# lisvulaczo/lodestar

Hardware: AMD Instinct MI355X
Metric: BLS signature sets verified/sec (whole node) at 1/2/4/8 MI355X; p50 batch latency (higher is better)
Workload: dtype u32

## Files before the change

### include/lodestar_bls.h

```cpp
#ifndef LODESTAR_BLS_H
#define LODESTAR_BLS_H

#include <stddef.h>
#include <stdint.h>

#ifdef __cplusplus
extern "C" {
#endif

#define LSG_OK 0
#define LSG_ERR_INVALID_ARG 1
#define LSG_ERR_NO_DEVICE 2
#define LSG_ERR_DEVICE 3
#define LSG_ERR_NOMEM 4
#define LSG_ERR_CLOSED 5
#define LSG_ERR_BUSY 6
#define LSG_ERR_ENTROPY 7

#define LSG_BLST_SUCCESS 0
#define LSG_BLST_BAD_ENCODING 1
#define LSG_BLST_POINT_NOT_ON_CURVE 2
#define LSG_BLST_POINT_NOT_IN_GROUP 3
#define LSG_BLST_AGGR_TYPE_MISMATCH 4
#define LSG_BLST_VERIFY_FAIL 5
// ... 35 lines not shown

typedef struct {
  int32_t status;
  int32_t err_code;
} lsg_job_result;

typedef struct {
  uint32_t batch_retries;
  uint32_t batch_sigs_success;
  uint64_t start_ns;
  uint64_t end_ns;
  uint32_t n_final_exps;
  uint32_t submit_us;
  int32_t key_error;
  uint32_t key_error_job;
} lsg_stats;

int lsg_init(int device_ordinal, lsg_ctx** out);
int lsg_init_devices(const int* device_ids, int n_devices, lsg_ctx** out);
int lsg_destroy(lsg_ctx* ctx);
int lsg_device_count(lsg_ctx* ctx, int32_t* n);
const char* lsg_last_error(lsg_ctx* ctx);
int lsg_device_name(lsg_ctx* ctx, char* buf, size_t len);
int lsg_reserve(lsg_ctx* ctx, size_t max_sets, size_t max_pks, size_t max_msg_bytes, int32_t n_slots);
int lsg_allocation_count(lsg_ctx* ctx, uint64_t* n);

int lsg_submit_jobs(lsg_ctx* ctx, const lsg_job* jobs, size_t n_jobs, uint64_t seed, lsg_ticket* ticket);
int lsg_wait_jobs(lsg_ctx* ctx, lsg_ticket ticket, lsg_job_result* results , lsg_stats* stats);
int lsg_jobs_partial(lsg_ctx* ctx, lsg_ticket ticket, uint8_t* out576, int32_t* has_batch);
int lsg_jobs_partial_device(lsg_ctx* ctx, lsg_ticket ticket, void* dev_out576, int32_t* has_batch);
int lsg_wait_jobs_node(lsg_ctx* ctx, lsg_ticket ticket, int32_t node_valid, lsg_job_result* results,
                       lsg_stats* stats);
int lsg_set_coalesce(lsg_ctx* ctx, uint32_t max_sets, int32_t max_inflight);
int lsg_assign_jobs(const uint32_t* job_sets, size_t n_jobs, int32_t n_devices, int32_t* owner);
int lsg_pipeline_slots(lsg_ctx* ctx, int32_t* n);
int lsg_poll(lsg_ctx* ctx, lsg_ticket ticket, int32_t* done);
int lsg_verify_jobs(lsg_ctx* ctx, const lsg_job* jobs, size_t n_jobs, uint64_t seed, lsg_job_result* results,
                    lsg_stats* stats);

int lsg_verify_sets(lsg_ctx* ctx, const lsg_set* sets, size_t n_sets, uint64_t seed, lsg_job_result* result);

int lsg_aggregate_pubkeys(lsg_ctx* ctx, const uint8_t* pks, uint32_t pk_len, size_t n, uint8_t* out96,
                          int32_t* err_code);
int lsg_aggregate_pubkeys_multi(lsg_ctx* ctx, const lsg_set* sets, size_t n_sets, uint8_t* out96, int32_t* err);

int lsg_hash_to_g2(lsg_ctx* ctx, const uint8_t* msgs, uint32_t msg_len, size_t n, const uint8_t* dst,
                   uint32_t dst_len, uint8_t* out192);

int lsg_sig_decode(lsg_ctx* ctx, const uint8_t* sigs, uint32_t sig_len, size_t n, uint8_t* out192, int32_t* err);

int lsg_batch_partial(lsg_ctx* ctx, const lsg_set* sets, size_t n_sets, uint64_t seed, uint8_t* out576,
                      int32_t* set_err, int32_t* any_error);
int lsg_final_verify(lsg_ctx* ctx, const uint8_t* partials576, size_t n_partials, int32_t* valid);
int lsg_final_submit(lsg_ctx* ctx, const uint8_t* partials576, size_t n_partials, lsg_ticket* ticket);
int lsg_final_submit_device(lsg_ctx* ctx, const void* dev_partials576, size_t n_partials, lsg_ticket* ticket);
int lsg_final_wait(lsg_ctx* ctx, lsg_ticket ticket, int32_t* valid);
int lsg_final_submit_groups(lsg_ctx* ctx, const uint8_t* partials576, size_t n_groups, size_t per_group,
                            lsg_ticket* ticket);
int lsg_final_wait_groups(lsg_ctx* ctx, lsg_ticket ticket, int32_t* valid );

int lsg_pubkey_table_set(lsg_ctx* ctx, size_t first_index, const uint8_t* pks, uint32_t pk_len, size_t n,
                         int32_t* err);
int lsg_pubkey_table_size(lsg_ctx* ctx, size_t* n);

int lsg_pubkey_validate(lsg_ctx* ctx, const uint8_t* pks, uint32_t pk_len, size_t n, uint8_t* out96, int32_t* err);

int lsg_aggregate_signatures(lsg_ctx* ctx, const uint8_t* sigs, uint32_t sig_len, const uint32_t* offsets,
                             size_t n_groups, uint8_t* out96, int32_t* err);

int lsg_signing_roots(lsg_ctx* ctx, const uint8_t* roots32, size_t n, const uint8_t* domain32, uint32_t domain_stride,
                      uint8_t* out32);
int lsg_attestation_signing_roots(lsg_ctx* ctx, const uint8_t* data128, size_t n, const uint8_t* domain32,
                                  uint32_t domain_stride, uint8_t* out32);
int lsg_deposit_signing_roots(lsg_ctx* ctx, const uint8_t* msgs88, size_t n, const uint8_t* domain32,
                              uint32_t domain_stride, uint8_t* out32);

int lsg_verify_deposits(lsg_ctx* ctx, const uint8_t* data184, size_t n, const uint8_t* domain32, uint64_t seed,
                        uint8_t* valid, int32_t* err);

int lsg_sign(lsg_ctx* ctx, const uint8_t* sks32, const uint8_t* msgs, uint32_t msg_len, size_t n, uint8_t* out96);
int lsg_sk_to_pk(lsg_ctx* ctx, const uint8_t* sks32, size_t n, uint8_t* out96);

int lsg_check_fp2_mul(lsg_ctx* ctx, const uint32_t* in, size_t n, uint32_t* out);
int lsg_probe_fp_mul_rate(lsg_ctx* ctx, double* fp_mul_per_s, double* mad_per_s);

int lsg_probe_mad_peak(lsg_ctx* ctx, double* mad_per_s);

int lsg_last_kernel_times(lsg_ctx* ctx, const char** names, double* ms, int max);

#ifdef __cplusplus
}
#endif
#endif
```

### lodestar_amd/_native.py

```python
import ctypes
import os
import struct
import threading

HERE = os.path.dirname(os.path.abspath(__file__))
LIB_PATH = os.environ.get("LSG_LIB", os.path.join(HERE, "liblodestar_bls.so"))
AB_LIB_PATH = os.path.join(HERE, "liblodestar_bls_ab.so")

LSG_OK = 0
LSG_ERR_NO_DEVICE = 2
LSG_ERR_BUSY = 6
LSG_ERR_ENTROPY = 7

LSG_INVALID = 0
LSG_VALID = 1
LSG_ERROR = 2

LSG_JOB_BATCHABLE = 1
LSG_JOB_PRIORITY = 2
LSG_JOB_VALIDATE_KEYS = 4

BLST_NAMES = {
    0: "BLST_SUCCESS", 1: "BLST_BAD_ENCODING", 2: "BLST_POINT_NOT_ON_CURVE", 3: "BLST_POINT_NOT_IN_GROUP",
    4: "BLST_AGGR_TYPE_MISMATCH", 5: "BLST_VERIFY_FAIL", 6: "BLST_PK_IS_INFINITY", 7: "BLST_BAD_SCALAR",
    10: "BLST_INVALID_SIZE",
}
LSG_ERR_EMPTY_SET = 100
LSG_ERR_EMPTY_AGGREGATE = 101
LSG_ERR_BAD_INDEX = 102
LSG_PK_INDEX = 4


def error_message(code):
    if code == LSG_ERR_EMPTY_SET:
        return "Empty signature set"
    if code == LSG_ERR_EMPTY_AGGREGATE:
        return "EMPTY_AGGREGATE_ARRAY"
    if code == LSG_ERR_BAD_INDEX:
        return "Unknown pubkey index"
    return "BLST_ERROR: " + BLST_NAMES.get(code, f"BLST_UNKNOWN_{code}")


class NativeUnavailable(RuntimeError):
    pass


class PkIndices(list):

    def tobytes(self):
        import array
        a = array.array("I", self)
        assert a.itemsize == 4
        return a.tobytes()


class LsgSet(ctypes.Structure):
    _fields_ = [
        ("pks", ctypes.c_void_p), ("pk_len", ctypes.c_uint32), ("n_pks", ctypes.c_uint32),
        ("msg", ctypes.c_void_p), ("msg_len", ctypes.c_uint32),
        ("sig", ctypes.c_void_p), ("sig_len", ctypes.c_uint32),
    ]


class LsgJob(ctypes.Structure):
    _fields_ = [("sets", ctypes.POINTER(LsgSet)), ("n_sets", ctypes.c_uint32), ("flags", ctypes.c_uint32)]


class LsgJobResult(ctypes.Structure):
    _fields_ = [("status", ctypes.c_int32), ("err_code", ctypes.c_int32)]


class LsgStats(ctypes.Structure):
    _fields_ = [
        ("batch_retries", ctypes.c_uint32), ("batch_sigs_success", ctypes.c_uint32),
        ("start_ns", ctypes.c_uint64), ("end_ns", ctypes.c_uint64),
        ("n_final_exps", ctypes.c_uint32), ("submit_us", ctypes.c_uint32),
        ("key_error", ctypes.c_int32), ("key_error_job", ctypes.c_uint32),
    ]


_lib = None
_lib_lock = threading.Lock()

EXPORTS = [
    "lsg_init", "lsg_init_devices", "lsg_destroy", "lsg_device_count", "lsg_last_error", "lsg_device_name",
    "lsg_reserve", "lsg_allocation_count", "lsg_verify_jobs", "lsg_verify_sets",
    "lsg_aggregate_pubkeys", "lsg_hash_to_g2", "lsg_sig_decode", "lsg_batch_partial", "lsg_final_verify",
    "lsg_probe_fp_mul_rate", "lsg_last_kernel_times", "lsg_sign", "lsg_sk_to_pk",
    "lsg_submit_jobs", "lsg_wait_jobs", "lsg_wait_jobs_node", "lsg_jobs_partial", "lsg_assign_jobs", "lsg_poll",
    "lsg_final_submit", "lsg_final_wait", "lsg_pipeline_slots", "lsg_probe_mad_peak",
    "lsg_pubkey_table_set", "lsg_pubkey_table_size", "lsg_pubkey_validate",
    "lsg_final_submit_groups", "lsg_final_wait_groups", "lsg_aggregate_signatures",
    "lsg_signing_roots", "lsg_attestation_signing_roots", "lsg_jobs_partial_device", "lsg_final_submit_device",
    "lsg_set_coalesce", "lsg_aggregate_pubkeys_multi", "lsg_check_fp2_mul",
    "lsg_deposit_signing_roots", "lsg_verify_deposits",
]


def load_library(path=LIB_PATH):
    global _lib
    with _lib_lock:
        if _lib is not None and path == LIB_PATH:
            return _lib
        if not os.path.exists(path):
            raise NativeUnavailable(f"{path} not built (run python -c 'import __graft_entry__; __graft_entry__.build()')")
        lib = ctypes.CDLL(path)
        vp, u32, u64, i32, sz = ctypes.c_void_p, ctypes.c_uint32, ctypes.c_uint64, ctypes.c_int32, ctypes.c_size_t
        pi32 = ctypes.POINTER(ctypes.c_int32)
        lib.lsg_init.argtypes = [ctypes.c_int, ctypes.POINTER(vp)]
        lib.lsg_init_devices.argtypes = [ctypes.POINTER(ctypes.c_int), ctypes.c_int, ctypes.POINTER(vp)]
        lib.lsg_device_count.argtypes = [vp, pi32]
        lib.lsg_reserve.argtypes = [vp, sz, sz, sz, i32]
        lib.lsg_allocation_count.argtypes = [vp, ctypes.POINTER(u64)]
        lib.lsg_wait_jobs_node.argtypes = [vp, u64, i32, ctypes.POINTER(LsgJobResult), ctypes.POINTER(LsgStats)]
        lib.lsg_jobs_partial.argtypes = [vp, u64, ctypes.c_char_p, pi32]
        lib.lsg_jobs_partial_device.argtypes = [vp, u64, vp, pi32]
        lib.lsg_final_submit_device.argtypes = [vp, vp, sz, ctypes.POINTER(u64)]
        lib.lsg_assign_jobs.argtypes = [ctypes.POINTER(u32), sz, i32, pi32]
        lib.lsg_destroy.argtypes = [vp]
        lib.lsg_last_error.argtypes = [vp]
        lib.lsg_last_error.restype = ctypes.c_char_p
        lib.lsg_device_name.argtypes = [vp, ctypes.c_char_p, sz]
        lib.lsg_verify_jobs.argtypes = [vp, ctypes.POINTER(LsgJob), sz, u64, ctypes.POINTER(LsgJobResult),
                                        ctypes.POINTER(LsgStats)]
        lib.lsg_verify_sets.argtypes = [vp, ctypes.POINTER(LsgSet), sz, u64, ctypes.POINTER(LsgJobResult)]
        lib.lsg_aggregate_pubkeys.argtypes = [vp, ctypes.c_char_p, u32, sz, ctypes.c_char_p, pi32]
        lib.lsg_aggregate_pubkeys_multi.argtypes = [vp, ctypes.POINTER(LsgSet), sz, ctypes.c_char_p, pi32]
        lib.lsg_hash_to_g2.argtypes = [vp, ctypes.c_char_p, u32, sz, ctypes.c_char_p, u32, ctypes.c_char_p]
        lib.lsg_sig_decode.argtypes = [vp, ctypes.c_char_p, u32, sz, ctypes.c_char_p, pi32]
        lib.lsg_batch_partial.argtypes = [vp, ctypes.POINTER(LsgSet), sz, u64, ctypes.c_char_p, pi32, pi32]
        lib.lsg_final_verify.argtypes = [vp, ctypes.c_char_p, sz, pi32]
        lib.lsg_probe_fp_mul_rate.argtypes = [vp, ctypes.POINTER(ctypes.c_double), ctypes.POINTER(ctypes.c_double)]
        lib.lsg_last_kernel_times.argtypes = [vp, ctypes.POINTER(ctypes.c_char_p), ctypes.POINTER(ctypes.c_double),
                                              ctypes.c_int]
        lib.lsg_sign.argtypes = [vp, ctypes.c_char_p, ctypes.c_char_p, u32, sz, ctypes.c_char_p]
        lib.lsg_sk_to_pk.argtypes = [vp, ctypes.c_char_p, sz, ctypes.c_char_p]
        pu64 = ctypes.POINTER(u64)
        lib.lsg_submit_jobs.argtypes = [vp, ctypes.POINTER(LsgJob), sz, u64, pu64]
        lib.lsg_wait_jobs.argtypes = [vp, u64, ctypes.POINTER(LsgJobResult), ctypes.POINTER(LsgStats)]
        lib.lsg_poll.argtypes = [vp, u64, pi32]
        lib.lsg_pubkey_table_set.argtypes = [vp, sz, ctypes.c_char_p, u32, sz, pi32]
        lib.lsg_pubkey_table_size.argtypes = [vp, ctypes.POINTER(sz)]
        lib.lsg_final_submit_groups.argtypes = [vp, ctypes.c_char_p, sz, sz, pu64]
        lib.lsg_final_wait_groups.argtypes = [vp, u64, pi32]
        lib.lsg_pubkey_validate.argtypes = [vp, ctypes.c_char_p, u32, sz, ctypes.c_char_p, pi32]
        lib.lsg_signing_roots.argtypes = [vp, ctypes.c_char_p, sz, ctypes.c_char_p, u32, ctypes.c_char_p]
        lib.lsg_attestation_signing_roots.argtypes = [vp, ctypes.c_char_p, sz, ctypes.c_char_p, u32, ctypes.c_char_p]
        lib.lsg_deposit_signing_roots.argtypes = [vp, ctypes.c_char_p, sz, ctypes.c_char_p, u32, ctypes.c_char_p]
        lib.lsg_verify_deposits.argtypes = [vp, ctypes.c_char_p, sz, ctypes.c_char_p, u64, ctypes.c_char_p, pi32]
        lib.lsg_aggregate_signatures.argtypes = [vp, ctypes.c_char_p, u32, ctypes.POINTER(u32), sz,
                                                 ctypes.c_char_p, pi32]
        lib.lsg_final_submit.argtypes = [vp, ctypes.c_char_p, sz, pu64]
        lib.lsg_final_wait.argtypes = [vp, u64, pi32]
        lib.lsg_pipeline_slots.argtypes = [vp, pi32]
        lib.lsg_set_coalesce.argtypes = [vp, u32, i32]
        lib.lsg_check_fp2_mul.argtypes = [vp, ctypes.c_char_p, sz, ctypes.c_char_p]
        lib.lsg_probe_mad_peak.argtypes = [vp, ctypes.POINTER(ctypes.c_double)]
        for name in EXPORTS:
            if name != "lsg_last_error":
                getattr(lib, name).restype = ctypes.c_int
        if path == LIB_PATH:
            _lib = lib
        return lib


class SetBuffer:

    def __init__(self, sets):
        self._keep = []
        sets = list(sets)
        self.arr = (LsgSet * max(len(sets), 1))()
        for i, (pks, msg, sig) in enumerate(sets):
            if isinstance(pks, PkIndices):
                pk_len, pkb = LSG_PK_INDEX, pks.tobytes()
            else:
                pk_len = len(pks[0]) if pks else 96
                if any(len(p) != pk_len for p in pks):
                    raise ValueError("all pubkeys of one set must share one encoding length")
                pkb = b"".join(pks)
            for b in (pkb, msg, sig):
                self._keep.append(b)
            s = self.arr[i]
            s.pks = ctypes.cast(ctypes.c_char_p(pkb), ctypes.c_void_p) if pkb else None
            s.pk_len = pk_len
            s.n_pks = len(pks)
            s.msg = ctypes.cast(ctypes.c_char_p(msg), ctypes.c_void_p) if msg else None
            s.msg_len = len(msg)
            s.sig = ctypes.cast(ctypes.c_char_p(sig), ctypes.c_void_p) if sig else None
            s.sig_len = len(sig)
        self.n = len(sets)


def assign_jobs(job_sizes, n_devices):
    lib = load_library()
    n = len(job_sizes)
    sizes = (ctypes.c_uint32 * max(n, 1))(*job_sizes)
    owner = (ctypes.c_int32 * max(n, 1))()
    rc = lib.lsg_assign_jobs(sizes, n, int(n_devices), owner)
    if rc != LSG_OK:
        raise ValueError(f"lsg_assign_jobs failed ({rc})")
    return list(owner[:n])


class PreparedJobs:

    def __init__(self, jobs):
        import numpy as np
        flat = [st for sets, _ in jobs for st in sets]
        n = len(flat)
        pk_parts, pk_len, n_pks = [], np.zeros(max(n, 1), np.uint32), np.zeros(max(n, 1), np.uint32)
        for i, (pks, _m, _s) in enumerate(flat):
            if isinstance(pks, PkIndices):
                pk_len[i], b = LSG_PK_INDEX, pks.tobytes()
            else:
                pk_len[i] = len(pks[0]) if pks else 96
                if any(len(p) != pk_len[i] for p in pks):
                    raise ValueError("all pubkeys of one set must share one encoding length")
                b = b"".join(pks)
            n_pks[i] = len(pks)
            pk_parts.append(b)

        def pack(parts):
            lens = np.array([len(p) for p in parts] or [0], np.uint64)
            offs = np.zeros_like(lens)
            if len(parts) > 1:
                offs[1:] = np.cumsum(lens)[:-1]
            buf = np.frombuffer(b"".join(parts) + b"\0", dtype=np.uint8).copy()
            return buf, offs, lens

        self._pk, pk_off, _ = pack(pk_parts)
        self._msg, msg_off, msg_len = pack([m for _, m, _ in flat])
        self._sig, sig_off, sig_len = pack([s for _, _, s in flat])
        self.sets = (LsgSet * max(n, 1))()
        dt = np.dtype({"names": ["pks", "pk_len", "n_pks", "msg", "msg_len", "sig", "sig_len"],
                       "formats": [np.uint64, np.uint32, np.uint32, np.uint64, np.uint32, np.uint64, np.uint32],
                       "offsets": [LsgSet.pks.offset, LsgSet.pk_len.offset, LsgSet.n_pks.offset, LsgSet.msg.offset,
                                   LsgSet.msg_len.offset, LsgSet.sig.offset, LsgSet.sig_len.offset],
                       "itemsize": ctypes.sizeof(LsgSet)})
        v = np.frombuffer(self.sets, dtype=dt)
# ... 268 lines not shown
            return []
        sl = len(sigs[0])
        assert all(len(s) == sl for s in sigs)
        out = ctypes.create_string_buffer(192 * len(sigs))
        err = (ctypes.c_int32 * len(sigs))()
        self._check(self.lib.lsg_sig_decode(self.h, b"".join(sigs), sl, len(sigs), out, err), "lsg_sig_decode")
        raw = out.raw
        return [(raw[192 * i:192 * i + 192], err[i]) for i in range(len(sigs))]

    def batch_partial(self, sets, seed=0):
        b = SetBuffer(sets)
        out = ctypes.create_string_buffer(576)
        errs = (ctypes.c_int32 * max(b.n, 1))()
        anyerr = ctypes.c_int32()
        self._check(self.lib.lsg_batch_partial(self.h, b.arr, b.n, seed, out, errs, ctypes.byref(anyerr)),
                    "lsg_batch_partial")
        return out.raw, [errs[i] for i in range(b.n)], bool(anyerr.value)

    def final_verify(self, partials):
        v = ctypes.c_int32()
        self._check(self.lib.lsg_final_verify(self.h, b"".join(partials), len(partials), ctypes.byref(v)),
                    "lsg_final_verify")
        return bool(v.value)

    def final_submit(self, partials):
        t = ctypes.c_uint64()
        rc = self.lib.lsg_final_submit(self.h, b"".join(partials), len(partials), ctypes.byref(t))
        if rc == LSG_ERR_BUSY:
            return None
        self._check(rc, "lsg_final_submit")
        return t.value

    def final_wait(self, ticket):
        v = ctypes.c_int32()
        self._check(self.lib.lsg_final_wait(self.h, ticket, ctypes.byref(v)), "lsg_final_wait")
        return bool(v.value)

    def final_submit_groups(self, groups):
        ng = len(groups)
        pg = len(groups[0]) if groups else 0
        if any(len(g) != pg for g in groups):
            raise ValueError("every group needs the same number of partials")
        t = ctypes.c_uint64()
        rc = self.lib.lsg_final_submit_groups(self.h, b"".join(b"".join(g) for g in groups), ng, pg, ctypes.byref(t))
        if rc == LSG_ERR_BUSY:
            return None
        self._check(rc, "lsg_final_submit_groups")
        t_ng = ng
        return (t.value, t_ng)

    def final_wait_groups(self, ticket):
        t, ng = ticket
        v = (ctypes.c_int32 * max(ng, 1))()
        self._check(self.lib.lsg_final_wait_groups(self.h, t, v), "lsg_final_wait_groups")
        return [bool(x) for x in v[:ng]]

    def sign(self, sks, msgs):
        if not sks:
            return []
        ml = len(msgs[0])
        out = ctypes.create_string_buffer(96 * len(sks))
        skb = b"".join(int(k).to_bytes(32, "big") for k in sks)
        self._check(self.lib.lsg_sign(self.h, skb, b"".join(msgs), ml, len(sks), out), "lsg_sign")
        raw = out.raw
        return [raw[96 * i:96 * i + 96] for i in range(len(sks))]

    def sk_to_pk(self, sks):
        if not sks:
            return []
        out = ctypes.create_string_buffer(96 * len(sks))
        skb = b"".join(int(k).to_bytes(32, "big") for k in sks)
        self._check(self.lib.lsg_sk_to_pk(self.h, skb, len(sks), out), "lsg_sk_to_pk")
        raw = out.raw
        return [raw[96 * i:96 * i + 96] for i in range(len(sks))]

    def check_fp2_mul(self, words):
        n = len(words) // 56
        assert len(words) == 56 * n
        out = ctypes.create_string_buffer(4 * 28 * n)
        src = struct.pack(f"<{len(words)}I", *words)
        self._check(self.lib.lsg_check_fp2_mul(self.h, src, n, out), "lsg_check_fp2_mul")
        return list(struct.unpack(f"<{28 * n}I", out.raw))

    def probe_fp_mul_rate(self):
        a, b = ctypes.c_double(), ctypes.c_double()
        self._check(self.lib.lsg_probe_fp_mul_rate(self.h, ctypes.byref(a), ctypes.byref(b)), "lsg_probe_fp_mul_rate")
        return a.value, b.value

    def last_kernel_times(self, max_entries=1024):
        names = (ctypes.c_char_p * max_entries)()
        ms = (ctypes.c_double * max_entries)()
        n = self.lib.lsg_last_kernel_times(self.h, names, ms, max_entries)
        return [(names[i].decode(), ms[i]) for i in range(n)]
```

### lodestar_amd/csrc/lsg_curve.hpp

```cpp
#pragma once
#include "lsg_tower.hpp"

LSG_INL fp_t fadd(const fp_t& a, const fp_t& b) { return fp_add(a, b); }
LSG_INL fp2_t fadd(const fp2_t& a, const fp2_t& b) { return fp2_add(a, b); }
LSG_INL fp_t fsub(const fp_t& a, const fp_t& b) { return fp_sub(a, b); }
LSG_INL fp2_t fsub(const fp2_t& a, const fp2_t& b) { return fp2_sub(a, b); }
LSG_INL fp_t fmul(const fp_t& a, const fp_t& b) { return fp_mul(a, b); }
LSG_INL fp2_t fmul(const fp2_t& a, const fp2_t& b) { return fp2_mul(a, b); }
LSG_INL fp_t fsqr(const fp_t& a) { return fp_sqr(a); }
LSG_INL fp2_t fsqr(const fp2_t& a) { return fp2_sqr(a); }
LSG_INL fp_t fneg(const fp_t& a) { return fp_neg(a); }
LSG_INL fp2_t fneg(const fp2_t& a) { return fp2_neg(a); }
LSG_INL fp_t fmul_b3(const fp_t& a) { return fp_mul12(a); }
LSG_INL fp2_t fmul_b3(const fp2_t& a) { return fp2_mul_b3(a); }
LSG_INL bool fis_zero(const fp_t& a) { return fp_is_zero(a); }
LSG_INL bool fis_zero(const fp2_t& a) { return fp2_is_zero(a); }
LSG_INL bool feq(const fp_t& a, const fp_t& b) { return fp_eq(a, b); }
LSG_INL bool feq(const fp2_t& a, const fp2_t& b) { return fp2_eq(a, b); }
LSG_INL fp_t fselect(bool c, const fp_t& a, const fp_t& b) { return fp_select(c, a, b); }
LSG_INL fp2_t fselect(bool c, const fp2_t& a, const fp2_t& b) { return fp2_select(c, a, b); }
LSG_INL fp_t finv(const fp_t& a) { return fp_inv(a); }
LSG_INL fp2_t finv(const fp2_t& a) { return fp2_inv(a); }
template <class F> LSG_INL F fzero();
template <> LSG_INL fp_t fzero<fp_t>() { return fp_zero(); }
template <> LSG_INL fp2_t fzero<fp2_t>() { return fp2_zero(); }
template <class F> LSG_INL F fone();
template <> LSG_INL fp_t fone<fp_t>() { return FP_ONE; }
template <> LSG_INL fp2_t fone<fp2_t>() { return fp2_one(); }

template <class F>
struct aff_t {
  F x, y;
};
template <class F>
struct proj_t {
  F X, Y, Z;
};
typedef aff_t<fp_t> g1a_t;
typedef aff_t<fp2_t> g2a_t;
typedef proj_t<fp_t> g1p_t;
typedef proj_t<fp2_t> g2p_t;

template <class F>
LSG_INL proj_t<F> proj_inf() {
  proj_t<F> r;
  r.X = fzero<F>();
  r.Y = fone<F>();
  r.Z = fzero<F>();
  return r;
}

template <class F>
LSG_INL proj_t<F> proj_from_aff(const aff_t<F>& a) {
  proj_t<F> r;
  r.X = a.x;
  r.Y = a.y;
  r.Z = fone<F>();
  return r;
}

template <class F>
LSG_INL bool proj_is_inf(const proj_t<F>& a) {
  return fis_zero(a.Z);
}

template <class F>
LSG_INL proj_t<F> proj_neg(const proj_t<F>& a) {
  proj_t<F> r = a;
  r.Y = fneg(a.Y);
  return r;
}

template <class F>
LSG_INL proj_t<F> proj_add(const proj_t<F>& p, const proj_t<F>& q) {
  F t0 = fmul(p.X, q.X);
  F t1 = fmul(p.Y, q.Y);
  F t2 = fmul(p.Z, q.Z);
  F t3 = fmul(fadd(p.X, p.Y), fadd(q.X, q.Y));
  F t4 = fadd(t0, t1);
  t3 = fsub(t3, t4);
  t4 = fmul(fadd(p.Y, p.Z), fadd(q.Y, q.Z));
  F X3 = fadd(t1, t2);
  t4 = fsub(t4, X3);
  X3 = fmul(fadd(p.X, p.Z), fadd(q.X, q.Z));
  F Y3 = fadd(t0, t2);
  Y3 = fsub(X3, Y3);
  X3 = fadd(t0, t0);
  t0 = fadd(X3, t0);
  t2 = fmul_b3(t2);
  F Z3 = fadd(t1, t2);
  t1 = fsub(t1, t2);
  Y3 = fmul_b3(Y3);
  X3 = fmul(t4, Y3);
  t2 = fmul(t3, t1);
  X3 = fsub(t2, X3);
  Y3 = fmul(Y3, t0);
  t1 = fmul(t1, Z3);
  Y3 = fadd(t1, Y3);
  t0 = fmul(t0, t3);
  Z3 = fmul(Z3, t4);
  Z3 = fadd(Z3, t0);
  proj_t<F> r;
  r.X = X3;
  r.Y = Y3;
  r.Z = Z3;
  return r;
}

template <class F>
LSG_INL proj_t<F> proj_add_mixed(const proj_t<F>& p, const aff_t<F>& q) {
  F t0 = fmul(p.X, q.x);
  F t1 = fmul(p.Y, q.y);
  F t3 = fmul(fadd(q.x, q.y), fadd(p.X, p.Y));
  F t4 = fadd(t0, t1);
  t3 = fsub(t3, t4);
  t4 = fadd(fmul(q.y, p.Z), p.Y);
  F Y3 = fadd(fmul(q.x, p.Z), p.X);
  F X3 = fadd(t0, t0);
  t0 = fadd(X3, t0);
  F t2 = fmul_b3(p.Z);
  F Z3 = fadd(t1, t2);
  t1 = fsub(t1, t2);
  Y3 = fmul_b3(Y3);
  X3 = fmul(t4, Y3);
  t2 = fmul(t3, t1);
  X3 = fsub(t2, X3);
  Y3 = fmul(Y3, t0);
  t1 = fmul(t1, Z3);
  Y3 = fadd(t1, Y3);
  t0 = fmul(t0, t3);
  Z3 = fmul(Z3, t4);
  Z3 = fadd(Z3, t0);
  proj_t<F> r;
  r.X = X3;
  r.Y = Y3;
  r.Z = Z3;
  return r;
}

template <class F>
LSG_INL proj_t<F> proj_dbl(const proj_t<F>& p) {
  F t0 = fsqr(p.Y);
  F Z3 = fadd(t0, t0);
  Z3 = fadd(Z3, Z3);
  Z3 = fadd(Z3, Z3);
  F t1 = fmul(p.Y, p.Z);
  F t2 = fmul_b3(fsqr(p.Z));
  F X3 = fmul(t2, Z3);
  F Y3 = fadd(t0, t2);
  Z3 = fmul(t1, Z3);
  t1 = fadd(t2, t2);
  t2 = fadd(t1, t2);
  t0 = fsub(t0, t2);
  Y3 = fmul(t0, Y3);
  Y3 = fadd(X3, Y3);
  t1 = fmul(p.X, p.Y);
  X3 = fmul(t0, t1);
  X3 = fadd(X3, X3);
  proj_t<F> r;
  r.X = X3;
  r.Y = Y3;
  r.Z = Z3;
  return r;
}

LSG_BIGFN g1p_t g1_add(g1p_t p, g1p_t q) { return proj_add(p, q); }
LSG_BIGFN g1p_t g1_add_mixed(g1p_t p, g1a_t q) { return proj_add_mixed(p, q); }
LSG_BIGFN g1p_t g1_dbl(g1p_t p) { return proj_dbl(p); }
#ifdef LSG_ROW_SPLIT
LSG_INL void kar_prep(fp_t* x, fp_t* y, int k, const fp2_t& a, const fp2_t& b) {
  x[k] = a.c0;
  y[k] = b.c0;
  x[k + 1] = a.c1;
  y[k + 1] = b.c1;
  x[k + 2] = fp_add(a.c0, a.c1);
  y[k + 2] = fp_add(b.c0, b.c1);
}
LSG_INL fp2_t kar_fin(const fp_t* z, int k) {
  return fp2_t(fp_sub(z[k], z[k + 1]), fp_sub(fp_sub(z[k + 2], z[k]), z[k + 1]));
}
LSG_INL g2p_t g2_add_rows(const g2p_t& p, const g2p_t& q) {
  fp_t x[18], y[18], z[18];
  kar_prep(x, y, 0, p.X, q.X);
  kar_prep(x, y, 3, p.Y, q.Y);
  kar_prep(x, y, 6, p.Z, q.Z);
  kar_prep(x, y, 9, fp2_add(p.X, p.Y), fp2_add(q.X, q.Y));
  kar_prep(x, y, 12, fp2_add(p.Y, p.Z), fp2_add(q.Y, q.Z));
  kar_prep(x, y, 15, fp2_add(p.X, p.Z), fp2_add(q.X, q.Z));
  fp_mul_list<18>(z, x, y);
  fp2_t t0 = kar_fin(z, 0), t1 = kar_fin(z, 3), t2 = kar_fin(z, 6);
  const fp2_t t3 = fp2_sub(kar_fin(z, 9), fp2_add(t0, t1));
  const fp2_t t4 = fp2_sub(kar_fin(z, 12), fp2_add(t1, t2));
  fp2_t Y3 = fp2_sub(kar_fin(z, 15), fp2_add(t0, t2));
  t0 = fp2_add(fp2_add(t0, t0), t0);
  t2 = fp2_mul_b3(t2);
  const fp2_t Z3 = fp2_add(t1, t2);
  t1 = fp2_sub(t1, t2);
  Y3 = fp2_mul_b3(Y3);
  kar_prep(x, y, 0, t4, Y3);
  kar_prep(x, y, 3, t3, t1);
  kar_prep(x, y, 6, Y3, t0);
  kar_prep(x, y, 9, t1, Z3);
  kar_prep(x, y, 12, t0, t3);
  kar_prep(x, y, 15, Z3, t4);
  fp_mul_list<18>(z, x, y);
  g2p_t r;
  r.X = fp2_sub(kar_fin(z, 3), kar_fin(z, 0));
  r.Y = fp2_add(kar_fin(z, 9), kar_fin(z, 6));
  r.Z = fp2_add(kar_fin(z, 15), kar_fin(z, 12));
  return r;
}
LSG_INL g2p_t g2_dbl_rows(const g2p_t& p) {
  fp_t x[12], y[12], z[12];
  kar_prep(x, y, 0, p.Y, p.Y);
  kar_prep(x, y, 3, p.Y, p.Z);
  kar_prep(x, y, 6, p.Z, p.Z);
  kar_prep(x, y, 9, p.X, p.Y);
  fp_mul_list<12>(z, x, y);
  const fp2_t t0 = kar_fin(z, 0), t1 = kar_fin(z, 3), t2 = fp2_mul_b3(kar_fin(z, 6)), xy = kar_fin(z, 9);
  const fp2_t z8 = fp2_dbl(fp2_dbl(fp2_dbl(t0)));
  const fp2_t y3 = fp2_add(t0, t2);
  const fp2_t s0 = fp2_sub(t0, fp2_add(fp2_add(t2, t2), t2));
  kar_prep(x, y, 0, t2, z8);
  kar_prep(x, y, 3, t1, z8);
  kar_prep(x, y, 6, s0, y3);
  kar_prep(x, y, 9, s0, xy);
  fp_mul_list<12>(z, x, y);
  g2p_t r;
  r.X = fp2_dbl(kar_fin(z, 9));
  r.Y = fp2_add(kar_fin(z, 0), kar_fin(z, 6));
  r.Z = kar_fin(z, 3);
  return r;
}
LSG_BIGFN g2p_t g2_add(g2p_t p, g2p_t q) { return g2_add_rows(p, q); }
LSG_BIGFN g2p_t g2_dbl(g2p_t p) { return g2_dbl_rows(p); }
#else
LSG_BIGFN g2p_t g2_add(g2p_t p, g2p_t q) { return proj_add(p, q); }
LSG_BIGFN g2p_t g2_dbl(g2p_t p) { return proj_dbl(p); }
#endif
LSG_BIGFN g2p_t g2_add_mixed(g2p_t p, g2a_t q) { return proj_add_mixed(p, q); }

LSG_INL g1p_t gadd(const g1p_t& p, const g1p_t& q) { return g1_add(p, q); }
LSG_INL g2p_t gadd(const g2p_t& p, const g2p_t& q) { return g2_add(p, q); }
LSG_INL g1p_t gdbl(const g1p_t& p) { return g1_dbl(p); }
LSG_INL g2p_t gdbl(const g2p_t& p) { return g2_dbl(p); }

template <class F>
struct jac_t {
  F X, Y, Z;
};

template <class F>
LSG_INL jac_t<F> jac_from_proj(const proj_t<F>& p) {
  F zz = fsqr(p.Z);
  jac_t<F> r;
  bool inf = fis_zero(p.Z);
  r.X = fselect(inf, fone<F>(), fmul(p.X, p.Z));
  r.Y = fselect(inf, fone<F>(), fmul(p.Y, zz));
  r.Z = p.Z;
  return r;
}

template <class F>
LSG_INL proj_t<F> jac_to_proj(const jac_t<F>& p) {
  F zz = fsqr(p.Z);
  proj_t<F> r;
  bool inf = fis_zero(p.Z);
  r.X = fmul(p.X, p.Z);
  r.Y = fselect(inf, fone<F>(), p.Y);
  r.Z = fmul(zz, p.Z);
  return r;
}

template <class F>
LSG_INL jac_t<F> jac_dbl_t(const jac_t<F>& p) {
  F A = fsqr(p.X);
  F B = fsqr(p.Y);
  F C = fsqr(B);
  F D = fsub(fsqr(fadd(p.X, B)), fadd(A, C));
  D = fadd(D, D);
  F E = fadd(fadd(A, A), A);
  F Fq = fsqr(E);
  jac_t<F> r;
  r.X = fsub(Fq, fadd(D, D));
  F C8 = fadd(C, C);
  C8 = fadd(C8, C8);
  C8 = fadd(C8, C8);
  r.Y = fsub(fmul(E, fsub(D, r.X)), C8);
  F yz = fmul(p.Y, p.Z);
  r.Z = fadd(yz, yz);
  return r;
}
LSG_BIGFN jac_t<fp_t> jac_dbl(jac_t<fp_t> p) { return jac_dbl_t(p); }
LSG_BIGFN jac_t<fp2_t> jac_dbl(jac_t<fp2_t> p) { return jac_dbl_t(p); }

template <class F>
LSG_INL jac_t<F> jac_add_proj(const jac_t<F>& acc, const proj_t<F>& q) {
  return jac_from_proj(gadd(jac_to_proj(acc), q));
}

template <class F>
LSG_INL proj_t<F> proj_mul_u64(const proj_t<F>& p, uint64_t k) {
  proj_t<F> T[16];
  T[0] = proj_inf<F>();
  T[1] = p;
  T[2] = gdbl(p);
#pragma unroll 1
  for (int d = 3; d < 16; d++) T[d] = gadd(T[d - 1], p);
  auto pick = [&](uint32_t d) { return T[d]; };
  jac_t<F> acc = jac_from_proj(pick((uint32_t)(k >> 60) & 15u));
#pragma unroll 1
  for (int w = 14; w >= 0; w--) {
    acc = jac_dbl(acc);
    acc = jac_dbl(acc);
    acc = jac_dbl(acc);
    acc = jac_dbl(acc);
    acc = jac_add_proj(acc, pick((uint32_t)(k >> (4 * w)) & 15u));
  }
  return jac_to_proj(acc);
}

template <class F>
LSG_INL proj_t<F> proj_pick_signed(const proj_t<F>& T1, const proj_t<F>& T2, const proj_t<F>& T3,
                                   const proj_t<F>& T4, int d) {
  const int a = d < 0 ? -d : d;
  proj_t<F> r = proj_inf<F>();
  auto take = [&](bool s, const proj_t<F>& t) {
    r.X = fselect(s, t.X, r.X);
    r.Y = fselect(s, t.Y, r.Y);
    r.Z = fselect(s, t.Z, r.Z);
  };
  take(a == 1, T1);
  take(a == 2, T2);
  take(a == 3, T3);
  take(a == 4, T4);
  r.Y = fselect(d < 0, fneg(r.Y), r.Y);
  return r;
}
template <class F>
LSG_INL proj_t<F> proj_mul_u64_s3(const proj_t<F>& p, uint64_t k) {
  const proj_t<F> T2 = gdbl(p);
  const proj_t<F> T3 = gadd(T2, p);
  const proj_t<F> T4 = gdbl(T2);
  uint32_t cm = 0;
#pragma unroll
  for (int i = 0; i < 21; i++) {
    const uint32_t v = (uint32_t)((k >> (3 * i)) & 7u) + ((cm >> i) & 1u);
    cm |= (v >= 4u ? 1u : 0u) << (i + 1);
  }
  auto digit = [&](int i) {
    return (int)((k >> (3 * i)) & 7u) + (int)((cm >> i) & 1u) - (i < 21 ? 8 * (int)((cm >> (i + 1)) & 1u) : 0);
  };
  jac_t<F> acc = jac_from_proj(proj_pick_signed(p, T2, T3, T4, digit(21)));
#pragma unroll 1
  for (int i = 20; i >= 0; i--) {
    acc = jac_dbl(acc);
    acc = jac_dbl(acc);
    acc = jac_dbl(acc);
    acc = jac_add_proj(acc, proj_pick_signed(p, T2, T3, T4, digit(i)));
  }
  return jac_to_proj(acc);
}

template <class F, class G>
LSG_INL proj_t<F> proj_mul_xabs_get(const G& get) {
  const uint64_t xa = ((uint64_t)LSG_X_ABS_HI << 32) | LSG_X_ABS_LO;
  jac_t<F> acc = jac_from_proj(get());
#pragma unroll 1
  for (int b = 62; b >= 0; b--) {
    acc = jac_dbl(acc);
    if ((xa >> b) & 1u) acc = jac_add_proj(acc, get());
  }
  return jac_to_proj(acc);
}
template <class F>
LSG_INL proj_t<F> proj_mul_xabs(const proj_t<F>& p) {
  return proj_mul_xabs_get<F>([&]() { return p; });
}

template <class F>
LSG_INL bool proj_eq(const proj_t<F>& a, const proj_t<F>& b) {
  bool ia = proj_is_inf(a), ib = proj_is_inf(b);
  if (ia || ib) return ia && ib;
  return feq(fmul(a.X, b.Z), fmul(b.X, a.Z)) && feq(fmul(a.Y, b.Z), fmul(b.Y, a.Z));
}

template <class F>
LSG_INL aff_t<F> proj_to_aff(const proj_t<F>& p) {
  F zi = finv(p.Z);
  aff_t<F> r;
  r.x = fmul(p.X, zi);
  r.y = fmul(p.Y, zi);
  return r;
}

LSG_INL g2p_t g2_psi(const g2p_t& p) {
  g2p_t r;
  r.X = fp2_mul(fp2_conj(p.X), PSI_CX);
  r.Y = fp2_mul(fp2_conj(p.Y), PSI_CY);
  r.Z = fp2_conj(p.Z);
  return r;
}
LSG_INL g2p_t g2_psi2(const g2p_t& p) {
  g2p_t r;
  r.X = fp2_mul_fp(p.X, PSI2_CX);
  r.Y = fp2_mul_fp(p.Y, PSI2_CY);
  r.Z = p.Z;
  return r;
}

template <class G>
LSG_INL bool g2_in_group_get(const G& get) {
  if (proj_is_inf(get())) return true;
  g2p_t xp = proj_neg(proj_mul_xabs_get<fp2_t>(get));
  return proj_eq(g2_psi(get()), xp);
}
LSG_BIGFN bool g2_in_group(g2p_t p) {
  return g2_in_group_get([&]() { return p; });
}

LSG_BIGFN bool g1_in_group(g1p_t p) {
  const uint32_t rw[8] = {0x73eda753u, 0x299d7d48u, 0x3339d808u, 0x09a1d805u,
                          0x53bda402u, 0xfffe5bfeu, 0xffffffffu, 0x00000001u};
  g1p_t acc = proj_inf<fp_t>();
#pragma unroll 1
  for (int w = 0; w < 8; w++) {
#pragma unroll 1
    for (int b = 31; b >= 0; b--) {
      acc = g1_dbl(acc);
      if ((rw[w] >> b) & 1u) acc = g1_add(acc, p);
    }
  }
  return proj_is_inf(acc);
}

LSG_INL bool g1_on_curve_aff(const g1a_t& a) {
  fp_t rhs = fp_add(fp_mul(fp_sqr(a.x), a.x), FP_B_G1);
  return fp_eq(fp_sqr(a.y), rhs);
}
LSG_INL bool g2_on_curve_aff(const g2a_t& a) {
  fp2_t rhs = fp2_add(fp2_mul(fp2_sqr(a.x), a.x), FP2_B_G2);
  return fp2_eq(fp2_sqr(a.y), rhs);
}

#ifndef LSG_BLST_SUCCESS
#define LSG_BLST_SUCCESS 0
#define LSG_BLST_BAD_ENCODING 1
#define LSG_BLST_POINT_NOT_ON_CURVE 2
#define LSG_BLST_POINT_NOT_IN_GROUP 3
#define LSG_BLST_AGGR_TYPE_MISMATCH 4
#define LSG_BLST_VERIFY_FAIL 5
#define LSG_BLST_PK_IS_INFINITY 6
#define LSG_BLST_BAD_SCALAR 7
#define LSG_BLST_INVALID_SIZE 10
#endif

LSG_INL int g2_uncompress(g2a_t& out, bool& inf, const uint8_t* in) {
  uint8_t in0 = in[0];
  inf = false;
  if (!(in0 & 0x80)) return LSG_BLST_BAD_ENCODING;
  if (in0 & 0x40) {
    uint32_t acc = in0 & 0x3f;
    for (int i = 1; i < 96; i++) acc |= in[i];
    if (acc == 0) {
      inf = true;
      out.x = fp2_zero();
      out.y = fp2_zero();
      return LSG_BLST_SUCCESS;
    }
    return LSG_BLST_BAD_ENCODING;
  }
  fp_t x1 = fp_from_be48(in);
  x1 = fp_mask_flags(x1);
  fp_t x0 = fp_from_be48(in + 48);
  if (!fp_canon_lt_p(x1) || !fp_canon_lt_p(x0)) return LSG_BLST_BAD_ENCODING;
  fp2_t x = fp2_make(fp_to_mont(x0), fp_to_mont(x1));
  fp2_t rhs = fp2_add(fp2_mul(fp2_sqr(x), x), FP2_B_G2);
  fp2_t y;
  if (!fp2_sqrt(y, rhs)) return LSG_BLST_POINT_NOT_ON_CURVE;
  bool want = (in0 & 0x20) != 0;
  if (fp2_lexi_largest(y) != want) y = fp2_neg(y);
  out.x = x;
  out.y = y;
  if (fp2_is_zero(x)) return LSG_BLST_POINT_NOT_IN_GROUP;
  return LSG_BLST_SUCCESS;
}

LSG_INL int g2_deserialize_uncompressed(g2a_t& out, bool& inf, const uint8_t* in) {
  uint8_t in0 = in[0];
  inf = false;
  if (in0 & 0x80) return LSG_BLST_BAD_ENCODING;
  if (in0 & 0x40) {
    uint32_t acc = in0 & 0x3f;
    for (int i = 1; i < 192; i++) acc |= in[i];
    if (acc == 0) {
      inf = true;
      out.x = fp2_zero();
      out.y = fp2_zero();
      return LSG_BLST_SUCCESS;
    }
// ... 87 lines not shown
```

### lodestar_amd/csrc/lsg_fp_pair.hpp

```cpp
#pragma once
#include "lsg_constants_r29.hpp"

#ifndef LSG_PAIR_G
#define LSG_PAIR_G 2
#endif
#define LSG_GROUP LSG_PAIR_G
#define LSG_PAIR_MODE 1
#define LSG_LEAN_TOWER 1
constexpr int LSG_PL = 14 / LSG_GROUP;
constexpr uint32_t LSG_M29 = (1u << 29) - 1;

#if LSG_PAIR_G == 2
#undef LSG_INL
#define LSG_INL __device__ __forceinline__
#undef LSG_NOINL
#define LSG_NOINL __device__ __noinline__
#define LSG_PFN __device__ __forceinline__
#define LSG_PLEAF __device__ __noinline__
LSG_PFN uint32_t pair_h() { return __lane_id() & 1u; }
template <int CTRL>
LSG_PFN uint32_t pdpp(uint32_t x) {
  return (uint32_t)__builtin_amdgcn_mov_dpp((int)x, CTRL, 0xf, 0xf, false);
}
template <int S>
// ... 311 lines not shown
  r.l[5] = hi[1];
  r.l[6] = hi[2];
  return r;
}
#define LSG_TAIL_PARAMS(x) fp_arg4_t x##_lo, fp_arg3_t x##_hi
#define LSG_TAIL_ARGS(v) fp_pack_lo(v), fp_pack_hi(v)
#define LSG_TAIL_UNPACK(x) fp_unpack2(x##_lo, x##_hi)
typedef uint32_t fp_arg_t __attribute__((ext_vector_type(8)));
LSG_PFN fp_arg_t fp_pack(const fp_t& a) {
  fp_arg_t v;
#pragma unroll
  for (int k = 0; k < LSG_PL; k++) v[k] = a.l[k];
  return v;
}
LSG_PFN fp_t fp_unpack(const fp_arg_t& v) {
  fp_t r;
#pragma unroll
  for (int k = 0; k < LSG_PL; k++) r.l[k] = v[k];
  return r;
}
#else
#define LSG_TAIL_PARAMS(x) fp_t x
#define LSG_TAIL_ARGS(v) (v)
#define LSG_TAIL_UNPACK(x) (x)
typedef fp_t fp_arg_t;
LSG_PFN fp_arg_t fp_pack(const fp_t& a) { return a; }
LSG_PFN fp_t fp_unpack(const fp_arg_t& v) { return v; }
#endif
struct fp_duo {
  fp_t x, y;
};
LSG_PLEAF fp_duo pair_mont_mul2_v(fp_arg_t a0, fp_arg_t b0, fp_arg_t a1, LSG_TAIL_PARAMS(b1)) {
  LSG_COUNT_MUL();
  LSG_COUNT_MUL();
  const fp_t x[2] = {fp_unpack(a0), fp_unpack(a1)}, y[2] = {fp_unpack(b0), LSG_TAIL_UNPACK(b1)};
  fp_t r[2];
#if LSG_LEAF_MODE == 2
  pair_mont_mul_n<2>(r, x, y);
#else
  pair_mont_mul_n<1>(&r[0], &x[0], &y[0]);
  LSG_SCHED_FENCE();
  pair_mont_mul_n<1>(&r[1], &x[1], &y[1]);
#endif
  return fp_duo{r[0], r[1]};
}
LSG_PFN fp_duo pair_mont_mul2(const fp_t& a0, const fp_t& b0, const fp_t& a1, const fp_t& b1) {
  return pair_mont_mul2_v(fp_pack(a0), fp_pack(b0), fp_pack(a1), LSG_TAIL_ARGS(b1));
}
LSG_PLEAF fp_duo pair_fp2_mul_v(fp_arg_t a0, fp_arg_t a1, fp_arg_t b0, LSG_TAIL_PARAMS(b1));
LSG_PLEAF fp_duo pair_fp2_sqr_v(fp_arg_t a0, fp_arg_t a1);
LSG_PFN fp_duo pair_fp2_mul(const fp_t& a0, const fp_t& a1, const fp_t& b0, const fp_t& b1) {
  return pair_fp2_mul_v(fp_pack(a0), fp_pack(a1), fp_pack(b0), LSG_TAIL_ARGS(b1));
}
LSG_PFN fp_duo pair_fp2_sqr(const fp_t& a0, const fp_t& a1) { return pair_fp2_sqr_v(fp_pack(a0), fp_pack(a1)); }
#if LSG_LEAF_MODE != 0
#define LSG_FP2_LEAF 1
#endif

LSG_PFN fp_t fp_zero() {
  fp_t r;
#pragma unroll
  for (int k = 0; k < LSG_PL; k++) r.l[k] = 0u;
  return r;
}
LSG_PFN fp_t fp_select(bool c, const fp_t& a, const fp_t& b) {
  fp_t r;
#pragma unroll
  for (int k = 0; k < LSG_PL; k++) r.l[k] = c ? a.l[k] : b.l[k];
  return r;
}
LSG_PFN fp_t fp_add(const fp_t& a, const fp_t& b) {
  fp_t r;
#pragma unroll
  for (int k = 0; k < LSG_PL; k++) r.l[k] = a.l[k] + b.l[k];
  return pair_carry(r);
}
LSG_PFN fp_t fp_sub(const fp_t& a, const fp_t& b) {
  fp_t r;
#pragma unroll
  for (int k = 0; k < LSG_PL; k++) r.l[k] = a.l[k] - b.l[k];
  return pair_carry(r);
}
LSG_PFN fp_t fp_neg(const fp_t& a) { return fp_sub(fp_zero(), a); }
LSG_PFN fp_t fp_mul(const fp_t& a, const fp_t& b) { return pair_mont_mul(a, b); }
#if LSG_LEAF_MODE == 0
LSG_PFN void fp_mul2(fp_t& r0, fp_t& r1, const fp_t& a0, const fp_t& b0, const fp_t& a1, const fp_t& b1) {
  fp_t t = pair_mont_mul(a0, b0);
  r1 = pair_mont_mul(a1, b1);
  r0 = t;
}
LSG_PFN void fp_mul3(fp_t& r0, fp_t& r1, fp_t& r2, const fp_t& a0, const fp_t& b0, const fp_t& a1, const fp_t& b1,
                     const fp_t& a2, const fp_t& b2) {
  fp_t t0 = pair_mont_mul(a0, b0);
  fp_t t1 = pair_mont_mul(a1, b1);
  r2 = pair_mont_mul(a2, b2);
  r0 = t0;
  r1 = t1;
}
#else
LSG_PFN void fp_mul2(fp_t& r0, fp_t& r1, const fp_t& a0, const fp_t& b0, const fp_t& a1, const fp_t& b1) {
  const fp_duo d = pair_mont_mul2(a0, b0, a1, b1);
  r0 = d.x;
  r1 = d.y;
}
LSG_PFN void fp_mul3(fp_t& r0, fp_t& r1, fp_t& r2, const fp_t& a0, const fp_t& b0, const fp_t& a1, const fp_t& b1,
                     const fp_t& a2, const fp_t& b2) {
  const fp_duo d = pair_mont_mul2(a0, b0, a1, b1);
  r2 = pair_mont_mul(a2, b2);
  r0 = d.x;
  r1 = d.y;
}
#endif
LSG_PFN void fp_mul9(fp_t* r, const fp_t* a, const fp_t* b) {
#pragma unroll
  for (int g = 0; g < 9; g += 3) fp_mul3(r[g], r[g + 1], r[g + 2], a[g], b[g], a[g + 1], b[g + 1], a[g + 2], b[g + 2]);
}

LSG_PLEAF fp_duo pair_fp2_mul_v(fp_arg_t va0, fp_arg_t va1, fp_arg_t vb0, LSG_TAIL_PARAMS(vb1)) {
  LSG_COUNT_MUL();
  LSG_COUNT_MUL();
  LSG_COUNT_MUL();
  const fp_t a0 = fp_unpack(va0), a1 = fp_unpack(va1), b0 = fp_unpack(vb0), b1 = LSG_TAIL_UNPACK(vb1);
#if LSG_FP2_SOP
  fp_duo d;
  pair_fp2_mul_sop(d.x, d.y, a0, a1, b0, b1);
  return d;
#endif
  fp_t t[3];
#if LSG_LEAF_MODE == 2
  const fp_t a[3] = {a0, a1, fp_add(a0, a1)}, b[3] = {b0, b1, fp_add(b0, b1)};
  pair_mont_mul_n<3>(t, a, b);
#else
  pair_mont_mul_n<1>(&t[0], &a0, &b0);
  LSG_SCHED_FENCE();
  pair_mont_mul_n<1>(&t[1], &a1, &b1);
  LSG_SCHED_FENCE();
  const fp_t s0 = fp_add(a0, a1), s1 = fp_add(b0, b1);
  pair_mont_mul_n<1>(&t[2], &s0, &s1);
#endif
  return fp_duo{fp_sub(t[0], t[1]), fp_sub(fp_sub(t[2], t[0]), t[1])};
}
LSG_PLEAF fp_duo pair_fp2_sqr_v(fp_arg_t va0, fp_arg_t va1) {
  LSG_COUNT_MUL();
  LSG_COUNT_MUL();
  const fp_t a0 = fp_unpack(va0), a1 = fp_unpack(va1);
  fp_t t[2];
#if LSG_LEAF_MODE == 2
  const fp_t a[2] = {fp_add(a0, a1), a0}, b[2] = {fp_sub(a0, a1), a1};
  pair_mont_mul_n<2>(t, a, b);
#else
  const fp_t s = fp_add(a0, a1), d = fp_sub(a0, a1);
  pair_mont_mul_n<1>(&t[0], &s, &d);
  LSG_SCHED_FENCE();
  pair_mont_mul_n<1>(&t[1], &a0, &a1);
#endif
  return fp_duo{t[0], fp_add(t[1], t[1])};
}

LSG_PLEAF fp_t pair_pow_fixed(fp_t a, const uint32_t* __restrict__ e) {
  auto mul = [](const fp_t& x, const fp_t& y) {
    LSG_COUNT_MUL();
    fp_t r;
    pair_mont_mul_n<1>(&r, &x, &y);
    return r;
  };
  fp_t T[8];
// ... 273 lines not shown
```

### lodestar_amd/csrc/lsg_host.hip

```cpp
#include <hip/hip_runtime.h>
#include <rccl/rccl.h>
#include <stdio.h>
#include <stdlib.h>
#include <errno.h>
#include <string.h>
#include <sys/random.h>
#include <time.h>

#include <algorithm>
#include <atomic>
#include <condition_variable>
#include <chrono>
#include <mutex>
#include <shared_mutex>
#include <thread>
#include <unordered_map>
#include <string>
#include <vector>

#include "../../include/lodestar_bls.h"
#include "lsg_launch.h"
#include "lsg_layout.h"
#include "lsg_serial.h"
#include "lsg_ab.h"
// ... 2952 lines not shown
    }
    return (int)LSG_OK;
  };
  size_t pkg = 0;
  for (size_t o = 0; o < n && !rc; pkg++) {
    const size_t cnt = std::min(DEPOSIT_PKG, n - o);
    lsg_ticket t = 0;
    if (out.size() >= DEPOSIT_INFLIGHT) {
      rc = wait_oldest();
      pkg--;
      continue;
    }
    {
      CtxLock lk(c->mu);
      const hipError_t he = hipSetDevice(d->device);
      if (he != hipSuccess)
        rc = fail_c(c, "hipSetDevice", he);
      else
        rc = submit_pkg(c, lk, jobs.data() + o, cnt, seed ? seed + 0x9e3779b97f4a7c15ull * pkg : 0, &t, true,
                        resident ? P_<uint8_t>(d->d_dep_roots) + 32 * o : nullptr);
    }
    if (rc == LSG_ERR_BUSY && !out.empty()) {
      rc = wait_oldest();
      pkg--;
      continue;
    }
    if (rc) break;
    out.push_back({t, o, cnt});
    o += cnt;
  }
  while (!out.empty()) {
    const int w = wait_oldest();
    if (!rc) rc = w;
  }
  return rc;
}

int lsg_sign(lsg_ctx* c, const uint8_t* sks32, const uint8_t* msgs, uint32_t msg_len, size_t n, uint8_t* out96) {
  if (!c || !out96 || (n && (!sks32 || !msgs))) return LSG_ERR_INVALID_ARG;
  LSG_ENTER(c);
  Slot* s = &c->dev[0]->util;
  timer_reset(s);
  if (n == 0) return LSG_OK;
  LSG_RC(util_hash(s, msgs, msg_len, n, DST_POP, DST_POP_LEN));
  LSG_RC(ensure(s, s->d_aux, 96 * n));
  LSG_RC(ensure(s, s->d_Fb, 32 * n));
  LSG_HIP(s, hipMemcpyAsync(s->d_Fb.p, sks32, 32 * n, hipMemcpyHostToDevice, s->st[0]));
  KL(s, "k_sign", lsgk::sign(S_(s), (int)n, P_<uint8_t>(s->d_Fb), P_<uint32_t>(s->d_H), P_<uint8_t>(s->d_aux)));
  LSG_HIP(s, hipMemcpyAsync(out96, s->d_aux.p, 96 * n, hipMemcpyDeviceToHost, s->st[0]));
  LSG_HIP(s, hipStreamSynchronize(s->st[0]));
  return LSG_OK;
}

int lsg_sk_to_pk(lsg_ctx* c, const uint8_t* sks32, size_t n, uint8_t* out96) {
  if (!c || !out96 || (n && !sks32)) return LSG_ERR_INVALID_ARG;
  LSG_ENTER(c);
  Slot* s = &c->dev[0]->util;
  timer_reset(s);
  if (n == 0) return LSG_OK;
  LSG_RC(ensure(s, s->d_aux, 96 * n));
  LSG_RC(ensure(s, s->d_Fb, 32 * n));
  LSG_HIP(s, hipMemcpyAsync(s->d_Fb.p, sks32, 32 * n, hipMemcpyHostToDevice, s->st[0]));
  KL(s, "k_sk_to_pk", lsgk::sk_to_pk(S_(s), (int)n, P_<uint8_t>(s->d_Fb), P_<uint8_t>(s->d_aux)));
  LSG_HIP(s, hipMemcpyAsync(out96, s->d_aux.p, 96 * n, hipMemcpyDeviceToHost, s->st[0]));
  LSG_HIP(s, hipStreamSynchronize(s->st[0]));
  return LSG_OK;
}

int lsg_check_fp2_mul(lsg_ctx* c, const uint32_t* in, size_t n, uint32_t* out) {
  if (!c || (n && (!in || !out)) || n > 0x7fffffffull / (4 * W_FP)) return LSG_ERR_INVALID_ARG;
  LSG_ENTER(c);
  if (n == 0) return LSG_OK;
  Slot* s = &c->dev[0]->util;
  timer_reset(s);
  LSG_RC(ensure(s, s->d_aux, 4 * 4 * W_FP * n));
  LSG_RC(ensure(s, s->d_Fb, 4 * 2 * W_FP * n));
  LSG_HIP(s, hipMemcpyAsync(s->d_aux.p, in, 4 * 4 * W_FP * n, hipMemcpyHostToDevice, s->st[0]));
  KL(s, "k_check_fp2_mul", lsgk::check_fp2_mul(S_(s), (int)n, P_<uint32_t>(s->d_aux), P_<uint32_t>(s->d_Fb)));
  LSG_HIP(s, hipMemcpyAsync(out, s->d_Fb.p, 4 * 2 * W_FP * n, hipMemcpyDeviceToHost, s->st[0]));
  LSG_HIP(s, hipStreamSynchronize(s->st[0]));
  return LSG_OK;
}

int lsg_probe_fp_mul_rate(lsg_ctx* c, double* fp_mul_per_s, double* mad_per_s) {
  if (!c || !fp_mul_per_s || !mad_per_s) return LSG_ERR_INVALID_ARG;
  LSG_ENTER(c);
  Slot* s = &c->dev[0]->util;
  hipDeviceProp_t prop;
  LSG_HIP(s, hipGetDeviceProperties(&prop, c->dev[0]->device));
  const int items = prop.multiProcessorCount * 32 * 32;
  LSG_RC(ensure(s, s->d_aux, 4 * W_FP * (size_t)items));
  std::vector<uint32_t> init(W_FP * (size_t)items, 0);
  for (size_t i = 0; i < init.size(); i += 4) init[i] = (uint32_t)(i * 2654435761u) & 0x1fffffffu;
  LSG_HIP(s, hipMemcpy(s->d_aux.p, init.data(), 4 * init.size(), hipMemcpyHostToDevice));
  const int iters = 64;
  hipStream_t S = s->st[0];
  LSG_HIP(s, lsgk::probe_fp_mul(S, items, 2, P_<uint32_t>(s->d_aux)));
  hipEvent_t a, b;
  LSG_HIP(s, hipEventCreate(&a));
  LSG_HIP(s, hipEventCreate(&b));
  LSG_HIP(s, hipEventRecord(a, S));
  LSG_HIP(s, lsgk::probe_fp_mul(S, items, iters, P_<uint32_t>(s->d_aux)));
  LSG_HIP(s, hipEventRecord(b, S));
  LSG_HIP(s, hipEventSynchronize(b));
  float ms = 0;
  LSG_HIP(s, hipEventElapsedTime(&ms, a, b));
  (void)hipEventDestroy(a);
  (void)hipEventDestroy(b);
  *fp_mul_per_s = (double)items * iters * 4.0 / (ms * 1e-3);
  *mad_per_s = *fp_mul_per_s * 300.0;
  return LSG_OK;
}

int lsg_probe_mad_peak(lsg_ctx* c, double* mad_per_s) {
  if (!c || !mad_per_s) return LSG_ERR_INVALID_ARG;
  LSG_ENTER(c);
  Slot* s = &c->dev[0]->util;
  hipDeviceProp_t prop;
  LSG_HIP(s, hipGetDeviceProperties(&prop, c->dev[0]->device));
  const int blocks = prop.multiProcessorCount * 32;
  const size_t threads = (size_t)blocks * 256;
  LSG_RC(ensure(s, s->d_aux, 8 * threads));
  hipStream_t S = s->st[0];
  const int iters = 4096;
  LSG_HIP(s, lsgk::probe_mad(S, blocks, 16, 3u, P_<uint64_t>(s->d_aux)));
  hipEvent_t a, b;
  LSG_HIP(s, hipEventCreate(&a));
  LSG_HIP(s, hipEventCreate(&b));
  LSG_HIP(s, hipEventRecord(a, S));
  LSG_HIP(s, lsgk::probe_mad(S, blocks, iters, 5u, P_<uint64_t>(s->d_aux)));
  LSG_HIP(s, hipEventRecord(b, S));
  LSG_HIP(s, hipEventSynchronize(b));
  float ms = 0;
  LSG_HIP(s, hipEventElapsedTime(&ms, a, b));
  (void)hipEventDestroy(a);
  (void)hipEventDestroy(b);
  *mad_per_s = (double)threads * iters * 16.0 / (ms * 1e-3);
  return LSG_OK;
}

int lsg_last_kernel_times(lsg_ctx* c, const char** names, double* ms, int max) {
  if (!c) return 0;
  std::lock_guard<std::mutex> lk(c->mu);
  const auto& v = c->dev[0]->last_times;
  int n = 0;
  for (size_t i = 0; i < v.size() && n < max; i++, n++) {
    if (names) names[n] = v[i].first;
    if (ms) ms[n] = v[i].second;
  }
  return n;
}

int lsg_assign_jobs(const uint32_t* job_sets, size_t n_jobs, int32_t n_devices, int32_t* owner) {
  if ((n_jobs && (!job_sets || !owner)) || n_devices < 1) return LSG_ERR_INVALID_ARG;
  assign_jobs(job_sets, n_jobs, n_devices, owner);
  return LSG_OK;
}

}
```

### lodestar_amd/csrc/lsg_k_miller.hip

```cpp
#include "lsg_kcommon.hpp"

constexpr int W_LINE_LANE = (int)(sizeof(line_t) / 4);
LSG_DEVI void line_store(uint32_t* __restrict__ lines, size_t n, size_t i, int st, const line_t& L) {
  uint32_t w[W_LINE_LANE];
  __builtin_memcpy(w, &L, sizeof(line_t));
  uint32_t* p = lines + (((size_t)st * W_LINE_LANE) * n + i) * LSG_GROUP + (threadIdx.x % LSG_GROUP);
#pragma unroll
  for (int k = 0; k < W_LINE_LANE; k++) p[(size_t)k * n * LSG_GROUP] = w[k];
}
LSG_DEVI line_t line_load(const uint32_t* __restrict__ lines, size_t n, size_t i, int st) {
  uint32_t w[W_LINE_LANE];
  const uint32_t* p = lines + (((size_t)st * W_LINE_LANE) * n + i) * LSG_GROUP + (threadIdx.x % LSG_GROUP);
#pragma unroll
  for (int k = 0; k < W_LINE_LANE; k++) w[k] = p[(size_t)k * n * LSG_GROUP];
  line_t L;
  __builtin_memcpy(&L, w, sizeof(line_t));
  return L;
}

__global__ void LSG_KERNEL_ATTR k_miller_lines(int n, const uint32_t* __restrict__ H, uint32_t* __restrict__ lines) {
  LANE_ITEM(n);
  (void)lead;
  const g2a_t Q = lane_load<g2a_t>(H, item);
  miller_lines(Q, [&](int st, const line_t& L) { line_store(lines, (size_t)n, item, st, L); });
// ... 1 lines not shown

#ifndef LSG_ACCUM_WAVES
#define LSG_ACCUM_WAVES 1
#endif
template <int K>
__global__ void LSG_KERNEL_ATTR_W(LSG_ACCUM_WAVES)
    k_miller_accum(int n_items, const int32_t* __restrict__ item_first, const int32_t* __restrict__ item_cnt,
                   const uint32_t* __restrict__ P, const uint8_t* __restrict__ pinf, const uint8_t* __restrict__ hinf,
                   const int32_t* __restrict__ err, int n_sets, const uint32_t* __restrict__ lines,
                   uint32_t* __restrict__ f) {
  LANE_ITEM(n_items);
  (void)lead;
  const int first = item_first[item], cnt = item_cnt[item];
  g1a_t Pk[K];
  bool use[K];
  int idx[K];
#pragma unroll
  for (int k = 0; k < K; k++) {
    const int i = first + (k < cnt ? k : cnt - 1);
    idx[k] = i;
    use[k] = k < cnt && err[i] == 0 && !pinf[i] && !hinf[i];
    Pk[k] = lane_load<g1a_t>(P, i);
  }
  lane_store(f, item, miller_accum_multi<K>(Pk, use, [&](int k, int st) {
               return line_load(lines, (size_t)n_sets, (size_t)idx[k], st);
             }));
}

__global__ void LSG_KERNEL_ATTR k_miller_lines_list(int n, const int32_t* __restrict__ list, const uint32_t* __restrict__ H,
                                                    uint32_t* __restrict__ lines) {
  LANE_ITEM(n);
  (void)lead;
  const g2a_t Q = lane_load<g2a_t>(H, (size_t)list[item]);
  miller_lines(Q, [&](int st, const line_t& L) { line_store(lines, (size_t)n, item, st, L); });
}
__global__ void LSG_KERNEL_ATTR_W(LSG_ACCUM_WAVES)
    k_miller_accum_list(int n, const int32_t* __restrict__ list, const uint32_t* __restrict__ P,
                        const uint8_t* __restrict__ pinf, const uint8_t* __restrict__ hinf, const int32_t* __restrict__ err,
                        const uint32_t* __restrict__ lines, uint32_t* __restrict__ f) {
  LANE_ITEM(n);
  (void)lead;
  const int i = list[item];
  g1a_t Pk[1] = {lane_load<g1a_t>(P, (size_t)i)};
  bool use[1] = {err[i] == 0 && !pinf[i] && !hinf[i]};
  lane_store(f, item, miller_accum_multi<1>(Pk, use, [&](int, int st) { return line_load(lines, (size_t)n, item, st); }));
}

constexpr int MF_ITEMS = 32;
constexpr int MF_F = 0, MF_L = 12, MF_V = 36, MF_T = 66, MF_COMPS = 90;
constexpr size_t MF_LDS_BYTES = (size_t)MF_COMPS * 7 * 64 * 4;

LSG_DEVI uint32_t* mf_slot(uint32_t* lds, int c) { return lds + (size_t)c * 7 * 64 + (threadIdx.x & 63); }
LSG_DEVI void mf_put(uint32_t* lds, int c, const fp_t& v) {
  uint32_t* p = mf_slot(lds, c);
#pragma unroll
  for (int k = 0; k < LSG_PL; k++) p[k * 64] = v.l[k];
}
LSG_DEVI fp_t mf_get(uint32_t* lds, int c) {
  const uint32_t* p = mf_slot(lds, c);
  fp_t v;
#pragma unroll
  for (int k = 0; k < LSG_PL; k++) v.l[k] = p[k * 64];
  return v;
}
LSG_DEVI void mf_put2(uint32_t* lds, int c, const fp2_t& v) {
  mf_put(lds, c, v.c0);
  mf_put(lds, c + 1, v.c1);
}
LSG_DEVI fp2_t mf_get2(uint32_t* lds, int c) { return fp2_t(mf_get(lds, c), mf_get(lds, c + 1)); }
#define MF_FC(j) (MF_F + 2 * (j))
#define MF_LC(k, j) (MF_L + 6 * (k) + 2 * (j))
#define MF_VC(p) ((p) < 15 ? MF_V + 2 * (p) : ((p) == 15 ? MF_LC(1, 2) : MF_LC(3, 2)))

LSG_DEVI void mf_sqr(uint32_t* lds, int w) {
  {
    fp6_t x, y;
    const fp6_t a = fp6_make(mf_get2(lds, MF_FC(0)), mf_get2(lds, MF_FC(1)), mf_get2(lds, MF_FC(2)));
    const fp6_t b = fp6_make(mf_get2(lds, MF_FC(3)), mf_get2(lds, MF_FC(4)), mf_get2(lds, MF_FC(5)));
    if (w < 2) {
      x = a;
      y = b;
    } else {
      x = fp6_add(a, b);
      y = fp6_add(a, fp6_mul_v(b));
    }
    fp2_t p0, p1, p2;
    if ((w & 1) == 0) {
      p0 = fp2_mul(x.c0, y.c0);
      p1 = fp2_mul(x.c1, y.c1);
      p2 = fp2_mul(x.c2, y.c2);
    } else {
      p0 = fp2_mul(fp2_add(x.c1, x.c2), fp2_add(y.c1, y.c2));
      p1 = fp2_mul(fp2_add(x.c0, x.c1), fp2_add(y.c0, y.c1));
      p2 = fp2_mul(fp2_add(x.c0, x.c2), fp2_add(y.c0, y.c2));
    }
    mf_put2(lds, MF_VC(3 * w), p0);
    mf_put2(lds, MF_VC(3 * w + 1), p1);
    mf_put2(lds, MF_VC(3 * w + 2), p2);
  }
  __syncthreads();
  auto fin = [&](int base, int j) {
    const fp2_t v0 = mf_get2(lds, MF_VC(base)), v1 = mf_get2(lds, MF_VC(base + 1)), v2 = mf_get2(lds, MF_VC(base + 2));
    if (j == 0) return fp2_add(v0, fp2_mul_xi(fp2_sub(fp2_sub(mf_get2(lds, MF_VC(base + 3)), v1), v2)));
    if (j == 1) return fp2_add(fp2_sub(fp2_sub(mf_get2(lds, MF_VC(base + 4)), v0), v1), fp2_mul_xi(v2));
    return fp2_add(fp2_sub(fp2_sub(mf_get2(lds, MF_VC(base + 5)), v0), v2), v1);
  };
  fp2_t o0, o1, o2;
  if (w == 0) {
    o0 = fin(0, 0);
    o1 = fin(0, 1);
    o2 = fin(0, 2);
  } else if (w == 1) {
    o0 = fp2_sub(fp2_sub(fin(6, 0), fin(0, 0)), fp2_mul_xi(fin(0, 2)));
  } else if (w == 2) {
    o0 = fp2_sub(fp2_sub(fin(6, 1), fin(0, 1)), fin(0, 0));
  } else {
    o0 = fp2_sub(fp2_sub(fin(6, 2), fin(0, 2)), fin(0, 1));
  }
  if (w == 0) {
    mf_put2(lds, MF_FC(3), fp2_add(o0, o0));
    mf_put2(lds, MF_FC(4), fp2_add(o1, o1));
    mf_put2(lds, MF_FC(5), fp2_add(o2, o2));
  } else {
    mf_put2(lds, MF_FC(w - 1), o0);
  }
}

LSG_DEVI void mf_pair_lines(uint32_t* lds, int w) {
  const int pi = w >> 1, h = w & 1;
  {
    const fp2_t a0 = mf_get2(lds, MF_LC(2 * pi, 0)), a1 = mf_get2(lds, MF_LC(2 * pi, 1)),
                a2 = mf_get2(lds, MF_LC(2 * pi, 2));
    const fp2_t b0 = mf_get2(lds, MF_LC(2 * pi + 1, 0)), b1 = mf_get2(lds, MF_LC(2 * pi + 1, 1)),
                b2 = mf_get2(lds, MF_LC(2 * pi + 1, 2));
    if (h == 0) {
      mf_put2(lds, MF_VC(6 * pi), fp2_mul(a0, b0));
      mf_put2(lds, MF_VC(6 * pi + 1), fp2_mul(a2, b2));
      mf_put2(lds, MF_VC(6 * pi + 2), fp2_mul(a1, b1));
    } else {
      mf_put2(lds, MF_VC(6 * pi + 3), fp2_mul(fp2_add(a0, a1), fp2_add(b0, b1)));
      mf_put2(lds, MF_VC(6 * pi + 4), fp2_mul(fp2_add(a0, a2), fp2_add(b0, b2)));
      mf_put2(lds, MF_VC(6 * pi + 5), fp2_mul(fp2_add(a1, a2), fp2_add(b1, b2)));
    }
  }
  __syncthreads();
  const fp2_t P0 = mf_get2(lds, MF_VC(6 * pi)), P1 = mf_get2(lds, MF_VC(6 * pi + 1)), P2 = mf_get2(lds, MF_VC(6 * pi + 2));
  if (h == 0) {
    mf_put2(lds, MF_LC(2 * pi, 0), fp2_add(P0, fp2_mul_xi(P1)));
    mf_put2(lds, MF_LC(2 * pi, 1), fp2_sub(fp2_sub(mf_get2(lds, MF_VC(6 * pi + 3)), P0), P2));
    mf_put2(lds, MF_LC(2 * pi, 2), P2);
  } else {
    mf_put2(lds, MF_LC(2 * pi + 1, 0), fp2_sub(fp2_sub(mf_get2(lds, MF_VC(6 * pi + 4)), P0), P1));
    mf_put2(lds, MF_LC(2 * pi + 1, 1), fp2_sub(fp2_sub(mf_get2(lds, MF_VC(6 * pi + 5)), P2), P1));
  }
  __syncthreads();
}

LSG_DEVI void mf_mul_pair(uint32_t* lds, int w, int k) {
  {
    const fp2_t m0 = mf_get2(lds, MF_LC(2 * k, 0)), m1 = mf_get2(lds, MF_LC(2 * k, 1)), m2 = mf_get2(lds, MF_LC(2 * k, 2));
    if (w == 0) {
      const fp2_t a0 = mf_get2(lds, MF_FC(0)), a1 = mf_get2(lds, MF_FC(1)), a2 = mf_get2(lds, MF_FC(2));
      mf_put2(lds, MF_VC(0), fp2_mul(a0, m0));
      mf_put2(lds, MF_VC(1), fp2_mul(a1, m1));
      mf_put2(lds, MF_VC(2), fp2_mul(a2, m2));
      mf_put2(lds, MF_VC(3), fp2_mul(fp2_add(a0, a1), fp2_add(m0, m1)));
      mf_put2(lds, MF_VC(4), fp2_mul(fp2_add(a1, a2), fp2_add(m1, m2)));
    } else if (w == 1) {
      const fp2_t m4 = mf_get2(lds, MF_LC(2 * k + 1, 0)), m5 = mf_get2(lds, MF_LC(2 * k + 1, 1));
      const fp2_t b0 = mf_get2(lds, MF_FC(3)), b1 = mf_get2(lds, MF_FC(4));
      mf_put2(lds, MF_VC(5), fp2_mul(fp2_add(mf_get2(lds, MF_FC(0)), mf_get2(lds, MF_FC(2))), fp2_add(m0, m2)));
      mf_put2(lds, MF_VC(6), fp2_mul(b0, m4));
      mf_put2(lds, MF_VC(7), fp2_mul(b1, m5));
      mf_put2(lds, MF_VC(8), fp2_mul(fp2_add(b0, b1), fp2_add(m4, m5)));
    } else if (w == 2) {
      const fp2_t m4 = mf_get2(lds, MF_LC(2 * k + 1, 0)), m5 = mf_get2(lds, MF_LC(2 * k + 1, 1));
      const fp2_t b2 = mf_get2(lds, MF_FC(5));
      mf_put2(lds, MF_VC(9), fp2_mul(b2, m4));
      mf_put2(lds, MF_VC(10), fp2_mul(b2, m5));
      const fp2_t s0 = fp2_add(mf_get2(lds, MF_FC(0)), mf_get2(lds, MF_FC(3)));
      const fp2_t s1 = fp2_add(mf_get2(lds, MF_FC(1)), mf_get2(lds, MF_FC(4)));
      mf_put2(lds, MF_VC(11), fp2_mul(s0, m0));
      mf_put2(lds, MF_VC(12), fp2_mul(s1, fp2_add(m1, m4)));
    } else {
      const fp2_t m4 = mf_get2(lds, MF_LC(2 * k + 1, 0)), m5 = mf_get2(lds, MF_LC(2 * k + 1, 1));
      const fp2_t s0 = fp2_add(mf_get2(lds, MF_FC(0)), mf_get2(lds, MF_FC(3)));
      const fp2_t s1 = fp2_add(mf_get2(lds, MF_FC(1)), mf_get2(lds, MF_FC(4)));
      const fp2_t s2 = fp2_add(mf_get2(lds, MF_FC(2)), mf_get2(lds, MF_FC(5)));
      const fp2_t q1 = fp2_add(m1, m4), q2 = fp2_add(m2, m5);
      mf_put2(lds, MF_VC(13), fp2_mul(s2, q2));
      mf_put2(lds, MF_VC(14), fp2_mul(fp2_add(s0, s1), fp2_add(m0, q1)));
      mf_put2(lds, MF_VC(15), fp2_mul(fp2_add(s1, s2), fp2_add(q1, q2)));
      mf_put2(lds, MF_VC(16), fp2_mul(fp2_add(s0, s2), fp2_add(m0, q2)));
    }
  }
  __syncthreads();
  auto V = [&](int p) { return mf_get2(lds, MF_VC(p)); };
  auto t0c = [&](int j) {
    if (j == 0) return fp2_add(V(0), fp2_mul_xi(fp2_sub(fp2_sub(V(4), V(1)), V(2))));
    if (j == 1) return fp2_add(fp2_sub(fp2_sub(V(3), V(0)), V(1)), fp2_mul_xi(V(2)));
    return fp2_add(fp2_sub(fp2_sub(V(5), V(0)), V(2)), V(1));
  };
  auto t2c = [&](int j) {
    if (j == 0) return fp2_add(V(11), fp2_mul_xi(fp2_sub(fp2_sub(V(15), V(12)), V(13))));
    if (j == 1) return fp2_add(fp2_sub(fp2_sub(V(14), V(11)), V(12)), fp2_mul_xi(V(13)));
    return fp2_add(fp2_sub(fp2_sub(V(16), V(11)), V(13)), V(12));
  };
  auto nc = [&](int j) {
    if (j == 0) return fp2_add(V(6), fp2_mul_xi(V(10)));
    if (j == 1) return fp2_sub(fp2_sub(V(8), V(6)), V(7));
    return fp2_add(V(7), V(9));
  };
  fp2_t o0, o1;
  int j0, j1 = -1;
  if (w == 0) {
    o0 = fp2_add(t0c(0), fp2_mul_xi(nc(1)));
    o1 = fp2_add(t0c(1), fp2_mul_xi(nc(2)));
    j0 = 0;
    j1 = 1;
  } else if (w == 1) {
    o0 = fp2_add(t0c(2), nc(0));
    o1 = fp2_sub(fp2_sub(t2c(0), t0c(0)), fp2_mul_xi(nc(2)));
    j0 = 2;
    j1 = 3;
  } else if (w == 2) {
    o0 = fp2_sub(fp2_sub(t2c(1), t0c(1)), nc(0));
    j0 = 4;
  } else {
    o0 = fp2_sub(fp2_sub(t2c(2), t0c(2)), nc(1));
    j0 = 5;
  }
  mf_put2(lds, MF_FC(j0), o0);
  if (j1 >= 0) mf_put2(lds, MF_FC(j1), o1);
  __syncthreads();
}

#ifndef LSG_MF_STAGED
#define LSG_MF_STAGED 1
#endif
LSG_DEVI void mf_put_line(uint32_t* lds, int wl, bool use, const fp2_t& l00, const fp2_t& l01P, const fp2_t& l11P) {
  mf_put2(lds, MF_LC(wl, 0), fp2_select(use, l00, fp2_one()));
  mf_put2(lds, MF_LC(wl, 1), fp2_select(use, l01P, fp2_zero()));
  mf_put2(lds, MF_LC(wl, 2), fp2_select(use, l11P, fp2_zero()));
}
LSG_DEVI void mf_dbl_line(uint32_t* lds, int wl, bool use, const uint32_t* __restrict__ P, size_t sl) {
  const int tb = MF_T + 6 * wl;
  fp2_t t0, t1, t2, v1;
  {
    const fp2_t X = mf_get2(lds, tb), Y = mf_get2(lds, tb + 2), Z = mf_get2(lds, tb + 4);
    t0 = fp2_sqr(Y);
    t1 = fp2_mul(Y, Z);
    t2 = fp2_mul_b3(fp2_sqr(Z));
    const fp2_t XX = fp2_sqr(X);
    v1 = fp2_mul(X, Y);
    const g1a_t Pk = lane_load<g1a_t>(P, sl);
    mf_put_line(lds, wl, use, fp2_sub(t2, t0), fp2_mul_fp(fp2_add(fp2_add(XX, XX), XX), Pk.x),
                fp2_mul_fp(fp2_neg(fp2_add(t1, t1)), Pk.y));
  }
  fp2_t Z3 = fp2_add(t0, t0);
  Z3 = fp2_add(Z3, Z3);
  Z3 = fp2_add(Z3, Z3);
  fp2_t X3 = fp2_mul(t2, Z3);
  fp2_t Y3 = fp2_add(t0, t2);
  mf_put2(lds, tb + 4, fp2_mul(t1, Z3));
  const fp2_t u2 = fp2_add(fp2_add(t2, t2), t2);
  const fp2_t s0 = fp2_sub(t0, u2);
  Y3 = fp2_mul(s0, Y3);
  mf_put2(lds, tb + 2, fp2_add(X3, Y3));
  X3 = fp2_mul(s0, v1);
  mf_put2(lds, tb, fp2_add(X3, X3));
}
LSG_DEVI void mf_add_line(uint32_t* lds, int wl, bool use, const uint32_t* __restrict__ P, const uint32_t* __restrict__ H,
                          size_t sl) {
  const int tb = MF_T + 6 * wl;
  fp2_t theta, delta;
  {
    const g2a_t Q = lane_load<g2a_t>(H, sl);
    const fp2_t Z = mf_get2(lds, tb + 4);
    theta = fp2_sub(mf_get2(lds, tb + 2), fp2_mul(Q.y, Z));
    delta = fp2_sub(mf_get2(lds, tb), fp2_mul(Q.x, Z));
    const fp2_t l00 = fp2_sub(fp2_mul(delta, Q.y), fp2_mul(theta, Q.x));
    const g1a_t Pk = lane_load<g1a_t>(P, sl);
    mf_put_line(lds, wl, use, l00, fp2_mul_fp(theta, Pk.x), fp2_mul_fp(fp2_neg(delta), Pk.y));
  }
  const fp2_t C = fp2_sqr(theta);
  const fp2_t D = fp2_sqr(delta);
  const fp2_t E = fp2_mul(D, delta);
  const fp2_t F = fp2_mul(mf_get2(lds, tb + 4), C);
  const fp2_t G = fp2_mul(mf_get2(lds, tb), D);
  const fp2_t Hs = fp2_sub(fp2_add(E, F), fp2_add(G, G));
  mf_put2(lds, tb, fp2_mul(delta, Hs));
  const fp2_t Y3 = fp2_sub(fp2_mul(theta, fp2_sub(G, Hs)), fp2_mul(E, mf_get2(lds, tb + 2)));
  mf_put2(lds, tb + 2, Y3);
  mf_put2(lds, tb + 4, fp2_mul(E, mf_get2(lds, tb + 4)));
}

#ifndef LSG_MF_PRIO
#define LSG_MF_PRIO 2
#endif
#ifndef LSG_MF_WAVES
#define LSG_MF_WAVES 2
#endif
__global__ void __launch_bounds__(256) __attribute__((amdgpu_waves_per_eu(LSG_MF_WAVES)))
k_miller_fused(int n_items, const int32_t* __restrict__ item_first, const int32_t* __restrict__ item_cnt,
               const uint32_t* __restrict__ P, const uint8_t* __restrict__ pinf, const uint8_t* __restrict__ hinf,
               const int32_t* __restrict__ err, const uint32_t* __restrict__ H, uint32_t* __restrict__ f_out) {
  extern __shared__ uint32_t lds[];
#if LSG_MF_PRIO
  __builtin_amdgcn_s_setprio(LSG_MF_PRIO);
#endif
  const int w = __builtin_amdgcn_readfirstlane((int)(threadIdx.x >> 6));
  const size_t it = (size_t)blockIdx.x * MF_ITEMS + ((threadIdx.x & 63) >> 1);
  const bool live = it < (size_t)n_items;
  const size_t itc = live ? it : 0;
  const int first = item_first[itc], cnt = item_cnt[itc];
  const int si = first + (w < cnt ? w : cnt - 1);
  const uint64_t use_mask = __ballot(live && w < cnt && err[si] == 0 && !pinf[si] && !hinf[si]);
  {
    const g2p_t T = proj_from_aff(lane_load<g2a_t>(H, (size_t)si));
    mf_put2(lds, MF_T + 6 * w, T.X);
    mf_put2(lds, MF_T + 6 * w + 2, T.Y);
    mf_put2(lds, MF_T + 6 * w + 4, T.Z);
  }
  auto line_phase = [&](bool add) {
    int wl = w, sl = si;
    asm volatile("" : "+s"(wl), "+v"(sl));
#if LSG_MF_STAGED
    const bool use = (use_mask >> __lane_id()) & 1u;
    if (add)
      mf_add_line(lds, wl, use, P, H, (size_t)sl);
    else
      mf_dbl_line(lds, wl, use, P, (size_t)sl);
#else
    g2p_t T;
    T.X = mf_get2(lds, MF_T + 6 * wl);
    T.Y = mf_get2(lds, MF_T + 6 * wl + 2);
    T.Z = mf_get2(lds, MF_T + 6 * wl + 4);
    line_t L = add ? ml_add_step_raw(T, lane_load<g2a_t>(H, (size_t)sl)) : ml_dbl_step_raw(T);
    mf_put2(lds, MF_T + 6 * wl, T.X);
    mf_put2(lds, MF_T + 6 * wl + 2, T.Y);
    mf_put2(lds, MF_T + 6 * wl + 4, T.Z);
    const g1a_t Pk = lane_load<g1a_t>(P, (size_t)sl);
    L = line_eval(L, Pk.x, Pk.y);
    const bool use = (use_mask >> __lane_id()) & 1u;
    mf_put2(lds, MF_LC(wl, 0), fp2_select(use, L.l00, fp2_one()));
    mf_put2(lds, MF_LC(wl, 1), fp2_select(use, L.l01, fp2_zero()));
    mf_put2(lds, MF_LC(wl, 2), fp2_select(use, L.l11, fp2_zero()));
#endif
    __syncthreads();
    mf_pair_lines(lds, wl);
#pragma unroll 1
    for (int k = 0; k < 2; k++) mf_mul_pair(lds, wl, k);
  };
  if (w < 2) {
    mf_put2(lds, MF_FC(3 * w), w == 0 ? fp2_one() : fp2_zero());
    mf_put2(lds, MF_FC(3 * w + 1), fp2_zero());
    mf_put2(lds, MF_FC(3 * w + 2), fp2_zero());
  }
  const uint64_t xa = ((uint64_t)LSG_X_ABS_HI << 32) | LSG_X_ABS_LO;
  line_phase(false);
  line_phase(true);
#pragma unroll 1
  for (int b = 61; b >= 0; b--) {
    mf_sqr(lds, w);
    line_phase(false);
    if ((xa >> b) & 1u) line_phase(true);
  }
  if (live) {
    uint32_t* o = f_out + it * (size_t)lsgl::W_F12 + pair_h();
#pragma unroll
    for (int j = 0; j < 3; j++) {
      const int c = 3 * w + j;
      fp_t v = mf_get(lds, MF_F + c);
// ... 38 lines not shown
```

### lodestar_amd/csrc/lsg_k_pk.hip

```cpp
#include "lsg_kcommon.hpp"
namespace {
#include "lsg_inv.hpp"
}

LSG_DEVI int pk_fetch_aff(size_t item, const uint8_t* __restrict__ pk, uint32_t stride, const uint32_t* __restrict__ pk_len,
                          const uint32_t* __restrict__ tab, const uint8_t* __restrict__ tab_ok, uint32_t tab_n,
                          g1a_t& a, bool& is_inf) {
  const uint32_t len = pk_len[item];
  is_inf = true;
  if (len == LSG_PK_INDEX) {
    const uint8_t* b = pk + (size_t)stride * item;
    const uint32_t idx = (uint32_t)b[0] | ((uint32_t)b[1] << 8) | ((uint32_t)b[2] << 16) | ((uint32_t)b[3] << 24);
    const uint8_t ok = idx < tab_n ? tab_ok[idx] : 0;
    a = lane_load<g1a_t>(tab + (size_t)(ok == 1 ? idx : 0) * lsgl::W_TAB, 0);
    is_inf = ok != 1;
    return ok ? 0 : LSG_ERR_BAD_INDEX;
  }
  a.x = fp_zero();
  a.y = fp_zero();
  bool inf = false;
  const int e = (len == 48 || len == 96) ? g1_deserialize(a, inf, pk + (size_t)stride * item, (int)len) : LSG_BLST_INVALID_SIZE;
  is_inf = e != 0 || inf;
  return e;
}
// ... 279 lines not shown

__global__ void LSG_KERNEL_ATTR k_pk_keyvalidate(int n, const int32_t* __restrict__ keys, const uint8_t* __restrict__ pk,
                                                 const uint32_t* __restrict__ pk_len, int32_t* __restrict__ code) {
  LANE_ITEM(n);
  const size_t key = (size_t)keys[item];
  g1p_t p;
  const int e = g1_key_validate(pk + 96 * key, pk_len[key], p);
  if (lead) code[item] = e;
}

__global__ void __launch_bounds__(64) k_pk_keyvalidate_apply(int n, const int32_t* __restrict__ sets,
                                                             const int32_t* __restrict__ code,
                                                             int32_t* __restrict__ set_err) {
  const size_t j = gtid();
  if (j >= (size_t)n) return;
  const int32_t e = code[j];
  if (e == 0) return;
  const int32_t set = sets[j];
  for (size_t k = j; k > 0 && sets[k - 1] == set; k--)
    if (code[k - 1] != 0) return;
  set_err[set] = e;
}

__global__ void LSG_KERNEL_ATTR k_pk_scale(int n, const uint32_t* __restrict__ agg, const uint64_t* __restrict__ rnd,
                                           uint32_t* __restrict__ Pp, uint32_t* __restrict__ zP,
                                           uint8_t* __restrict__ pinf) {
  LANE_ITEM(n);
  g1p_t acc = lane_load<g1p_t>(agg, item);
  uint64_t r = rnd[item];
  bool is_inf = proj_is_inf(acc);
  if (r != 0 && !is_inf) acc = proj_mul_u64_s3(acc, r);
  lane_store(Pp, item, acc);
  lane_store(zP, item, is_inf ? fp_zero() : acc.Z);
  if (lead) pinf[item] = is_inf ? 1 : 0;
}

__global__ void LSG_KERNEL_ATTR k_pk_affine(int n, const uint32_t* __restrict__ Pp, const uint32_t* __restrict__ zinv,
                                            uint32_t* __restrict__ P) {
  LANE_ITEM(n);
  (void)lead;
  g1p_t p = lane_load<g1p_t>(Pp, item);
  fp_t zi = lane_load<fp_t>(zinv, item);
  g1a_t a;
  fp_mul2(a.x, a.y, p.X, zi, p.Y, zi);
  lane_store(P, item, a);
}

__global__ void LSG_KERNEL_ATTR k_pk_mask(int n, const uint32_t* __restrict__ Pp, const int32_t* __restrict__ err,
                                          const uint8_t* __restrict__ pinf, uint32_t* __restrict__ out) {
  LANE_ITEM(n);
  (void)lead;
  g1p_t p = proj_inf<fp_t>();
  if (err[item] == 0 && !pinf[item]) p = lane_load<g1p_t>(Pp, item);
  lane_store(out, item, p);
}
__global__ void LSG_KERNEL_ATTR k_g1p_affine_inv(int n, const uint32_t* __restrict__ Pp, uint32_t* __restrict__ P,
                                                 uint8_t* __restrict__ pinf) {
  LANE_ITEM(n);
  const g1p_t p = lane_load<g1p_t>(Pp, item);
  const bool is_inf = proj_is_inf(p);
  const fp_t d = pair_inv_gcd(pair_canon(is_inf ? fp_one() : p.Z));
  const fp_t zi = pair_mont_mul(d, fp_t(FP_RCUBE));
  g1a_t a;
  fp_mul2(a.x, a.y, p.X, zi, p.Y, zi);
  lane_store(P, item, a);
  if (lead) pinf[item] = is_inf ? 1 : 0;
}

__global__ void LSG_KERNEL_ATTR k_g1p_to_bytes(int n, const uint32_t* __restrict__ pts, uint8_t* __restrict__ out) {
  LANE_ITEM(n);
  (void)lead;
  g1p_t p = lane_load<g1p_t>(pts, item);
  bool is_inf = proj_is_inf(p);
  g1a_t a;
  if (is_inf) {
    a.x = fp_zero();
    a.y = fp_zero();
  } else {
    a = proj_to_aff(p);
  }
  g1_serialize(out + 96 * item, a, is_inf);
}

__global__ void LSG_KERNEL_ATTR k_sk_to_pk(int n, const uint8_t* __restrict__ sks, uint8_t* __restrict__ out96) {
  LANE_ITEM(n);
  (void)lead;
  g1a_t g;
  g.x = fp_t(G1_GEN_X);
  g.y = fp_t(G1_GEN_Y);
  const g1p_t base = proj_from_aff(g);
  g1p_t acc = proj_inf<fp_t>();
  const uint8_t* k = sks + 32 * item;
  for (int byte = 0; byte < 32; byte++) {
    uint32_t v = k[byte];
    for (int b = 7; b >= 0; b--) {
      acc = g1_dbl(acc);
      g1p_t s = g1_add(acc, base);
      bool bit = (v >> b) & 1u;
      acc.X = fp_select(bit, s.X, acc.X);
      acc.Y = fp_select(bit, s.Y, acc.Y);
      acc.Z = fp_select(bit, s.Z, acc.Z);
    }
  }
  bool is_inf = proj_is_inf(acc);
  g1a_t a;
  if (is_inf) {
    a.x = fp_zero();
    a.y = fp_zero();
  } else {
    a = proj_to_aff(acc);
  }
  g1_serialize(out96 + 96 * item, a, is_inf);
}

namespace lsgk {
hipError_t pk_decode(hipStream_t st, int n, const uint8_t* pk, uint32_t stride, const uint32_t* pk_len, uint32_t* pts,
                     int32_t* err, const uint32_t* tab, const uint8_t* tab_ok, uint32_t tab_n) {
  LSG_LAUNCH_ITEMS(k_pk_decode, n, st, n, pk, stride, pk_len, pts, err, tab, tab_ok, tab_n);
}
hipError_t pk_gather_aff(hipStream_t st, int n, const uint8_t* pk, uint32_t stride, const uint32_t* pk_len, uint32_t* pts,
                         uint8_t* inf, int32_t* err, const uint32_t* tab, const uint8_t* tab_ok, uint32_t tab_n) {
  LSG_LAUNCH_ITEMS(k_pk_gather_aff, n, st, n, pk, stride, pk_len, pts, inf, err, tab, tab_ok, tab_n);
}
hipError_t pk_agg_seg(hipStream_t st, int n_chunks, int ips_log2, const int32_t* chunks, const uint8_t* pk, uint32_t stride,
                      const uint32_t* pk_len, int32_t* err, const uint32_t* tab, const uint8_t* tab_ok, uint32_t tab_n,
                      uint32_t* dst, uint32_t* tmp) {
  LSG_LAUNCH_ITEMS(k_pk_agg_seg, (size_t)n_chunks << ips_log2, st, n_chunks, ips_log2, chunks, pk, stride, pk_len, err,
                   tab, tab_ok, tab_n, dst, tmp);
}
hipError_t agg_leaf(hipStream_t st, const AggTreeArgs& a) {
  if (a.L <= 0) return hipSuccess;
  hipLaunchKernelGGL(k_agg_leaf, dim3((unsigned)(a.n_c0 / LSG_ITEMS_PER_BLOCK)), dim3(LSG_TPB), 0, st, a);
  return hipGetLastError();
}
hipError_t agg_step(hipStream_t st, const AggTreeArgs& a, int t) {
  hipLaunchKernelGGL(k_agg_step, dim3((unsigned)((a.n_c0 >> t) / LSG_ITEMS_PER_BLOCK)), dim3(LSG_TPB), 0, st, a, t);
  return hipGetLastError();
}
hipError_t agg_final(hipStream_t st, const AggTreeArgs& a, int n_sets, const int32_t* src, uint32_t* agg) {
  LSG_LAUNCH_ITEMS(k_agg_final, n_sets, st, a, n_sets, src, agg);
}
hipError_t pk_validate(hipStream_t st, int n, const uint8_t* pk, uint32_t len, uint32_t* pts, int32_t* err) {
  LSG_LAUNCH_ITEMS(k_pk_validate, n, st, n, pk, len, pts, err);
}
hipError_t pk_keyvalidate(hipStream_t st, int n, const int32_t* keys, const uint8_t* pk, const uint32_t* pk_len,
                          int32_t* code) {
  LSG_LAUNCH_ITEMS(k_pk_keyvalidate, n, st, n, keys, pk, pk_len, code);
}
hipError_t pk_keyvalidate_apply(hipStream_t st, int n, const int32_t* sets, const int32_t* code, int32_t* set_err) {
  if (n <= 0) return hipSuccess;
  hipLaunchKernelGGL(k_pk_keyvalidate_apply, dim3((n + 63) / 64), dim3(64), 0, st, n, sets, code, set_err);
  return hipGetLastError();
}
hipError_t pk_scale(hipStream_t st, int n, const uint32_t* agg, const uint64_t* rnd, uint32_t* Pp, uint32_t* zP,
                    uint8_t* pinf) {
  LSG_LAUNCH_ITEMS(k_pk_scale, n, st, n, agg, rnd, Pp, zP, pinf);
}
hipError_t pk_affine(hipStream_t st, int n, const uint32_t* Pp, const uint32_t* zinv, uint32_t* P) {
  LSG_LAUNCH_ITEMS(k_pk_affine, n, st, n, Pp, zinv, P);
}
hipError_t pk_mask(hipStream_t st, int n, const uint32_t* Pp, const int32_t* err, const uint8_t* pinf, uint32_t* out) {
  LSG_LAUNCH_ITEMS(k_pk_mask, n, st, n, Pp, err, pinf, out);
}
hipError_t g1p_affine_inv(hipStream_t st, int n, const uint32_t* Pp, uint32_t* P, uint8_t* pinf) {
  LSG_LAUNCH_ITEMS(k_g1p_affine_inv, n, st, n, Pp, P, pinf);
}
hipError_t g1p_to_bytes(hipStream_t st, int n, const uint32_t* pts, uint8_t* out96) {
  LSG_LAUNCH_ITEMS(k_g1p_to_bytes, n, st, n, pts, out96);
}
hipError_t sk_to_pk(hipStream_t st, int n, const uint8_t* sks, uint8_t* out96) {
  LSG_LAUNCH_ITEMS(k_sk_to_pk, n, st, n, sks, out96);
}
}
```

### lodestar_amd/csrc/lsg_k_reduce.hip

```cpp
#include "lsg_kcommon.hpp"
namespace {
#include "lsg_inv.hpp"
}

template <int OP>
struct seg_op;
template <>
struct seg_op<0> {
  typedef g1p_t T;
  static LSG_DEVI T ident() { return proj_inf<fp_t>(); }
  static LSG_DEVI T op(const T& a, const T& b) { return g1_add(a, b); }
};
template <>
struct seg_op<1> {
  typedef g2p_t T;
  static LSG_DEVI T ident() { return proj_inf<fp2_t>(); }
  static LSG_DEVI T op(const T& a, const T& b) { return g2_add(a, b); }
};
template <>
struct seg_op<2> {
  typedef fp12_t T;
  static LSG_DEVI T ident() { return fp12_one(); }
  static LSG_DEVI T op(const T& a, const T& b) { return fp12_mul(a, b); }
};
// ... 62 lines not shown
  const int n_chunks = (n + LSG_BINV_T - 1) / LSG_BINV_T;
  LANE_ITEM(n_chunks);
  (void)lead;
  const fp_t one = fp_one();
  const int first = (int)item * LSG_BINV_T, last = min(n, first + LSG_BINV_T);
  fp_t acc = lane_load<fp_t>(tinv, item);
#pragma unroll 1
  for (int k = last - 1; k >= first; k--) {
    fp_t x = lane_load<fp_t>(in, k);
    const bool z = zero_to_one && fp_is_zero(x);
    fp_t r = k > first ? fp_mul(acc, lane_load<fp_t>(pre, k - 1)) : acc;
    lane_store(out, k, z ? fp_zero() : r);
    if (k > first && !z) acc = fp_mul(acc, x);
  }
}

__global__ void LSG_KERNEL_ATTR k_binv_block(int n, int T, int zero_to_one, const uint32_t* __restrict__ in,
                                             uint32_t* __restrict__ pre, uint32_t* __restrict__ out) {
  __shared__ uint32_t H[2 * LSG_ITEMS_PER_BLOCK * lsgl::W_FP], I[2 * LSG_ITEMS_PER_BLOCK * lsgl::W_FP];
  lsg_lane_setup();
#if LSG_RED_PRIO
  __builtin_amdgcn_s_setprio(LSG_RED_PRIO);
#endif
  const int l = (int)(threadIdx.x / LSG_GROUP);
  const int64_t first = ((int64_t)blockIdx.x * LSG_ITEMS_PER_BLOCK + l) * T;
  const int64_t last = first + T < (int64_t)n ? first + T : (int64_t)n;
  const fp_t one = fp_one();
  fp_t acc = one;
#pragma unroll 1
  for (int64_t k = first; k < last; k++) {
    fp_t x = lane_load<fp_t>(in, (size_t)k);
    if (zero_to_one) x = fp_select(fp_is_zero(x), one, x);
    acc = k == first ? x : fp_mul(acc, x);
    if (T > 1) lane_store(pre, (size_t)k, acc);
  }
  fp_t inv = block_inv<LSG_ITEMS_PER_BLOCK>(H, I, l, acc);
#pragma unroll 1
  for (int64_t k = last - 1; k >= first; k--) {
    const fp_t x = lane_load<fp_t>(in, (size_t)k);
    const bool z = zero_to_one && fp_is_zero(x);
    const fp_t r = k > first ? fp_mul(inv, lane_load<fp_t>(pre, (size_t)k - 1)) : inv;
    lane_store(out, (size_t)k, z ? fp_zero() : r);
    if (k > first && !z) inv = fp_mul(inv, x);
  }
}

__global__ void LSG_KERNEL_ATTR k_blobs_to_fp12(int n, const uint8_t* __restrict__ blobs, uint32_t* __restrict__ out) {
  LANE_ITEM(n);
  (void)lead;
  lane_store(out, item, fp12_from_canon_bytes(blobs + 576 * item));
}
__global__ void LSG_KERNEL_ATTR k_fp12_to_canon(int n, const uint32_t* __restrict__ in, uint8_t* __restrict__ out) {
  LANE_ITEM(n);
  (void)lead;
  fp12_to_canon_bytes(out + 576 * item, lane_load<fp12_t>(in, item));
}

__global__ void LSG_KERNEL_ATTR_W(1) k_fp12_pow_u64(const uint8_t* __restrict__ in576, uint64_t r,
                                                    uint8_t* __restrict__ out576) {
  LANE_ITEM(1);
  (void)lead;
  const fp12_t f = fp12_from_canon_bytes(in576);
  fp12_t acc = f;
  int top = 63;
  while (top > 0 && !((r >> top) & 1u)) top--;
#pragma unroll 1
  for (int b = top - 1; b >= 0; b--) {
    acc = fp12_sqr(acc);
    if ((r >> b) & 1u) acc = fp12_mul(acc, f);
  }
  fp12_to_canon_bytes(out576, acc);
}

__global__ void LSG_KERNEL_ATTR k_check_fp2_mul(int n, const uint32_t* __restrict__ in, uint32_t* __restrict__ out) {
  LANE_ITEM(n);
  (void)lead;
  const fp2_t a(lane_load<fp_t>(in, 4 * item), lane_load<fp_t>(in, 4 * item + 1));
  const fp2_t b(lane_load<fp_t>(in, 4 * item + 2), lane_load<fp_t>(in, 4 * item + 3));
  const fp2_t c = fp2_mul(a, b);
  lane_store(out, 2 * item, c.c0);
  lane_store(out, 2 * item + 1, c.c1);
}

__global__ void LSG_KERNEL_ATTR k_probe_fp_mul(int n, int iters, uint32_t* __restrict__ io) {
  LANE_ITEM(n);
  (void)lead;
  fp_t a = lane_load<fp_t>(io, item), b = fp_t(FP_R2), c = fp_t(FP_R3), d = fp_t(FP_HALF);
  for (int k = 0; k < iters; k++) {
    a = fp_mul(a, b);
    b = fp_mul(b, c);
    c = fp_mul(c, d);
    d = fp_mul(d, a);
  }
  lane_store(io, item, fp_add(fp_add(a, b), fp_add(c, d)));
}

__global__ void __launch_bounds__(256) k_probe_mad(int iters, uint32_t seed, uint64_t* __restrict__ io) {
  const uint32_t t = blockIdx.x * blockDim.x + threadIdx.x;
  uint64_t acc[16];
  uint32_t x[16];
#pragma unroll
  for (int k = 0; k < 16; k++) {
    acc[k] = t + k;
    x[k] = (t * 2654435761u) ^ (seed + 977u * k);
  }
  const uint32_t y = seed | 1u;
  for (int i = 0; i < iters; i++) {
#pragma unroll
    for (int k = 0; k < 16; k++) acc[k] = (uint64_t)x[k] * y + acc[k];
  }
  uint64_t r = 0;
#pragma unroll
  for (int k = 0; k < 16; k++) r ^= acc[k];
  io[t] = r;
}

namespace lsgk {
hipError_t seg_reduce(hipStream_t st, int op, int n_chunks, int ips_log2, const int32_t* chunks, const int32_t* idx,
                      const uint32_t* src, uint32_t* dst, uint32_t* tmp) {
  const size_t items = (size_t)n_chunks << ips_log2;
  if (op == 0) LSG_LAUNCH_ITEMS(k_seg_reduce<0>, items, st, n_chunks, ips_log2, chunks, idx, src, dst, tmp);
  if (op == 1) LSG_LAUNCH_ITEMS(k_seg_reduce<1>, items, st, n_chunks, ips_log2, chunks, idx, src, dst, tmp);
  LSG_LAUNCH_ITEMS(k_seg_reduce<2>, items, st, n_chunks, ips_log2, chunks, idx, src, dst, tmp);
}
hipError_t binv_fold(hipStream_t st, int n, int zero_to_one, const uint32_t* in, uint32_t* pre, uint32_t* tot) {
  LSG_LAUNCH_ITEMS(k_binv_fold, (n + LSG_BINV_T - 1) / LSG_BINV_T, st, n, zero_to_one, in, pre, tot);
}
hipError_t binv_block(hipStream_t st, int n, int T, int zero_to_one, const uint32_t* in, uint32_t* pre, uint32_t* out) {
  if (n <= 0) return hipSuccess;
  const size_t chunks = ((size_t)n + T - 1) / T;
  hipLaunchKernelGGL(k_binv_block, dim3(lane_blocks(chunks)), dim3(LSG_TPB), 0, st, n, T, zero_to_one, in, pre, out);
  return hipGetLastError();
}
hipError_t binv_root(hipStream_t st, const uint32_t* top, uint32_t* inv) {
  LSG_LAUNCH_ITEMS(k_binv_root, 1, st, top, inv);
}
hipError_t binv_unfold(hipStream_t st, int n, int zero_to_one, const uint32_t* in, const uint32_t* pre,
                       const uint32_t* tinv, uint32_t* out) {
  LSG_LAUNCH_ITEMS(k_binv_unfold, (n + LSG_BINV_T - 1) / LSG_BINV_T, st, n, zero_to_one, in, pre, tinv, out);
}
hipError_t blobs_to_fp12(hipStream_t st, int n, const uint8_t* blobs, uint32_t* out) {
  LSG_LAUNCH_ITEMS(k_blobs_to_fp12, n, st, n, blobs, out);
}
hipError_t fp12_to_canon(hipStream_t st, int n, const uint32_t* in, uint8_t* out576) {
  LSG_LAUNCH_ITEMS(k_fp12_to_canon, n, st, n, in, out576);
}
hipError_t fp12_pow_u64(hipStream_t st, const uint8_t* in576, uint64_t r, uint8_t* out576) {
  LSG_LAUNCH_ITEMS(k_fp12_pow_u64, 1, st, in576, r, out576);
}
hipError_t check_fp2_mul(hipStream_t st, int n, const uint32_t* in, uint32_t* out) {
  LSG_LAUNCH_ITEMS(k_check_fp2_mul, n, st, n, in, out);
}
hipError_t probe_fp_mul(hipStream_t st, int items, int iters, uint32_t* io) {
  LSG_LAUNCH_ITEMS(k_probe_fp_mul, items, st, items, iters, io);
}
hipError_t probe_mad(hipStream_t st, int blocks, int iters, uint32_t seed, uint64_t* io) {
  if (blocks <= 0) return hipSuccess;
  hipLaunchKernelGGL(k_probe_mad, dim3(blocks), dim3(256), 0, st, iters, seed, io);
  return hipGetLastError();
}
}
```

### lodestar_amd/csrc/lsg_k_sig.hip

```cpp
#include "lsg_kcommon.hpp"

__global__ void LSG_KERNEL_ATTR k_sig_decode(int n, const uint8_t* __restrict__ sig, const uint32_t* __restrict__ sig_len,
                                             uint32_t* __restrict__ sig_aff, uint8_t* __restrict__ inf,
                                             int32_t* __restrict__ err) {
  LANE_ITEM(n);
  uint32_t len = sig_len[item];
  g2a_t p;
  p.x = fp2_zero();
  p.y = fp2_zero();
  bool is_inf = false;
  int e;
  if (len == 96)
    e = g2_uncompress(p, is_inf, sig + 192 * item);
  else if (len == 192)
    e = g2_deserialize_uncompressed(p, is_inf, sig + 192 * item);
  else
    e = LSG_BLST_INVALID_SIZE;
  lane_store(sig_aff, item, p);
  if (lead) {
    inf[item] = is_inf ? 1 : 0;
    err[item] = e;
  }
}

__global__ void LSG_KERNEL_ATTR k_sig_subgroup(int n, const uint32_t* __restrict__ sig_aff,
                                               const uint8_t* __restrict__ inf, int32_t* __restrict__ err) {
  __shared__ uint32_t park[sizeof(g2a_t) / 4 * LSG_TPB];
  LANE_ITEM(n);
  if (err[item] != 0 || inf[item]) return;
  lds_park(park, lane_load<g2a_t>(sig_aff, item));
  bool ok = g2_in_group_get([&]() { return proj_from_aff(lds_unpark<g2a_t>(park)); });
  if (lead && !ok) err[item] = LSG_BLST_POINT_NOT_IN_GROUP;
}

LSG_DEVI bool sig_usable(size_t i, const uint8_t* inf, const int32_t* err, const uint8_t* pinf) {
  return err[i] == 0 && !inf[i] && !(pinf && pinf[i]);
}
__global__ void LSG_KERNEL_ATTR k_sig_proj(int n, const uint32_t* __restrict__ sig_aff, const uint8_t* __restrict__ inf,
                                           const int32_t* __restrict__ err, const uint8_t* __restrict__ pinf,
                                           uint32_t* __restrict__ out) {
  LANE_ITEM(n);
  (void)lead;
  g2p_t r = proj_inf<fp2_t>();
  if (sig_usable(item, inf, err, pinf)) r = proj_from_aff(lane_load<g2a_t>(sig_aff, item));
  lane_store(out, item, r);
}
__global__ void LSG_KERNEL_ATTR_W(1) k_sig_scale3(int n, const uint32_t* __restrict__ sig_aff, const uint8_t* __restrict__ inf,
                                                  const int32_t* __restrict__ err, const uint8_t* __restrict__ pinf,
                                                  const uint64_t* __restrict__ rnd, const uint8_t* __restrict__ mode,
                                                  uint32_t* __restrict__ out) {
  LANE_ITEM(n);
  (void)lead;
  if (mode && !mode[item]) return;
  g2p_t r = proj_inf<fp2_t>();
  if (sig_usable(item, inf, err, pinf)) {
    r = proj_from_aff(lane_load<g2a_t>(sig_aff, item));
    if (rnd[item] != 0) r = proj_mul_u64_s3(r, rnd[item]);
  }
  lane_store(out, item, r);
}

__global__ void LSG_KERNEL_ATTR k_g2a_to_bytes(int n, const uint32_t* __restrict__ pts, const uint8_t* __restrict__ inf,
                                               uint8_t* __restrict__ out) {
  LANE_ITEM(n);
  (void)lead;
  g2_serialize(out + 192 * item, lane_load<g2a_t>(pts, item), inf[item] != 0);
}

__global__ void LSG_KERNEL_ATTR k_g2p_compress(int n, const uint32_t* __restrict__ pts, uint8_t* __restrict__ out96) {
  LANE_ITEM(n);
  (void)lead;
  g2p_t p = lane_load<g2p_t>(pts, item);
  bool is_inf = proj_is_inf(p);
  g2a_t a;
  if (is_inf) {
    a.x = fp2_zero();
    a.y = fp2_zero();
  } else {
    a = proj_to_aff(p);
  }
  g2_compress(out96 + 96 * item, a, is_inf);
}

__global__ void LSG_KERNEL_ATTR k_g2p_to_canon(int n, const uint32_t* __restrict__ in, uint8_t* __restrict__ out) {
  LANE_ITEM(n);
  (void)lead;
  g2p_to_canon_bytes(out + 288 * item, lane_load<g2p_t>(in, item));
}

template <class F>
__device__ proj_t<F> proj_mul_be256(const proj_t<F>& p, const uint8_t* k) {
  proj_t<F> acc = proj_inf<F>();
  for (int byte = 0; byte < 32; byte++) {
    uint32_t v = k[byte];
    for (int b = 7; b >= 0; b--) {
      acc = gdbl(acc);
      proj_t<F> s = gadd(acc, p);
      bool bit = (v >> b) & 1u;
      acc.X = fselect(bit, s.X, acc.X);
      acc.Y = fselect(bit, s.Y, acc.Y);
      acc.Z = fselect(bit, s.Z, acc.Z);
    }
  }
  return acc;
}

__global__ void LSG_KERNEL_ATTR k_sign(int n, const uint8_t* __restrict__ sks, const uint32_t* __restrict__ H,
                                       uint8_t* __restrict__ out96) {
  LANE_ITEM(n);
  (void)lead;
  g2p_t s = proj_mul_be256(proj_from_aff(lane_load<g2a_t>(H, item)), sks + 32 * item);
  bool is_inf = proj_is_inf(s);
  g2a_t a;
  if (is_inf) {
// ... 44 lines not shown
```

### lodestar_amd/csrc/lsg_launch.h

```cpp
#pragma once
#include <hip/hip_runtime.h>
#include <stddef.h>
#include <stdint.h>

namespace lsgk {
hipError_t expand_msg(hipStream_t st, int n, const uint8_t* msg, const uint32_t* off, const uint32_t* len,
                      const uint8_t* dst, uint32_t dst_len, uint8_t* ub);
hipError_t h2c_prep(hipStream_t st, int n, const uint8_t* ub, uint32_t* U, uint32_t* norms);
hipError_t h2c_map(hipStream_t st, int n, const uint32_t* U, const uint32_t* ninv, uint32_t* Hp);
hipError_t h2c_clear(hipStream_t st, int n, uint32_t* Hp, uint32_t* zN, uint8_t* hinf);
hipError_t h2c_gather(hipStream_t st, int n, const uint32_t* mid, const uint32_t* Hm, const uint8_t* hinfm, uint32_t* H,
                      uint8_t* hinf);
hipError_t h2c_affine(hipStream_t st, int n, const uint32_t* Hp, const uint32_t* ninv, const uint8_t* hinf,
                      uint32_t* H);
hipError_t signing_root(hipStream_t st, int n, const uint8_t* roots, const uint8_t* domains, uint32_t dstride,
                        uint8_t* out32);
hipError_t attestation_signing_root(hipStream_t st, int n, const uint8_t* data, const uint8_t* domains,
                                    uint32_t dstride, uint8_t* out32);
hipError_t deposit_signing_root(hipStream_t st, int n, const uint8_t* data, uint32_t stride, const uint8_t* domains,
                                uint32_t dstride, uint8_t* out32);

hipError_t sig_decode(hipStream_t st, int n, const uint8_t* sig, const uint32_t* sig_len, uint32_t* sig_aff,
                      uint8_t* inf, int32_t* err);
hipError_t sig_subgroup(hipStream_t st, int n, const uint32_t* sig_aff, const uint8_t* inf, int32_t* err);
hipError_t sig_prep(hipStream_t st, int n, const uint32_t* sig_aff, const uint8_t* inf, const int32_t* err,
                    const uint8_t* pinf, const uint64_t* rnd, const uint8_t* mode, uint32_t* out);
hipError_t sig_scale_only(hipStream_t st, int n, const uint32_t* sig_aff, const uint8_t* inf, const int32_t* err,
                          const uint8_t* pinf, const uint64_t* rnd, const uint8_t* mode, uint32_t* out);
hipError_t g2a_to_bytes(hipStream_t st, int n, const uint32_t* pts, const uint8_t* inf, uint8_t* out192);
hipError_t g2p_compress(hipStream_t st, int n, const uint32_t* pts, uint8_t* out96);
hipError_t g2p_to_canon(hipStream_t st, int n, const uint32_t* pts, uint8_t* out288);
hipError_t sign(hipStream_t st, int n, const uint8_t* sks, const uint32_t* H, uint8_t* out96);

hipError_t pk_decode(hipStream_t st, int n, const uint8_t* pk, uint32_t stride, const uint32_t* pk_len, uint32_t* pts,
                     int32_t* err, const uint32_t* tab, const uint8_t* tab_ok, uint32_t tab_n);
hipError_t pk_validate(hipStream_t st, int n, const uint8_t* pk, uint32_t len, uint32_t* pts, int32_t* err);
hipError_t pk_keyvalidate(hipStream_t st, int n, const int32_t* keys, const uint8_t* pk, const uint32_t* pk_len,
                          int32_t* code);
hipError_t pk_keyvalidate_apply(hipStream_t st, int n, const int32_t* sets, const int32_t* code, int32_t* set_err);
hipError_t pk_gather_aff(hipStream_t st, int n, const uint8_t* pk, uint32_t stride, const uint32_t* pk_len, uint32_t* pts,
                         uint8_t* inf, int32_t* err, const uint32_t* tab, const uint8_t* tab_ok, uint32_t tab_n);
hipError_t pk_agg_seg(hipStream_t st, int n_chunks, int ips_log2, const int32_t* chunks, const uint8_t* pk, uint32_t stride,
                      const uint32_t* pk_len, int32_t* err, const uint32_t* tab, const uint8_t* tab_ok, uint32_t tab_n,
                      uint32_t* dst, uint32_t* tmp);
struct AggTreeArgs {
  int L = 0, T = 1;
  int64_t n_c0 = 0, N0 = 0;
  const int32_t* blk_set = nullptr;
  const int32_t* set_o0 = nullptr;
  const int32_t* set_len = nullptr;
  const int32_t* set_pk0 = nullptr;
  const uint8_t* pk = nullptr;
  uint32_t stride = 0;
  const uint32_t* pk_len = nullptr;
  int32_t* pk_err = nullptr;
  const uint32_t* tab = nullptr;
  const uint8_t* tab_ok = nullptr;
  uint32_t tab_n = 0;
  uint32_t* pts = nullptr;
  uint8_t* inf = nullptr;
  uint32_t* pre[2] = {nullptr, nullptr};
  uint32_t* cinv[2] = {nullptr, nullptr};
  uint8_t* flag[2] = {nullptr, nullptr};
};
hipError_t agg_leaf(hipStream_t st, const AggTreeArgs& a);
hipError_t agg_step(hipStream_t st, const AggTreeArgs& a, int t);
hipError_t agg_final(hipStream_t st, const AggTreeArgs& a, int n_sets, const int32_t* src, uint32_t* agg);
hipError_t pk_scale(hipStream_t st, int n, const uint32_t* agg, const uint64_t* rnd, uint32_t* Pp, uint32_t* zP,
                    uint8_t* pinf);
hipError_t pk_affine(hipStream_t st, int n, const uint32_t* Pp, const uint32_t* zinv, uint32_t* P);
hipError_t pk_mask(hipStream_t st, int n, const uint32_t* Pp, const int32_t* err, const uint8_t* pinf, uint32_t* out);
hipError_t g1p_affine_inv(hipStream_t st, int n, const uint32_t* Pp, uint32_t* P, uint8_t* pinf);
hipError_t g1p_to_bytes(hipStream_t st, int n, const uint32_t* pts, uint8_t* out96);
hipError_t sk_to_pk(hipStream_t st, int n, const uint8_t* sks, uint8_t* out96);

hipError_t miller_fused(hipStream_t st, int n_items, const int32_t* item_first, const int32_t* item_cnt,
                        const uint32_t* P, const uint8_t* pinf, const uint8_t* hinf, const int32_t* err,
                        const uint32_t* H, uint32_t* f);
hipError_t miller_lines(hipStream_t st, int n, const uint32_t* H, uint32_t* lines);
hipError_t miller_lines_list(hipStream_t st, int n, const int32_t* list, const uint32_t* H, uint32_t* lines);
hipError_t miller_accum_list(hipStream_t st, int n, const int32_t* list, const uint32_t* P, const uint8_t* pinf,
                             const uint8_t* hinf, const int32_t* err, const uint32_t* lines, uint32_t* f);
hipError_t miller_accum(hipStream_t st, int K, int n_items, const int32_t* item_first, const int32_t* item_cnt,
                        const uint32_t* P, const uint8_t* pinf, const uint8_t* hinf, const int32_t* err, int n_sets,
                        const uint32_t* lines, uint32_t* f);

hipError_t seg_reduce(hipStream_t st, int op, int n_chunks, int ips_log2, const int32_t* chunks, const int32_t* idx,
                      const uint32_t* src, uint32_t* dst, uint32_t* tmp);
hipError_t binv_fold(hipStream_t st, int n, int zero_to_one, const uint32_t* in, uint32_t* pre, uint32_t* tot);
hipError_t binv_root(hipStream_t st, const uint32_t* top, uint32_t* inv);
hipError_t binv_block(hipStream_t st, int n, int T, int zero_to_one, const uint32_t* in, uint32_t* pre, uint32_t* out);
hipError_t binv_unfold(hipStream_t st, int n, int zero_to_one, const uint32_t* in, const uint32_t* pre,
                       const uint32_t* tinv, uint32_t* out);
hipError_t blobs_to_fp12(hipStream_t st, int n, const uint8_t* blobs, uint32_t* out);
hipError_t fp12_to_canon(hipStream_t st, int n, const uint32_t* in, uint8_t* out576);
hipError_t fp12_pow_u64(hipStream_t st, const uint8_t* in576, uint64_t r, uint8_t* out576);
hipError_t probe_fp_mul(hipStream_t st, int items, int iters, uint32_t* io);
hipError_t check_fp2_mul(hipStream_t st, int n, const uint32_t* in, uint32_t* out);
hipError_t probe_mad(hipStream_t st, int blocks, int iters, uint32_t seed, uint64_t* io);
}
```

### lodestar_amd/csrc/lsg_pairing.hpp

```cpp
#pragma once
#include "lsg_curve.hpp"

struct line_t {
  fp2_t l00, l01, l11;
};

LSG_BIGFN line_t ml_dbl_step_raw(g2p_t& T) {
  fp2_t t0 = fp2_sqr(T.Y);
  fp2_t t1 = fp2_mul(T.Y, T.Z);
  fp2_t t2 = fp2_mul_b3(fp2_sqr(T.Z));
  fp2_t XX = fp2_sqr(T.X);
  line_t L;
  L.l00 = fp2_sub(t2, t0);
  L.l01 = fp2_add(fp2_add(XX, XX), XX);
  L.l11 = fp2_neg(fp2_add(t1, t1));
  fp2_t Z3 = fp2_add(t0, t0);
  Z3 = fp2_add(Z3, Z3);
  Z3 = fp2_add(Z3, Z3);
  fp2_t X3 = fp2_mul(t2, Z3);
  fp2_t Y3 = fp2_add(t0, t2);
  Z3 = fp2_mul(t1, Z3);
  fp2_t u1 = fp2_add(t2, t2);
  fp2_t u2 = fp2_add(u1, t2);
  fp2_t s0 = fp2_sub(t0, u2);
  Y3 = fp2_mul(s0, Y3);
  Y3 = fp2_add(X3, Y3);
  fp2_t v1 = fp2_mul(T.X, T.Y);
  X3 = fp2_mul(s0, v1);
  X3 = fp2_add(X3, X3);
  T.X = X3;
  T.Y = Y3;
  T.Z = Z3;
  return L;
}

LSG_BIGFN line_t ml_add_step_raw(g2p_t& T, g2a_t Q) {
  fp2_t theta = fp2_sub(T.Y, fp2_mul(Q.y, T.Z));
  fp2_t delta = fp2_sub(T.X, fp2_mul(Q.x, T.Z));
  line_t L;
  L.l00 = fp2_sub(fp2_mul(delta, Q.y), fp2_mul(theta, Q.x));
  L.l01 = theta;
  L.l11 = fp2_neg(delta);
  fp2_t C = fp2_sqr(theta);
  fp2_t D = fp2_sqr(delta);
  fp2_t E = fp2_mul(D, delta);
  fp2_t F = fp2_mul(T.Z, C);
  fp2_t G = fp2_mul(T.X, D);
  fp2_t H = fp2_sub(fp2_add(E, F), fp2_add(G, G));
  fp2_t X3 = fp2_mul(delta, H);
  fp2_t Y3 = fp2_sub(fp2_mul(theta, fp2_sub(G, H)), fp2_mul(E, T.Y));
  fp2_t Z3 = fp2_mul(E, T.Z);
  T.X = X3;
  T.Y = Y3;
  T.Z = Z3;
  return L;
}

LSG_INL line_t line_eval(line_t L, const fp_t& xP, const fp_t& yP) {
  L.l01 = fp2_mul_fp(L.l01, xP);
  L.l11 = fp2_mul_fp(L.l11, yP);
  return L;
}

#ifdef LSG_ROW_SPLIT
LSG_INL line_t ml_dbl_step_rows(g2p_t& T, const fp_t& xP, const fp_t& yP) {
  fp_t x[16], y[16], z[16];
  kar_prep(x, y, 0, T.Y, T.Y);
  kar_prep(x, y, 3, T.Y, T.Z);
  kar_prep(x, y, 6, T.Z, T.Z);
  kar_prep(x, y, 9, T.X, T.X);
  kar_prep(x, y, 12, T.X, T.Y);
  fp_mul_list<15>(z, x, y);
  const fp2_t t0 = kar_fin(z, 0), t1 = kar_fin(z, 3), t2 = fp2_mul_b3(kar_fin(z, 6)), XX = kar_fin(z, 9),
              v1 = kar_fin(z, 12);
  line_t L;
  L.l00 = fp2_sub(t2, t0);
  const fp2_t l01 = fp2_add(fp2_add(XX, XX), XX), l11 = fp2_neg(fp2_add(t1, t1));
  const fp2_t z8 = fp2_dbl(fp2_dbl(fp2_dbl(t0)));
  const fp2_t y3 = fp2_add(t0, t2);
  const fp2_t s0 = fp2_sub(t0, fp2_add(fp2_add(t2, t2), t2));
  kar_prep(x, y, 0, t2, z8);
  kar_prep(x, y, 3, t1, z8);
  kar_prep(x, y, 6, s0, y3);
  kar_prep(x, y, 9, s0, v1);
  x[12] = l01.c0;
  y[12] = xP;
  x[13] = l01.c1;
  y[13] = xP;
  x[14] = l11.c0;
  y[14] = yP;
  x[15] = l11.c1;
  y[15] = yP;
  fp_mul_list<16>(z, x, y);
  const fp2_t X3 = kar_fin(z, 0);
  T.X = fp2_dbl(kar_fin(z, 9));
  T.Y = fp2_add(X3, kar_fin(z, 6));
  T.Z = kar_fin(z, 3);
  L.l01 = fp2_t(z[12], z[13]);
  L.l11 = fp2_t(z[14], z[15]);
  return L;
}
LSG_INL line_t ml_add_step_rows(g2p_t& T, const g2a_t& Q, const fp_t& xP, const fp_t& yP) {
  fp_t x[13], y[13], z[13];
  kar_prep(x, y, 0, Q.y, T.Z);
  kar_prep(x, y, 3, Q.x, T.Z);
  fp_mul_list<6>(z, x, y);
  const fp2_t theta = fp2_sub(T.Y, kar_fin(z, 0)), delta = fp2_sub(T.X, kar_fin(z, 3));
  kar_prep(x, y, 0, delta, Q.y);
  kar_prep(x, y, 3, theta, Q.x);
  kar_prep(x, y, 6, theta, theta);
  kar_prep(x, y, 9, delta, delta);
  fp_mul_list<12>(z, x, y);
  line_t L;
  L.l00 = fp2_sub(kar_fin(z, 0), kar_fin(z, 3));
  const fp2_t C = kar_fin(z, 6), D = kar_fin(z, 9), l11 = fp2_neg(delta);
  kar_prep(x, y, 0, D, delta);
  kar_prep(x, y, 3, T.Z, C);
  kar_prep(x, y, 6, T.X, D);
  x[9] = theta.c0;
  y[9] = xP;
  x[10] = theta.c1;
  y[10] = xP;
  x[11] = l11.c0;
  y[11] = yP;
  x[12] = l11.c1;
  y[12] = yP;
  fp_mul_list<13>(z, x, y);
  const fp2_t E = kar_fin(z, 0), F = kar_fin(z, 3), G = kar_fin(z, 6);
  L.l01 = fp2_t(z[9], z[10]);
  L.l11 = fp2_t(z[11], z[12]);
  const fp2_t H = fp2_sub(fp2_add(E, F), fp2_add(G, G));
  kar_prep(x, y, 0, delta, H);
  kar_prep(x, y, 3, theta, fp2_sub(G, H));
  kar_prep(x, y, 6, E, T.Y);
  kar_prep(x, y, 9, E, T.Z);
  fp_mul_list<12>(z, x, y);
  T.X = kar_fin(z, 0);
  T.Y = fp2_sub(kar_fin(z, 3), kar_fin(z, 6));
  T.Z = kar_fin(z, 9);
  return L;
}
LSG_INL line_t ml_dbl_step(g2p_t& T, fp_t xP, fp_t yP) { return ml_dbl_step_rows(T, xP, yP); }
LSG_INL line_t ml_add_step(g2p_t& T, g2a_t Q, fp_t xP, fp_t yP) { return ml_add_step_rows(T, Q, xP, yP); }
#else
// ... 147 lines not shown
```

### lodestar_amd/csrc/lsg_tower.hpp

```cpp
#pragma once

#ifndef LSG_BIGFN
#define LSG_BIGFN LSG_NOINL
#endif

LSG_INL fp_t fp_one() { return fp_t(FP_ONE); }
LSG_INL fp_t fp_dbl(const fp_t& a) { return fp_add(a, a); }
LSG_INL fp_t fp_sqr(const fp_t& a) { return fp_mul(a, a); }
LSG_INL fp_t fp_to_mont(const fp_t& a) { return fp_mul(a, fp_t(FP_R2)); }
LSG_INL fp_t fp_from_mont(const fp_t& a) { return fp_canonical(fp_mul(a, fp_t(FP_ONE_CANON))); }
LSG_INL fp_t fp_from_be48(const uint8_t* b) { return fp_from_be_bytes(b, 12); }

LSG_BIGFN fp_t fp_pow_fixed(fp_t a, const uint32_t* e) {
#ifdef LSG_POW_LEAF
  return pair_pow_fixed(a, e);
#else
  fp_t T[8];
  T[0] = a;
  const fp_t a2 = fp_sqr(a);
#pragma unroll
  for (int k = 1; k < 8; k++) T[k] = fp_mul(T[k - 1], a2);
  int i = 383;
  while (i >= 0 && !((e[i >> 5] >> (i & 31)) & 1u)) i--;
  fp_t r = fp_one();
  bool started = false;
  while (i >= 0) {
    if (!((e[i >> 5] >> (i & 31)) & 1u)) {
      r = fp_sqr(r);
      i--;
      continue;
    }
    int j = i - 3 < 0 ? 0 : i - 3;
    while (!((e[j >> 5] >> (j & 31)) & 1u)) j++;
    uint32_t v = 0;
    for (int t = i; t >= j; t--) v = (v << 1) | ((e[t >> 5] >> (t & 31)) & 1u);
    if (started)
      for (int t = i; t >= j; t--) r = fp_sqr(r);
    fp_t tv = T[0];
#pragma unroll
    for (int k = 1; k < 8; k++) tv = fp_select(v == (uint32_t)(2 * k + 1), T[k], tv);
    r = started ? fp_mul(r, tv) : tv;
    started = true;
    i = j - 1;
  }
  return r;
#endif
}

#ifndef LSG_POW_IDS
enum { LSG_POW_INV = 0, LSG_POW_SQRT = 1, LSG_POW_SQRT34 = 2 };
#endif
LSG_BIGFN fp_t fp_pow_id(fp_t a, int id) {
#ifdef LSG_POW_PLAN
  return pair_pow_plan(a, id);
#else
  return fp_pow_fixed(a, id == LSG_POW_INV ? LSG_EXP_P_MINUS_2
                         : id == LSG_POW_SQRT ? LSG_EXP_P_PLUS_1_DIV_4 : LSG_EXP_P_MINUS_3_DIV_4);
#endif
}

LSG_INL fp_t fp_inv(const fp_t& a) { return fp_pow_id(a, LSG_POW_INV); }

LSG_INL fp_t fp_mul12(const fp_t& a) {
  fp_t a2 = fp_dbl(a);
  fp_t a4 = fp_dbl(a2);
  fp_t a8 = fp_dbl(a4);
  return fp_add(a8, a4);
}

struct fp2_t {
  fp_t c0, c1;
  fp2_t() = default;
  LSG_INL fp2_t(const fp_t& a, const fp_t& b) : c0(a), c1(b) {}
  LSG_INL fp2_t(const fp2c_t& c) : c0(c.c0), c1(c.c1) {}
};
struct fp6_t {
  fp2_t c0, c1, c2;
};
struct fp12_t {
  fp6_t c0, c1;
};

LSG_INL fp2_t fp2_make(const fp_t& a, const fp_t& b) { return fp2_t(a, b); }
LSG_INL fp2_t fp2_zero() { return fp2_t(fp_zero(), fp_zero()); }
LSG_INL fp2_t fp2_one() { return fp2_t(fp_one(), fp_zero()); }
LSG_INL bool fp2_is_zero(const fp2_t& a) { return fp_is_zero(a.c0) && fp_is_zero(a.c1); }
LSG_INL bool fp2_eq(const fp2_t& a, const fp2_t& b) { return fp_eq(a.c0, b.c0) && fp_eq(a.c1, b.c1); }
LSG_INL fp2_t fp2_select(bool c, const fp2_t& a, const fp2_t& b) {
  return fp2_t(fp_select(c, a.c0, b.c0), fp_select(c, a.c1, b.c1));
}
LSG_INL fp2_t fp2_add(const fp2_t& a, const fp2_t& b) { return fp2_t(fp_add(a.c0, b.c0), fp_add(a.c1, b.c1)); }
LSG_INL fp2_t fp2_sub(const fp2_t& a, const fp2_t& b) { return fp2_t(fp_sub(a.c0, b.c0), fp_sub(a.c1, b.c1)); }
LSG_INL fp2_t fp2_dbl(const fp2_t& a) { return fp2_add(a, a); }
LSG_INL fp2_t fp2_neg(const fp2_t& a) { return fp2_t(fp_neg(a.c0), fp_neg(a.c1)); }
LSG_INL fp2_t fp2_conj(const fp2_t& a) { return fp2_t(a.c0, fp_neg(a.c1)); }

LSG_INL fp2_t fp2_mul(const fp2_t& a, const fp2_t& b) {
#ifdef LSG_FP2_LEAF
  const fp_duo d = pair_fp2_mul(a.c0, a.c1, b.c0, b.c1);
  return fp2_t(d.x, d.y);
#else
  fp_t t0, t1, t2;
  fp_mul3(t0, t1, t2, a.c0, b.c0, a.c1, b.c1, fp_add(a.c0, a.c1), fp_add(b.c0, b.c1));
  return fp2_t(fp_sub(t0, t1), fp_sub(fp_sub(t2, t0), t1));
#endif
}

LSG_INL fp2_t fp2_sqr(const fp2_t& a) {
#ifdef LSG_FP2_LEAF
  const fp_duo d = pair_fp2_sqr(a.c0, a.c1);
  return fp2_t(d.x, d.y);
#else
  fp_t t0, t1;
  fp_mul2(t0, t1, fp_add(a.c0, a.c1), fp_sub(a.c0, a.c1), a.c0, a.c1);
  return fp2_t(t0, fp_dbl(t1));
#endif
}

LSG_INL fp2_t fp2_mul_fp(const fp2_t& a, const fp_t& k) {
  fp_t r0, r1;
  fp_mul2(r0, r1, a.c0, k, a.c1, k);
  return fp2_t(r0, r1);
}

template <int N>
LSG_INL void fp_mul_list(fp_t* r, const fp_t* x, const fp_t* y) {
#ifdef LSG_ROW_SPLIT
#ifndef LSG_SPLIT_MIN
#define LSG_SPLIT_MIN 4
#endif
  if (N >= LSG_SPLIT_MIN) {
    fp_mul_list_rows<N>(r, x, y);
    return;
  }
#endif
#pragma unroll
  for (int g = 0; g + 9 <= N; g += 9) fp_mul9(r + g, x + g, y + g);
  constexpr int T = N % 9, B = N - T;
#pragma unroll
  for (int g = B; g + 3 <= N; g += 3) fp_mul3(r[g], r[g + 1], r[g + 2], x[g], y[g], x[g + 1], y[g + 1], x[g + 2], y[g + 2]);
  constexpr int B2 = B + (T / 3) * 3;
  if (N - B2 == 2) fp_mul2(r[B2], r[B2 + 1], x[B2], y[B2], x[B2 + 1], y[B2 + 1]);
  if (N - B2 == 1) r[B2] = fp_mul(x[B2], y[B2]);
}

template <int K>
LSG_INL void fp2_mul_n(fp2_t* r, const fp2_t* a, const fp2_t* b) {
  fp_t x[3 * K], y[3 * K], z[3 * K];
#pragma unroll
  for (int k = 0; k < K; k++) {
    x[3 * k] = a[k].c0;
    y[3 * k] = b[k].c0;
    x[3 * k + 1] = a[k].c1;
    y[3 * k + 1] = b[k].c1;
    x[3 * k + 2] = fp_add(a[k].c0, a[k].c1);
    y[3 * k + 2] = fp_add(b[k].c0, b[k].c1);
  }
  fp_mul_list<3 * K>(z, x, y);
#pragma unroll
  for (int k = 0; k < K; k++)
    r[k] = fp2_t(fp_sub(z[3 * k], z[3 * k + 1]), fp_sub(fp_sub(z[3 * k + 2], z[3 * k]), z[3 * k + 1]));
}

template <int K>
LSG_INL void fp2_sqr_n(fp2_t* r, const fp2_t* a) {
  fp_t x[2 * K], y[2 * K], z[2 * K];
#pragma unroll
  for (int k = 0; k < K; k++) {
    x[2 * k] = fp_add(a[k].c0, a[k].c1);
    y[2 * k] = fp_sub(a[k].c0, a[k].c1);
    x[2 * k + 1] = a[k].c0;
    y[2 * k + 1] = a[k].c1;
  }
  fp_mul_list<2 * K>(z, x, y);
#pragma unroll
  for (int k = 0; k < K; k++) r[k] = fp2_t(z[2 * k], fp_dbl(z[2 * k + 1]));
}

LSG_INL fp2_t fp2_mul_xi(const fp2_t& a) { return fp2_t(fp_sub(a.c0, a.c1), fp_add(a.c0, a.c1)); }

LSG_INL fp_t fp2_norm(const fp2_t& a) {
  fp_t s0, s1;
  fp_mul2(s0, s1, a.c0, a.c0, a.c1, a.c1);
  return fp_add(s0, s1);
}

LSG_INL fp2_t fp2_inv(const fp2_t& a) {
  fp_t ni = fp_inv(fp2_norm(a));
  return fp2_t(fp_mul(a.c0, ni), fp_neg(fp_mul(a.c1, ni)));
}

LSG_INL fp2_t fp2_mul_b3(const fp2_t& a) {
  fp2_t t = fp2_mul_xi(a);
  return fp2_t(fp_mul12(t.c0), fp_mul12(t.c1));
}

LSG_INL uint32_t fp2_sgn0(const fp2_t& a) {
  fp_t c0 = fp_from_mont(a.c0), c1 = fp_from_mont(a.c1);
  uint32_t sign0 = fp_canon_parity(c0);
  uint32_t zero0 = fp_is_zero(c0) ? 1u : 0u;
  uint32_t sign1 = fp_canon_parity(c1);
  return sign0 | (zero0 & sign1);
}

LSG_INL bool fp2_lexi_largest(const fp2_t& y) {
  fp_t c0 = fp_from_mont(y.c0), c1 = fp_from_mont(y.c1);
  return fp_is_zero(c1) ? fp_canon_gt_half(c0) : fp_canon_gt_half(c1);
}

LSG_INL fp_t fp2_norm_sqrt_candidate(const fp2_t& a, bool* is_sq) {
  fp_t n = fp2_norm(a);
  fp_t s = fp_pow_id(n, LSG_POW_SQRT);
  *is_sq = fp_eq(fp_sqr(s), n);
  return s;
}
LSG_BIGFN bool fp2_sqrt_with_norm_root(fp2_t& out, fp2_t a, fp_t s) {
  fp_t c = fp_mul(fp_add(a.c0, s), fp_t(FP_HALF));
  c = fp_select(fp_is_zero(c), a.c0, c);
  fp_t t = fp_pow_id(c, LSG_POW_SQRT34);
  fp_t ct = fp_mul(c, t);
  bool c_sq = fp_eq(fp_mul(ct, t), fp_one()) || fp_is_zero(c);
  fp_t h = fp_mul(fp_mul(a.c1, t), fp_t(FP_HALF));
  fp2_t r = c_sq ? fp2_t(ct, h) : fp2_t(h, fp_neg(ct));
  out = r;
  return fp2_eq(fp2_sqr(r), a);
}
LSG_BIGFN bool fp2_sqrt(fp2_t& out, fp2_t a) {
  bool ok;
  fp_t s = fp2_norm_sqrt_candidate(a, &ok);
  bool r = fp2_sqrt_with_norm_root(out, a, s);
  return ok && r;
}

LSG_INL fp6_t fp6_make(const fp2_t& a, const fp2_t& b, const fp2_t& c) {
  fp6_t r;
  r.c0 = a;
  r.c1 = b;
  r.c2 = c;
  return r;
}
LSG_INL fp6_t fp6_zero() { return fp6_make(fp2_zero(), fp2_zero(), fp2_zero()); }
LSG_INL fp6_t fp6_one() { return fp6_make(fp2_one(), fp2_zero(), fp2_zero()); }
LSG_INL fp6_t fp6_add(const fp6_t& a, const fp6_t& b) {
  return fp6_make(fp2_add(a.c0, b.c0), fp2_add(a.c1, b.c1), fp2_add(a.c2, b.c2));
}
LSG_INL fp6_t fp6_sub(const fp6_t& a, const fp6_t& b) {
  return fp6_make(fp2_sub(a.c0, b.c0), fp2_sub(a.c1, b.c1), fp2_sub(a.c2, b.c2));
}
LSG_INL fp6_t fp6_neg(const fp6_t& a) { return fp6_make(fp2_neg(a.c0), fp2_neg(a.c1), fp2_neg(a.c2)); }

LSG_INL void fp6_mul_prep(fp2_t* A, fp2_t* B, const fp6_t& a, const fp6_t& b) {
  A[0] = a.c0;
  B[0] = b.c0;
  A[1] = a.c1;
  B[1] = b.c1;
  A[2] = a.c2;
  B[2] = b.c2;
  A[3] = fp2_add(a.c1, a.c2);
  B[3] = fp2_add(b.c1, b.c2);
  A[4] = fp2_add(a.c0, a.c1);
  B[4] = fp2_add(b.c0, b.c1);
  A[5] = fp2_add(a.c0, a.c2);
  B[5] = fp2_add(b.c0, b.c2);
}
LSG_INL fp6_t fp6_mul_fin(const fp2_t* V) {
  fp2_t c0 = fp2_add(V[0], fp2_mul_xi(fp2_sub(fp2_sub(V[3], V[1]), V[2])));
  fp2_t c1 = fp2_add(fp2_sub(fp2_sub(V[4], V[0]), V[1]), fp2_mul_xi(V[2]));
  fp2_t c2 = fp2_add(fp2_sub(fp2_sub(V[5], V[0]), V[2]), V[1]);
  fp6_t r;
  r.c0 = c0;
  r.c1 = c1;
  r.c2 = c2;
  return r;
}
#ifdef LSG_LEAN_TOWER
LSG_BIGFN fp6_t fp6_mul(fp6_t a, fp6_t b) {
  fp2_t v0 = fp2_mul(a.c0, b.c0);
  fp2_t v1 = fp2_mul(a.c1, b.c1);
  fp2_t v2 = fp2_mul(a.c2, b.c2);
  fp2_t c0 = fp2_add(v0, fp2_mul_xi(fp2_sub(fp2_sub(fp2_mul(fp2_add(a.c1, a.c2), fp2_add(b.c1, b.c2)), v1), v2)));
  fp2_t c1 = fp2_add(fp2_sub(fp2_sub(fp2_mul(fp2_add(a.c0, a.c1), fp2_add(b.c0, b.c1)), v0), v1), fp2_mul_xi(v2));
  fp2_t c2 = fp2_add(fp2_sub(fp2_sub(fp2_mul(fp2_add(a.c0, a.c2), fp2_add(b.c0, b.c2)), v0), v2), v1);
  return fp6_make(c0, c1, c2);
}
#else
LSG_BIGFN fp6_t fp6_mul(fp6_t a, fp6_t b) {
  fp2_t A[6], B[6], V[6];
  fp6_mul_prep(A, B, a, b);
  fp2_mul_n<6>(V, A, B);
  return fp6_mul_fin(V);
}
#endif

LSG_INL fp6_t fp6_mul_v(const fp6_t& a) { return fp6_make(fp2_mul_xi(a.c2), a.c0, a.c1); }

LSG_BIGFN fp6_t fp6_mul_01(fp6_t a, fp2_t b0, fp2_t b1) {
  fp2_t t0 = fp2_mul(a.c0, b0);
  fp2_t t1 = fp2_mul(a.c1, b1);
  fp2_t c0 = fp2_add(fp2_mul_xi(fp2_mul(a.c2, b1)), t0);
  fp2_t c1 = fp2_sub(fp2_sub(fp2_mul(fp2_add(a.c0, a.c1), fp2_add(b0, b1)), t0), t1);
  fp2_t c2 = fp2_add(fp2_mul(a.c2, b0), t1);
  return fp6_make(c0, c1, c2);
}

LSG_INL fp6_t fp6_mul_1(const fp6_t& a, const fp2_t& b1) {
  return fp6_make(fp2_mul_xi(fp2_mul(a.c2, b1)), fp2_mul(a.c0, b1), fp2_mul(a.c1, b1));
}

LSG_BIGFN fp6_t fp6_inv(fp6_t a) {
  fp2_t t0 = fp2_sub(fp2_sqr(a.c0), fp2_mul_xi(fp2_mul(a.c1, a.c2)));
  fp2_t t1 = fp2_sub(fp2_mul_xi(fp2_sqr(a.c2)), fp2_mul(a.c0, a.c1));
  fp2_t t2 = fp2_sub(fp2_sqr(a.c1), fp2_mul(a.c0, a.c2));
  fp2_t den = fp2_add(fp2_mul(a.c0, t0), fp2_mul_xi(fp2_add(fp2_mul(a.c2, t1), fp2_mul(a.c1, t2))));
  fp2_t di = fp2_inv(den);
  return fp6_make(fp2_mul(t0, di), fp2_mul(t1, di), fp2_mul(t2, di));
}

LSG_INL fp12_t fp12_make(const fp6_t& a, const fp6_t& b) {
  fp12_t r;
  r.c0 = a;
  r.c1 = b;
  return r;
}
LSG_INL fp12_t fp12_one() { return fp12_make(fp6_one(), fp6_zero()); }
LSG_INL bool fp12_is_one(const fp12_t& a) {
  return fp2_eq(a.c0.c0, fp2_one()) && fp2_is_zero(a.c0.c1) && fp2_is_zero(a.c0.c2) && fp2_is_zero(a.c1.c0) &&
         fp2_is_zero(a.c1.c1) && fp2_is_zero(a.c1.c2);
}
LSG_INL fp12_t fp12_conj(const fp12_t& a) { return fp12_make(a.c0, fp6_neg(a.c1)); }

#ifdef LSG_LEAN_TOWER
LSG_BIGFN fp12_t fp12_mul(fp12_t a, fp12_t b) {
  fp6_t t0 = fp6_mul(a.c0, b.c0);
  fp6_t t1 = fp6_mul(a.c1, b.c1);
  fp6_t t2 = fp6_mul(fp6_add(a.c0, a.c1), fp6_add(b.c0, b.c1));
  return fp12_make(fp6_add(t0, fp6_mul_v(t1)), fp6_sub(fp6_sub(t2, t0), t1));
}
LSG_BIGFN fp12_t fp12_sqr(fp12_t a) {
  fp6_t t = fp6_mul(a.c0, a.c1);
  fp6_t u = fp6_mul(fp6_add(a.c0, a.c1), fp6_add(a.c0, fp6_mul_v(a.c1)));
  return fp12_make(fp6_sub(fp6_sub(u, t), fp6_mul_v(t)), fp6_add(t, t));
}
#else
LSG_BIGFN fp12_t fp12_mul(fp12_t a, fp12_t b) {
  fp2_t A[18], B[18], V[18];
  fp6_mul_prep(A, B, a.c0, b.c0);
  fp6_mul_prep(A + 6, B + 6, a.c1, b.c1);
  fp6_mul_prep(A + 12, B + 12, fp6_add(a.c0, a.c1), fp6_add(b.c0, b.c1));
  fp2_mul_n<18>(V, A, B);
  fp6_t t0 = fp6_mul_fin(V), t1 = fp6_mul_fin(V + 6), t2 = fp6_mul_fin(V + 12);
  return fp12_make(fp6_add(t0, fp6_mul_v(t1)), fp6_sub(fp6_sub(t2, t0), t1));
}

LSG_BIGFN fp12_t fp12_sqr(fp12_t a) {
  fp2_t A[12], B[12], V[12];
  fp6_mul_prep(A, B, a.c0, a.c1);
  fp6_mul_prep(A + 6, B + 6, fp6_add(a.c0, a.c1), fp6_add(a.c0, fp6_mul_v(a.c1)));
  fp2_mul_n<12>(V, A, B);
  fp6_t t = fp6_mul_fin(V), u = fp6_mul_fin(V + 6);
  return fp12_make(fp6_sub(fp6_sub(u, t), fp6_mul_v(t)), fp6_add(t, t));
}
#endif

LSG_INL void fp4_square(fp2_t& c0, fp2_t& c1, const fp2_t& a, const fp2_t& b) {
  fp2_t t0 = fp2_sqr(a);
  fp2_t t1 = fp2_sqr(b);
  c0 = fp2_add(fp2_mul_xi(t1), t0);
  c1 = fp2_sub(fp2_sub(fp2_sqr(fp2_add(a, b)), t0), t1);
}

LSG_BIGFN fp12_t fp12_cyclotomic_sqr(fp12_t f) {
  fp2_t z0 = f.c0.c0, z4 = f.c0.c1, z3 = f.c0.c2, z2 = f.c1.c0, z1 = f.c1.c1, z5 = f.c1.c2;
#ifdef LSG_LEAN_TOWER
  fp2_t t0, t1, u0, u1, t2, t3;
  fp4_square(t0, t1, z0, z1);
  fp4_square(u0, u1, z2, z3);
  fp4_square(t2, t3, z4, z5);
#else
  fp2_t S[9], Q[9];
  S[0] = z0;
  S[1] = z1;
  S[2] = fp2_add(z0, z1);
  S[3] = z2;
  S[4] = z3;
  S[5] = fp2_add(z2, z3);
  S[6] = z4;
  S[7] = z5;
  S[8] = fp2_add(z4, z5);
  fp2_sqr_n<9>(Q, S);
  fp2_t t0 = fp2_add(fp2_mul_xi(Q[1]), Q[0]);
  fp2_t t1 = fp2_sub(fp2_sub(Q[2], Q[0]), Q[1]);
  fp2_t u0 = fp2_add(fp2_mul_xi(Q[4]), Q[3]);
  fp2_t u1 = fp2_sub(fp2_sub(Q[5], Q[3]), Q[4]);
  fp2_t t2 = fp2_add(fp2_mul_xi(Q[7]), Q[6]);
  fp2_t t3 = fp2_sub(fp2_sub(Q[8], Q[6]), Q[7]);
#endif
  z0 = fp2_sub(t0, z0);
  z0 = fp2_add(fp2_add(z0, z0), t0);
  z1 = fp2_add(t1, z1);
  z1 = fp2_add(fp2_add(z1, z1), t1);
  t0 = u0;
  t1 = u1;
  z4 = fp2_sub(t0, z4);
  z4 = fp2_add(fp2_add(z4, z4), t0);
  z5 = fp2_add(t1, z5);
  z5 = fp2_add(fp2_add(z5, z5), t1);
  t0 = fp2_mul_xi(t3);
  z2 = fp2_add(t0, z2);
  z2 = fp2_add(fp2_add(z2, z2), t0);
  z3 = fp2_sub(t2, z3);
  z3 = fp2_add(fp2_add(z3, z3), t2);
#ifdef LSG_PAIR_MODE
  fp2_t* zs[6] = {&z0, &z1, &z2, &z3, &z4, &z5};
  for (int k = 0; k < 6; k++) *zs[k] = fp2_t(fp_tame(zs[k]->c0), fp_tame(zs[k]->c1));
#endif
  return fp12_make(fp6_make(z0, z4, z3), fp6_make(z2, z1, z5));
}

LSG_BIGFN fp12_t fp12_mul_line(fp12_t f, fp2_t l00, fp2_t l01, fp2_t l11) {
#ifdef LSG_LEAN_TOWER
  fp6_t t0 = fp6_mul_01(f.c0, l00, l01);
  fp6_t u = fp6_mul_01(fp6_add(f.c0, f.c1), l00, fp2_add(l01, l11));
  fp6_t t1 = fp6_mul_1(f.c1, l11);
  return fp12_make(fp6_add(t0, fp6_mul_v(t1)), fp6_sub(fp6_sub(u, t0), t1));
#else
  const fp6_t& a = f.c0;
  const fp6_t& c = f.c1;
  fp6_t s = fp6_add(f.c0, f.c1);
  fp2_t m = fp2_add(l01, l11);
  fp2_t A[13], B[13], V[13];
  A[0] = a.c0; B[0] = l00;
  A[1] = a.c1; B[1] = l01;
  A[2] = a.c2; B[2] = l01;
  A[3] = fp2_add(a.c0, a.c1); B[3] = fp2_add(l00, l01);
  A[4] = a.c2; B[4] = l00;
  A[5] = s.c0; B[5] = l00;
  A[6] = s.c1; B[6] = m;
  A[7] = s.c2; B[7] = m;
  A[8] = fp2_add(s.c0, s.c1); B[8] = fp2_add(l00, m);
  A[9] = s.c2; B[9] = l00;
  A[10] = c.c2; B[10] = l11;
  A[11] = c.c0; B[11] = l11;
  A[12] = c.c1; B[12] = l11;
  fp2_mul_n<13>(V, A, B);
  fp6_t t0 = fp6_make(fp2_add(fp2_mul_xi(V[2]), V[0]), fp2_sub(fp2_sub(V[3], V[0]), V[1]), fp2_add(V[4], V[1]));
  fp6_t u = fp6_make(fp2_add(fp2_mul_xi(V[7]), V[5]), fp2_sub(fp2_sub(V[8], V[5]), V[6]), fp2_add(V[9], V[6]));
  fp6_t t1 = fp6_make(fp2_mul_xi(V[10]), V[11], V[12]);
  return fp12_make(fp6_add(t0, fp6_mul_v(t1)), fp6_sub(fp6_sub(u, t0), t1));
#endif
}

LSG_BIGFN fp12_t fp12_inv(fp12_t a) {
  fp6_t t = fp6_sub(fp6_mul(a.c0, a.c0), fp6_mul_v(fp6_mul(a.c1, a.c1)));
  fp6_t ti = fp6_inv(t);
  return fp12_make(fp6_mul(a.c0, ti), fp6_neg(fp6_mul(a.c1, ti)));
}

LSG_BIGFN fp12_t fp12_frob(fp12_t a) {
  fp12_t r;
  r.c0.c0 = fp2_conj(a.c0.c0);
  r.c1.c0 = fp2_mul(fp2_conj(a.c1.c0), FROB1_G1);
  r.c0.c1 = fp2_mul(fp2_conj(a.c0.c1), FROB1_G2);
  r.c1.c1 = fp2_mul(fp2_conj(a.c1.c1), FROB1_G3);
  r.c0.c2 = fp2_mul(fp2_conj(a.c0.c2), FROB1_G4);
  r.c1.c2 = fp2_mul(fp2_conj(a.c1.c2), FROB1_G5);
  return r;
}

LSG_BIGFN fp12_t fp12_frob2(fp12_t a) {
  fp12_t r;
  r.c0.c0 = a.c0.c0;
  r.c1.c0 = fp2_mul(a.c1.c0, FROB2_G1);
  r.c0.c1 = fp2_mul(a.c0.c1, FROB2_G2);
  r.c1.c1 = fp2_mul(a.c1.c1, FROB2_G3);
  r.c0.c2 = fp2_mul(a.c0.c2, FROB2_G4);
  r.c1.c2 = fp2_mul(a.c1.c2, FROB2_G5);
  return r;
}
```

Baseline: 3.396 million.

## Add lazy-carry field accumulators and Jacobian formulas for scalar multiplication

```diff
diff --git a/include/lodestar_bls.h b/include/lodestar_bls.h
--- a/include/lodestar_bls.h
+++ b/include/lodestar_bls.h
@@ -141,6 +141,8 @@
 int lsg_sk_to_pk(lsg_ctx* ctx, const uint8_t* sks32, size_t n, uint8_t* out96);
 
 int lsg_check_fp2_mul(lsg_ctx* ctx, const uint32_t* in, size_t n, uint32_t* out);
+int lsg_check_fp_acc(lsg_ctx* ctx, const uint32_t* in, size_t n, uint32_t* out);
+int lsg_check_g1_scale(lsg_ctx* ctx, const uint8_t* in96, const uint64_t* k, size_t n, uint8_t* out96);
 int lsg_probe_fp_mul_rate(lsg_ctx* ctx, double* fp_mul_per_s, double* mad_per_s);
 
 int lsg_probe_mad_peak(lsg_ctx* ctx, double* mad_per_s);
diff --git a/lodestar_amd/_native.py b/lodestar_amd/_native.py
--- a/lodestar_amd/_native.py
+++ b/lodestar_amd/_native.py
@@ -92,7 +92,7 @@
     "lsg_pubkey_table_set", "lsg_pubkey_table_size", "lsg_pubkey_validate",
     "lsg_final_submit_groups", "lsg_final_wait_groups", "lsg_aggregate_signatures",
     "lsg_signing_roots", "lsg_attestation_signing_roots", "lsg_jobs_partial_device", "lsg_final_submit_device",
-    "lsg_set_coalesce", "lsg_aggregate_pubkeys_multi", "lsg_check_fp2_mul",
+    "lsg_set_coalesce", "lsg_aggregate_pubkeys_multi", "lsg_check_fp2_mul", "lsg_check_fp_acc", "lsg_check_g1_scale",
     "lsg_deposit_signing_roots", "lsg_verify_deposits",
 ]
 
@@ -155,6 +155,8 @@
         lib.lsg_pipeline_slots.argtypes = [vp, pi32]
         lib.lsg_set_coalesce.argtypes = [vp, u32, i32]
         lib.lsg_check_fp2_mul.argtypes = [vp, ctypes.c_char_p, sz, ctypes.c_char_p]
+        lib.lsg_check_fp_acc.argtypes = [vp, ctypes.c_char_p, sz, ctypes.c_char_p]
+        lib.lsg_check_g1_scale.argtypes = [vp, ctypes.c_char_p, ctypes.c_char_p, sz, ctypes.c_char_p]
         lib.lsg_probe_mad_peak.argtypes = [vp, ctypes.POINTER(ctypes.c_double)]
         for name in EXPORTS:
             if name != "lsg_last_error":
@@ -589,6 +591,23 @@
         self._check(self.lib.lsg_check_fp2_mul(self.h, src, n, out), "lsg_check_fp2_mul")
         return list(struct.unpack(f"<{28 * n}I", out.raw))
 
+    def check_fp_acc(self, words):
+        n = len(words) // 84
+        assert len(words) == 84 * n
+        out = ctypes.create_string_buffer(4 * 56 * n)
+        src = struct.pack(f"<{len(words)}I", *words)
+        self._check(self.lib.lsg_check_fp_acc(self.h, src, n, out), "lsg_check_fp_acc")
+        return list(struct.unpack(f"<{56 * n}I", out.raw))
+
+    def check_g1_scale(self, points96, scalars):
+        n = len(points96)
+        assert n == len(scalars) and all(len(p) == 96 for p in points96)
+        out = ctypes.create_string_buffer(96 * n)
+        self._check(self.lib.lsg_check_g1_scale(self.h, b"".join(points96), struct.pack(f"<{n}Q", *scalars), n, out),
+                    "lsg_check_g1_scale")
+        raw = out.raw
+        return [raw[96 * i:96 * i + 96] for i in range(n)]
+
     def probe_fp_mul_rate(self):
         a, b = ctypes.c_double(), ctypes.c_double()
         self._check(self.lib.lsg_probe_fp_mul_rate(self.h, ctypes.byref(a), ctypes.byref(b)), "lsg_probe_fp_mul_rate")
diff --git a/lodestar_amd/csrc/lsg_curve.hpp b/lodestar_amd/csrc/lsg_curve.hpp
--- a/lodestar_amd/csrc/lsg_curve.hpp
+++ b/lodestar_amd/csrc/lsg_curve.hpp
@@ -21,6 +21,8 @@
 LSG_INL fp2_t fselect(bool c, const fp2_t& a, const fp2_t& b) { return fp2_select(c, a, b); }
 LSG_INL fp_t finv(const fp_t& a) { return fp_inv(a); }
 LSG_INL fp2_t finv(const fp2_t& a) { return fp2_inv(a); }
+LSG_INL fp_acc_t<1, 0> facc(const fp_t& a) { return fp_acc(a); }
+LSG_INL fp2_acc_t<1, 0> facc(const fp2_t& a) { return fp2_acc(a); }
 template <class F> LSG_INL F fzero();
 template <> LSG_INL fp_t fzero<fp_t>() { return fp_zero(); }
 template <> LSG_INL fp2_t fzero<fp2_t>() { return fp2_zero(); }
@@ -77,16 +79,12 @@
   F t1 = fmul(p.Y, q.Y);
   F t2 = fmul(p.Z, q.Z);
   F t3 = fmul(fadd(p.X, p.Y), fadd(q.X, q.Y));
-  F t4 = fadd(t0, t1);
-  t3 = fsub(t3, t4);
-  t4 = fmul(fadd(p.Y, p.Z), fadd(q.Y, q.Z));
-  F X3 = fadd(t1, t2);
-  t4 = fsub(t4, X3);
-  X3 = fmul(fadd(p.X, p.Z), fadd(q.X, q.Z));
-  F Y3 = fadd(t0, t2);
-  Y3 = fsub(X3, Y3);
-  X3 = fadd(t0, t0);
-  t0 = fadd(X3, t0);
+  t3 = facc(t3).sub(t0).sub(t1).carry();
+  F t4 = fmul(fadd(p.Y, p.Z), fadd(q.Y, q.Z));
+  t4 = facc(t4).sub(t1).sub(t2).carry();
+  F X3 = fmul(fadd(p.X, p.Z), fadd(q.X, q.Z));
+  F Y3 = facc(X3).sub(t0).sub(t2).carry();
+  t0 = facc(t0).add(t0).add(t0).carry();
   t2 = fmul_b3(t2);
   F Z3 = fadd(t1, t2);
   t1 = fsub(t1, t2);
@@ -112,17 +110,15 @@
   F t0 = fmul(p.X, q.x);
   F t1 = fmul(p.Y, q.y);
   F t3 = fmul(fadd(q.x, q.y), fadd(p.X, p.Y));
-  F t4 = fadd(t0, t1);
-  t3 = fsub(t3, t4);
-  t4 = fadd(fmul(q.y, p.Z), p.Y);
+  t3 = facc(t3).sub(t0).sub(t1).carry();
+  F t4 = fadd(fmul(q.y, p.Z), p.Y);
   F Y3 = fadd(fmul(q.x, p.Z), p.X);
-  F X3 = fadd(t0, t0);
-  t0 = fadd(X3, t0);
+  t0 = facc(t0).add(t0).add(t0).carry();
   F t2 = fmul_b3(p.Z);
   F Z3 = fadd(t1, t2);
   t1 = fsub(t1, t2);
   Y3 = fmul_b3(Y3);
-  X3 = fmul(t4, Y3);
+  F X3 = fmul(t4, Y3);
   t2 = fmul(t3, t1);
   X3 = fsub(t2, X3);
   Y3 = fmul(Y3, t0);
@@ -149,9 +145,7 @@
   F X3 = fmul(t2, Z3);
   F Y3 = fadd(t0, t2);
   Z3 = fmul(t1, Z3);
-  t1 = fadd(t2, t2);
-  t2 = fadd(t1, t2);
-  t0 = fsub(t0, t2);
+  t0 = facc(t0).sub(t2).sub(t2).sub(t2).carry();
   Y3 = fmul(t0, Y3);
   Y3 = fadd(X3, Y3);
   t1 = fmul(p.X, p.Y);
@@ -277,16 +271,15 @@
   F A = fsqr(p.X);
   F B = fsqr(p.Y);
   F C = fsqr(B);
-  F D = fsub(fsqr(fadd(p.X, B)), fadd(A, C));
+  F D = facc(fsqr(fadd(p.X, B))).sub(A).sub(C).carry();
   D = fadd(D, D);
-  F E = fadd(fadd(A, A), A);
+  F E = facc(A).add(A).add(A).carry();
   F Fq = fsqr(E);
   jac_t<F> r;
-  r.X = fsub(Fq, fadd(D, D));
-  F C8 = fadd(C, C);
-  C8 = fadd(C8, C8);
-  C8 = fadd(C8, C8);
-  r.Y = fsub(fmul(E, fsub(D, r.X)), C8);
+  r.X = facc(Fq).sub(D).sub(D).carry();
+  F C4 = fadd(C, C);
+  C4 = fadd(C4, C4);
+  r.Y = facc(fmul(E, fsub(D, r.X))).sub(C4).sub(C4).carry();
   F yz = fmul(p.Y, p.Z);
   r.Z = fadd(yz, yz);
   return r;
@@ -297,6 +290,94 @@
 template <class F>
 LSG_INL jac_t<F> jac_add_proj(const jac_t<F>& acc, const proj_t<F>& q) {
   return jac_from_proj(gadd(jac_to_proj(acc), q));
+}
+
+LSG_INL bool lsg_any(bool b) {
+#if defined(__HIP_DEVICE_COMPILE__)
+  return __builtin_amdgcn_ballot_w64(b) != 0;
+#else
+  return b;
+#endif
+}
+#ifdef LSG_COUNT_JAC_FALLBACK
+extern unsigned long long lsg_jac_fallbacks;
+#define LSG_COUNT_FALLBACK() (lsg_jac_fallbacks++)
+#else
+#define LSG_COUNT_FALLBACK() ((void)0)
+#endif
+template <class F>
+LSG_INL jac_t<F> jac_select(bool c, const jac_t<F>& a, const jac_t<F>& b) {
+  jac_t<F> r;
+  r.X = fselect(c, a.X, b.X);
+  r.Y = fselect(c, a.Y, b.Y);
+  r.Z = fselect(c, a.Z, b.Z);
+  return r;
+}
+template <class F>
+LSG_INL jac_t<F> jac_from_aff(const aff_t<F>& a) {
+  jac_t<F> r;
+  r.X = a.x;
+  r.Y = a.y;
+  r.Z = fone<F>();
+  return r;
+}
+template <class F>
+LSG_INL jac_t<F> jac_add_mixed(const jac_t<F>& p, bool& p_inf, const aff_t<F>& q) {
+  F Z1Z1 = fsqr(p.Z);
+  F U2 = fmul(q.x, Z1Z1);
+  F S2 = fmul(fmul(q.y, p.Z), Z1Z1);
+  F H = fsub(U2, p.X);
+  F HH = fsqr(H);
+  F I = fadd(HH, HH);
+  I = fadd(I, I);
+  F J = fmul(H, I);
+  F rr = facc(S2).add(S2).sub(p.Y).sub(p.Y).carry();
+  F V = fmul(p.X, I);
+  jac_t<F> r;
+  r.X = facc(fsqr(rr)).sub(J).sub(V).sub(V).carry();
+  F YJ = fmul(p.Y, J);
+  r.Y = facc(fmul(rr, fsub(V, r.X))).sub(YJ).sub(YJ).carry();
+  r.Z = facc(fsqr(fadd(p.Z, H))).sub(Z1Z1).sub(HH).carry();
+  const bool exc = !p_inf && fis_zero(r.Z);
+  if (lsg_any(exc)) {
+    LSG_COUNT_FALLBACK();
+    r = jac_add_proj(p, proj_from_aff(q));
+    p_inf = fis_zero(r.Z);
+    return r;
+  }
+  r = jac_select(p_inf, jac_from_aff(q), r);
+  p_inf = false;
+  return r;
+}
+template <class F>
+LSG_INL jac_t<F> jac_add(const jac_t<F>& p, bool& p_inf, const jac_t<F>& q, bool q_inf) {
+  F Z1Z1 = fsqr(p.Z);
+  F Z2Z2 = fsqr(q.Z);
+  F U1 = fmul(p.X, Z2Z2);
+  F U2 = fmul(q.X, Z1Z1);
+  F S1 = fmul(fmul(p.Y, q.Z), Z2Z2);
+  F S2 = fmul(fmul(q.Y, p.Z), Z1Z1);
+  F H = fsub(U2, U1);
+  F I = fsqr(fadd(H, H));
+  F J = fmul(H, I);
+  F rr = facc(S2).add(S2).sub(S1).sub(S1).carry();
+  F V = fmul(U1, I);
+  jac_t<F> r;
+  r.X = facc(fsqr(rr)).sub(J).sub(V).sub(V).carry();
+  F SJ = fmul(S1, J);
+  r.Y = facc(fmul(rr, fsub(V, r.X))).sub(SJ).sub(SJ).carry();
+  r.Z = fmul(facc(fsqr(fadd(p.Z, q.Z))).sub(Z1Z1).sub(Z2Z2).carry(), H);
+  const bool exc = !p_inf && !q_inf && fis_zero(r.Z);
+  if (lsg_any(exc)) {
+    LSG_COUNT_FALLBACK();
+    r = jac_add_proj(p, jac_to_proj(q));
+    p_inf = fis_zero(r.Z);
+    return r;
+  }
+  r = jac_select(q_inf, p, r);
+  r = jac_select(p_inf, q, r);
+  p_inf = p_inf && q_inf;
+  return r;
 }
 
 template <class F>
@@ -321,27 +402,29 @@
 }
 
 template <class F>
-LSG_INL proj_t<F> proj_pick_signed(const proj_t<F>& T1, const proj_t<F>& T2, const proj_t<F>& T3,
-                                   const proj_t<F>& T4, int d) {
+LSG_INL jac_t<F> jac_pick_signed(const jac_t<F>& T1, const jac_t<F>& T2, const jac_t<F>& T3, const jac_t<F>& T4,
+                                 bool i1, bool i3, int d, bool* inf) {
   const int a = d < 0 ? -d : d;
-  proj_t<F> r = proj_inf<F>();
-  auto take = [&](bool s, const proj_t<F>& t) {
-    r.X = fselect(s, t.X, r.X);
-    r.Y = fselect(s, t.Y, r.Y);
-    r.Z = fselect(s, t.Z, r.Z);
-  };
-  take(a == 1, T1);
-  take(a == 2, T2);
-  take(a == 3, T3);
-  take(a == 4, T4);
+  jac_t<F> r;
+  r.X = fone<F>();
+  r.Y = fone<F>();
+  r.Z = fzero<F>();
+  r = jac_select(a == 1, T1, r);
+  r = jac_select(a == 2, T2, r);
+  r = jac_select(a == 3, T3, r);
+  r = jac_select(a == 4, T4, r);
   r.Y = fselect(d < 0, fneg(r.Y), r.Y);
+  *inf = a == 0 || (a == 3 ? i3 : i1);
   return r;
 }
 template <class F>
 LSG_INL proj_t<F> proj_mul_u64_s3(const proj_t<F>& p, uint64_t k) {
-  const proj_t<F> T2 = gdbl(p);
-  const proj_t<F> T3 = gadd(T2, p);
-  const proj_t<F> T4 = gdbl(T2);
+  const bool i1 = fis_zero(p.Z);
+  const jac_t<F> T1 = jac_from_proj(p);
+  const jac_t<F> T2 = jac_dbl(T1);
+  bool i3 = i1;
+  const jac_t<F> T3 = jac_add(T2, i3, T1, i1);
+  const jac_t<F> T4 = jac_dbl(T2);
   uint32_t cm = 0;
 #pragma unroll
   for (int i = 0; i < 21; i++) {
@@ -351,13 +434,16 @@
   auto digit = [&](int i) {
     return (int)((k >> (3 * i)) & 7u) + (int)((cm >> i) & 1u) - (i < 21 ? 8 * (int)((cm >> (i + 1)) & 1u) : 0);
   };
-  jac_t<F> acc = jac_from_proj(proj_pick_signed(p, T2, T3, T4, digit(21)));
+  bool acc_inf;
+  jac_t<F> acc = jac_pick_signed(T1, T2, T3, T4, i1, i3, digit(21), &acc_inf);
 #pragma unroll 1
   for (int i = 20; i >= 0; i--) {
     acc = jac_dbl(acc);
     acc = jac_dbl(acc);
     acc = jac_dbl(acc);
-    acc = jac_add_proj(acc, proj_pick_signed(p, T2, T3, T4, digit(i)));
+    bool q_inf;
+    const jac_t<F> q = jac_pick_signed(T1, T2, T3, T4, i1, i3, digit(i), &q_inf);
+    acc = jac_add(acc, acc_inf, q, q_inf);
   }
   return jac_to_proj(acc);
 }
@@ -373,6 +459,18 @@
   }
   return jac_to_proj(acc);
 }
+template <class F, class G>
+LSG_INL proj_t<F> proj_mul_xabs_aff_get(const G& geta) {
+  const uint64_t xa = ((uint64_t)LSG_X_ABS_HI << 32) | LSG_X_ABS_LO;
+  jac_t<F> acc = jac_from_aff(geta());
+  bool acc_inf = false;
+#pragma unroll 1
+  for (int b = 62; b >= 0; b--) {
+    acc = jac_dbl(acc);
+    if ((xa >> b) & 1u) acc = jac_add_mixed(acc, acc_inf, geta());
+  }
+  return jac_to_proj(acc);
+}
 template <class F>
 LSG_INL proj_t<F> proj_mul_xabs(const proj_t<F>& p) {
   return proj_mul_xabs_get<F>([&]() { return p; });
@@ -415,7 +513,19 @@
   g2p_t xp = proj_neg(proj_mul_xabs_get<fp2_t>(get));
   return proj_eq(g2_psi(get()), xp);
 }
+template <class G>
+LSG_INL bool g2_in_group_aff_get(const G& geta) {
+  g2p_t xp = proj_neg(proj_mul_xabs_aff_get<fp2_t>(geta));
+  return proj_eq(g2_psi(proj_from_aff(geta())), xp);
+}
 LSG_BIGFN bool g2_in_group(g2p_t p) {
+  if (proj_is_inf(p)) return true;
+  if (fp2_eq(p.Z, fp2_one())) {
+    g2a_t a;
+    a.x = p.X;
+    a.y = p.Y;
+    return g2_in_group_aff_get([&]() { return a; });
+  }
   return g2_in_group_get([&]() { return p; });
 }
 
diff --git a/lodestar_amd/csrc/lsg_fp_pair.hpp b/lodestar_amd/csrc/lsg_fp_pair.hpp
--- a/lodestar_amd/csrc/lsg_fp_pair.hpp
+++ b/lodestar_amd/csrc/lsg_fp_pair.hpp
@@ -417,6 +417,88 @@
   return pair_carry(r);
 }
 LSG_PFN fp_t fp_neg(const fp_t& a) { return fp_sub(fp_zero(), a); }
+
+#ifndef LSG_ACC_FOLD
+#define LSG_FP_ACC 1
+#if defined(LSG_ACC_CHECK) && LSG_PAIR_G == 1
+#define LSG_ACC_CHECKING 1
+extern unsigned long long lsg_acc_check_fail, lsg_acc_check_carries;
+#define LSG_ACC_W(x) (x).w
+#else
+#define LSG_ACC_W(x) nullptr
+#endif
+template <int P, int N>
+struct fp_acc_t {
+  static_assert(P >= 0 && N >= 0 && P <= 3 && N <= 3,
+                "fp_acc_t: at most 3 terms added and 3 subtracted between two carries (32-bit limbs)");
+  uint32_t l[LSG_PL];
+#ifdef LSG_ACC_CHECKING
+  int64_t w[LSG_PL];
+#endif
+  template <int S, int P2, int N2>
+  LSG_PFN fp_acc_t<P2, N2> with(const uint32_t* b, const int64_t* bw) const {
+    fp_acc_t<P2, N2> r;
+#pragma unroll
+    for (int k = 0; k < LSG_PL; k++) r.l[k] = S > 0 ? l[k] + b[k] : l[k] - b[k];
+#ifdef LSG_ACC_CHECKING
+    for (int k = 0; k < LSG_PL; k++) r.w[k] = w[k] + S * (bw ? bw[k] : (int64_t)(int32_t)b[k]);
+#else
+    (void)bw;
+#endif
+    return r;
+  }
+  LSG_PFN fp_acc_t<P + 1, N> add(const fp_t& b) const { return with<1, P + 1, N>(b.l, nullptr); }
+  LSG_PFN fp_acc_t<P, N + 1> sub(const fp_t& b) const { return with<-1, P, N + 1>(b.l, nullptr); }
+  template <int P2, int N2>
+  LSG_PFN fp_acc_t<P + P2, N + N2> add(const fp_acc_t<P2, N2>& b) const {
+    return with<1, P + P2, N + N2>(b.l, LSG_ACC_W(b));
+  }
+  template <int P2, int N2>
+  LSG_PFN fp_acc_t<P + N2, N + P2> sub(const fp_acc_t<P2, N2>& b) const {
+    return with<-1, P + N2, N + P2>(b.l, LSG_ACC_W(b));
+  }
+  template <int P2, int N2>
+  LSG_PFN fp_acc_t<P2, N2> widen() const {
+    static_assert(P2 >= P && N2 >= N, "fp_acc_t: widen() only raises the term counts");
+    fp_acc_t<P2, N2> r;
+#pragma unroll
+    for (int k = 0; k < LSG_PL; k++) r.l[k] = l[k];
+#ifdef LSG_ACC_CHECKING
+    for (int k = 0; k < LSG_PL; k++) r.w[k] = w[k];
+#endif
+    return r;
+  }
+  LSG_PFN fp_t carry() const {
+    fp_t r;
+#pragma unroll
+    for (int k = 0; k < LSG_PL; k++) r.l[k] = l[k];
+#ifdef LSG_ACC_CHECKING
+    lsg_acc_check_carries++;
+    for (int k = 0; k < LSG_PL; k++)
+      if ((int64_t)(int32_t)l[k] != w[k]) lsg_acc_check_fail++;
+#endif
+    return pair_carry(r);
+  }
+};
+LSG_PFN fp_acc_t<1, 0> fp_acc(const fp_t& a) {
+  fp_acc_t<1, 0> r;
+#pragma unroll
+  for (int k = 0; k < LSG_PL; k++) r.l[k] = a.l[k];
+#ifdef LSG_ACC_CHECKING
+  for (int k = 0; k < LSG_PL; k++) r.w[k] = (int64_t)(int32_t)a.l[k];
+#endif
+  return r;
+}
+LSG_PFN fp_acc_t<0, 1> fp_acc_neg(const fp_t& a) {
+  fp_acc_t<0, 1> r;
+#pragma unroll
+  for (int k = 0; k < LSG_PL; k++) r.l[k] = 0u - a.l[k];
+#ifdef LSG_ACC_CHECKING
+  for (int k = 0; k < LSG_PL; k++) r.w[k] = -(int64_t)(int32_t)a.l[k];
+#endif
+  return r;
+}
+#endif
 LSG_PFN fp_t fp_mul(const fp_t& a, const fp_t& b) { return pair_mont_mul(a, b); }
 #if LSG_LEAF_MODE == 0
 LSG_PFN void fp_mul2(fp_t& r0, fp_t& r1, const fp_t& a0, const fp_t& b0, const fp_t& a1, const fp_t& b1) {
diff --git a/lodestar_amd/csrc/lsg_host.hip b/lodestar_amd/csrc/lsg_host.hip
--- a/lodestar_amd/csrc/lsg_host.hip
+++ b/lodestar_amd/csrc/lsg_host.hip
@@ -3058,6 +3058,39 @@
   return LSG_OK;
 }
 
+int lsg_check_fp_acc(lsg_ctx* c, const uint32_t* in, size_t n, uint32_t* out) {
+  if (!c || (n && (!in || !out)) || n > 0x7fffffffull / (6 * W_FP)) return LSG_ERR_INVALID_ARG;
+  LSG_ENTER(c);
+  if (n == 0) return LSG_OK;
+  Slot* s = &c->dev[0]->util;
+  timer_reset(s);
+  LSG_RC(ensure(s, s->d_aux, 4 * 6 * W_FP * n));
+  LSG_RC(ensure(s, s->d_Fb, 4 * 4 * W_FP * n));
+  LSG_HIP(s, hipMemcpyAsync(s->d_aux.p, in, 4 * 6 * W_FP * n, hipMemcpyHostToDevice, s->st[0]));
+  KL(s, "k_check_fp_acc", lsgk::check_fp_acc(S_(s), (int)n, P_<uint32_t>(s->d_aux), P_<uint32_t>(s->d_Fb)));
+  LSG_HIP(s, hipMemcpyAsync(out, s->d_Fb.p, 4 * 4 * W_FP * n, hipMemcpyDeviceToHost, s->st[0]));
+  LSG_HIP(s, hipStreamSynchronize(s->st[0]));
+  return LSG_OK;
+}
+
+int lsg_check_g1_scale(lsg_ctx* c, const uint8_t* in96, const uint64_t* k, size_t n, uint8_t* out96) {
+  if (!c || (n && (!in96 || !k || !out96)) || n > 0x7fffffffull / 96) return LSG_ERR_INVALID_ARG;
+  LSG_ENTER(c);
+  if (n == 0) return LSG_OK;
+  Slot* s = &c->dev[0]->util;
+  timer_reset(s);
+  LSG_RC(ensure(s, s->d_aux, (96 + 8) * n));
+  LSG_RC(ensure(s, s->d_Fb, 96 * n));
+  uint8_t* d_in = P_<uint8_t>(s->d_aux);
+  LSG_HIP(s, hipMemcpyAsync(d_in, in96, 96 * n, hipMemcpyHostToDevice, s->st[0]));
+  LSG_HIP(s, hipMemcpyAsync(d_in + 96 * n, k, 8 * n, hipMemcpyHostToDevice, s->st[0]));
+  KL(s, "k_check_g1_scale",
+     lsgk::check_g1_scale(S_(s), (int)n, d_in, (const uint64_t*)(d_in + 96 * n), P_<uint8_t>(s->d_Fb)));
+  LSG_HIP(s, hipMemcpyAsync(out96, s->d_Fb.p, 96 * n, hipMemcpyDeviceToHost, s->st[0]));
+  LSG_HIP(s, hipStreamSynchronize(s->st[0]));
+  return LSG_OK;
+}
+
 int lsg_probe_fp_mul_rate(lsg_ctx* c, double* fp_mul_per_s, double* mad_per_s) {
   if (!c || !fp_mul_per_s || !mad_per_s) return LSG_ERR_INVALID_ARG;
   LSG_ENTER(c);
diff --git a/lodestar_amd/csrc/lsg_k_miller.hip b/lodestar_amd/csrc/lsg_k_miller.hip
--- a/lodestar_amd/csrc/lsg_k_miller.hip
+++ b/lodestar_amd/csrc/lsg_k_miller.hip
@@ -107,7 +107,7 @@
       y = b;
     } else {
       x = fp6_add(a, b);
-      y = fp6_add(a, fp6_mul_v(b));
+      y = fp6_add_mul_v(a, b);
     }
     fp2_t p0, p1, p2;
     if ((w & 1) == 0) {
@@ -124,30 +124,17 @@
     mf_put2(lds, MF_VC(3 * w + 2), p2);
   }
   __syncthreads();
-  auto fin = [&](int base, int j) {
-    const fp2_t v0 = mf_get2(lds, MF_VC(base)), v1 = mf_get2(lds, MF_VC(base + 1)), v2 = mf_get2(lds, MF_VC(base + 2));
-    if (j == 0) return fp2_add(v0, fp2_mul_xi(fp2_sub(fp2_sub(mf_get2(lds, MF_VC(base + 3)), v1), v2)));
-    if (j == 1) return fp2_add(fp2_sub(fp2_sub(mf_get2(lds, MF_VC(base + 4)), v0), v1), fp2_mul_xi(v2));
-    return fp2_add(fp2_sub(fp2_sub(mf_get2(lds, MF_VC(base + 5)), v0), v2), v1);
-  };
-  fp2_t o0, o1, o2;
+  auto V = [&](int p) { return mf_get2(lds, MF_VC(p)); };
   if (w == 0) {
-    o0 = fin(0, 0);
-    o1 = fin(0, 1);
-    o2 = fin(0, 2);
+    mf_put2(lds, MF_FC(3), fp12_sqr_coef<3>(V));
+    mf_put2(lds, MF_FC(4), fp12_sqr_coef<4>(V));
+    mf_put2(lds, MF_FC(5), fp12_sqr_coef<5>(V));
   } else if (w == 1) {
-    o0 = fp2_sub(fp2_sub(fin(6, 0), fin(0, 0)), fp2_mul_xi(fin(0, 2)));
+    mf_put2(lds, MF_FC(0), fp12_sqr_coef<0>(V));
   } else if (w == 2) {
-    o0 = fp2_sub(fp2_sub(fin(6, 1), fin(0, 1)), fin(0, 0));
+    mf_put2(lds, MF_FC(1), fp12_sqr_coef<1>(V));
   } else {
-    o0 = fp2_sub(fp2_sub(fin(6, 2), fin(0, 2)), fin(0, 1));
-  }
-  if (w == 0) {
-    mf_put2(lds, MF_FC(3), fp2_add(o0, o0));
-    mf_put2(lds, MF_FC(4), fp2_add(o1, o1));
-    mf_put2(lds, MF_FC(5), fp2_add(o2, o2));
-  } else {
-    mf_put2(lds, MF_FC(w - 1), o0);
+    mf_put2(lds, MF_FC(2), fp12_sqr_coef<2>(V));
   }
 }
 
@@ -169,14 +156,14 @@
     }
   }
   __syncthreads();
-  const fp2_t P0 = mf_get2(lds, MF_VC(6 * pi)), P1 = mf_get2(lds, MF_VC(6 * pi + 1)), P2 = mf_get2(lds, MF_VC(6 * pi + 2));
+  auto V = [&](int p) { return mf_get2(lds, MF_VC(6 * pi + p)); };
   if (h == 0) {
-    mf_put2(lds, MF_LC(2 * pi, 0), fp2_add(P0, fp2_mul_xi(P1)));
-    mf_put2(lds, MF_LC(2 * pi, 1), fp2_sub(fp2_sub(mf_get2(lds, MF_VC(6 * pi + 3)), P0), P2));
-    mf_put2(lds, MF_LC(2 * pi, 2), P2);
+    mf_put2(lds, MF_LC(2 * pi, 0), line_pair_coef<0>(V));
+    mf_put2(lds, MF_LC(2 * pi, 1), line_pair_coef<1>(V));
+    mf_put2(lds, MF_LC(2 * pi, 2), V(2));
   } else {
-    mf_put2(lds, MF_LC(2 * pi + 1, 0), fp2_sub(fp2_sub(mf_get2(lds, MF_VC(6 * pi + 4)), P0), P1));
-    mf_put2(lds, MF_LC(2 * pi + 1, 1), fp2_sub(fp2_sub(mf_get2(lds, MF_VC(6 * pi + 5)), P2), P1));
+    mf_put2(lds, MF_LC(2 * pi + 1, 0), line_pair_coef<2>(V));
+    mf_put2(lds, MF_LC(2 * pi + 1, 1), line_pair_coef<3>(V));
   }
   __syncthreads();
 }
@@ -209,54 +196,29 @@
       mf_put2(lds, MF_VC(12), fp2_mul(s1, fp2_add(m1, m4)));
     } else {
       const fp2_t m4 = mf_get2(lds, MF_LC(2 * k + 1, 0)), m5 = mf_get2(lds, MF_LC(2 * k + 1, 1));
-      const fp2_t s0 = fp2_add(mf_get2(lds, MF_FC(0)), mf_get2(lds, MF_FC(3)));
+      const fp2_t a0 = mf_get2(lds, MF_FC(0)), b0 = mf_get2(lds, MF_FC(3));
       const fp2_t s1 = fp2_add(mf_get2(lds, MF_FC(1)), mf_get2(lds, MF_FC(4)));
       const fp2_t s2 = fp2_add(mf_get2(lds, MF_FC(2)), mf_get2(lds, MF_FC(5)));
-      const fp2_t q1 = fp2_add(m1, m4), q2 = fp2_add(m2, m5);
+      const fp2_t q2 = fp2_add(m2, m5);
       mf_put2(lds, MF_VC(13), fp2_mul(s2, q2));
-      mf_put2(lds, MF_VC(14), fp2_mul(fp2_add(s0, s1), fp2_add(m0, q1)));
-      mf_put2(lds, MF_VC(15), fp2_mul(fp2_add(s1, s2), fp2_add(q1, q2)));
-      mf_put2(lds, MF_VC(16), fp2_mul(fp2_add(s0, s2), fp2_add(m0, q2)));
+      mf_put2(lds, MF_VC(14), fp2_mul(fp2_acc(a0).add(b0).add(s1).carry(), fp2_acc(m0).add(m1).add(m4).carry()));
+      mf_put2(lds, MF_VC(15), fp2_mul(fp2_add(s1, s2), fp2_acc(m1).add(m4).add(q2).carry()));
+      mf_put2(lds, MF_VC(16), fp2_mul(fp2_acc(a0).add(b0).add(s2).carry(), fp2_add(m0, q2)));
     }
   }
   __syncthreads();
   auto V = [&](int p) { return mf_get2(lds, MF_VC(p)); };
-  auto t0c = [&](int j) {
-    if (j == 0) return fp2_add(V(0), fp2_mul_xi(fp2_sub(fp2_sub(V(4), V(1)), V(2))));
-    if (j == 1) return fp2_add(fp2_sub(fp2_sub(V(3), V(0)), V(1)), fp2_mul_xi(V(2)));
-    return fp2_add(fp2_sub(fp2_sub(V(5), V(0)), V(2)), V(1));
-  };
-  auto t2c = [&](int j) {
-    if (j == 0) return fp2_add(V(11), fp2_mul_xi(fp2_sub(fp2_sub(V(15), V(12)), V(13))));
-    if (j == 1) return fp2_add(fp2_sub(fp2_sub(V(14), V(11)), V(12)), fp2_mul_xi(V(13)));
-    return fp2_add(fp2_sub(fp2_sub(V(16), V(11)), V(13)), V(12));
-  };
-  auto nc = [&](int j) {
-    if (j == 0) return fp2_add(V(6), fp2_mul_xi(V(10)));
-    if (j == 1) return fp2_sub(fp2_sub(V(8), V(6)), V(7));
-    return fp2_add(V(7), V(9));
-  };
-  fp2_t o0, o1;
-  int j0, j1 = -1;
   if (w == 0) {
-    o0 = fp2_add(t0c(0), fp2_mul_xi(nc(1)));
-    o1 = fp2_add(t0c(1), fp2_mul_xi(nc(2)));
-    j0 = 0;
-    j1 = 1;
+    mf_put2(lds, MF_FC(0), fp12_mul_pair_coef<0>(V));
+    mf_put2(lds, MF_FC(1), fp12_mul_pair_coef<1>(V));
   } else if (w == 1) {
-    o0 = fp2_add(t0c(2), nc(0));
-    o1 = fp2_sub(fp2_sub(t2c(0), t0c(0)), fp2_mul_xi(nc(2)));
-    j0 = 2;
-    j1 = 3;
+    mf_put2(lds, MF_FC(2), fp12_mul_pair_coef<2>(V));
+    mf_put2(lds, MF_FC(3), fp12_mul_pair_coef<3>(V));
   } else if (w == 2) {
-    o0 = fp2_sub(fp2_sub(t2c(1), t0c(1)), nc(0));
-    j0 = 4;
+    mf_put2(lds, MF_FC(4), fp12_mul_pair_coef<4>(V));
   } else {
-    o0 = fp2_sub(fp2_sub(t2c(2), t0c(2)), nc(1));
-    j0 = 5;
-  }
-  mf_put2(lds, MF_FC(j0), o0);
-  if (j1 >= 0) mf_put2(lds, MF_FC(j1), o1);
+    mf_put2(lds, MF_FC(5), fp12_mul_pair_coef<5>(V));
+  }
   __syncthreads();
 }
 
@@ -279,8 +241,8 @@
     const fp2_t XX = fp2_sqr(X);
     v1 = fp2_mul(X, Y);
     const g1a_t Pk = lane_load<g1a_t>(P, sl);
-    mf_put_line(lds, wl, use, fp2_sub(t2, t0), fp2_mul_fp(fp2_add(fp2_add(XX, XX), XX), Pk.x),
-                fp2_mul_fp(fp2_neg(fp2_add(t1, t1)), Pk.y));
+    mf_put_line(lds, wl, use, fp2_sub(t2, t0), fp2_mul_fp(fp2_acc(XX).add(XX).add(XX).carry(), Pk.x),
+                fp2_mul_fp(fp2_acc_neg(t1).sub(t1).carry(), Pk.y));
   }
   fp2_t Z3 = fp2_add(t0, t0);
   Z3 = fp2_add(Z3, Z3);
@@ -288,8 +250,7 @@
   fp2_t X3 = fp2_mul(t2, Z3);
   fp2_t Y3 = fp2_add(t0, t2);
   mf_put2(lds, tb + 4, fp2_mul(t1, Z3));
-  const fp2_t u2 = fp2_add(fp2_add(t2, t2), t2);
-  const fp2_t s0 = fp2_sub(t0, u2);
+  const fp2_t s0 = fp2_acc(t0).sub(t2).sub(t2).sub(t2).carry();
   Y3 = fp2_mul(s0, Y3);
   mf_put2(lds, tb + 2, fp2_add(X3, Y3));
   X3 = fp2_mul(s0, v1);
@@ -313,7 +274,7 @@
   const fp2_t E = fp2_mul(D, delta);
   const fp2_t F = fp2_mul(mf_get2(lds, tb + 4), C);
   const fp2_t G = fp2_mul(mf_get2(lds, tb), D);
-  const fp2_t Hs = fp2_sub(fp2_add(E, F), fp2_add(G, G));
+  const fp2_t Hs = fp2_acc(E).add(F).sub(G).sub(G).carry();
   mf_put2(lds, tb, fp2_mul(delta, Hs));
   const fp2_t Y3 = fp2_sub(fp2_mul(theta, fp2_sub(G, Hs)), fp2_mul(E, mf_get2(lds, tb + 2)));
   mf_put2(lds, tb + 2, Y3);
diff --git a/lodestar_amd/csrc/lsg_k_pk.hip b/lodestar_amd/csrc/lsg_k_pk.hip
--- a/lodestar_amd/csrc/lsg_k_pk.hip
+++ b/lodestar_amd/csrc/lsg_k_pk.hip
@@ -385,6 +385,25 @@
   g1_serialize(out + 96 * item, a, is_inf);
 }
 
+__global__ void LSG_KERNEL_ATTR k_check_g1_scale(int n, const uint8_t* __restrict__ in96, const uint64_t* __restrict__ k,
+                                                 uint8_t* __restrict__ out96) {
+  LANE_ITEM(n);
+  (void)lead;
+  g1a_t p;
+  bool inf;
+  (void)g1_deserialize(p, inf, in96 + 96 * item, 96);
+  const g1p_t r = proj_mul_u64_s3(inf ? proj_inf<fp_t>() : proj_from_aff(p), k[item]);
+  const bool is_inf = proj_is_inf(r);
+  g1a_t a;
+  if (is_inf) {
+    a.x = fp_zero();
+    a.y = fp_zero();
+  } else {
+    a = proj_to_aff(r);
+  }
+  g1_serialize(out96 + 96 * item, a, is_inf);
+}
+
 __global__ void LSG_KERNEL_ATTR k_sk_to_pk(int n, const uint8_t* __restrict__ sks, uint8_t* __restrict__ out96) {
   LANE_ITEM(n);
   (void)lead;
@@ -471,6 +490,9 @@
 hipError_t g1p_to_bytes(hipStream_t st, int n, const uint32_t* pts, uint8_t* out96) {
   LSG_LAUNCH_ITEMS(k_g1p_to_bytes, n, st, n, pts, out96);
 }
+hipError_t check_g1_scale(hipStream_t st, int n, const uint8_t* in96, const uint64_t* k, uint8_t* out96) {
+  LSG_LAUNCH_ITEMS(k_check_g1_scale, n, st, n, in96, k, out96);
+}
 hipError_t sk_to_pk(hipStream_t st, int n, const uint8_t* sks, uint8_t* out96) {
   LSG_LAUNCH_ITEMS(k_sk_to_pk, n, st, n, sks, out96);
 }
diff --git a/lodestar_amd/csrc/lsg_k_reduce.hip b/lodestar_amd/csrc/lsg_k_reduce.hip
--- a/lodestar_amd/csrc/lsg_k_reduce.hip
+++ b/lodestar_amd/csrc/lsg_k_reduce.hip
@@ -168,6 +168,19 @@
   lane_store(out, 2 * item + 1, c.c1);
 }
 
+__global__ void LSG_KERNEL_ATTR k_check_fp_acc(int n, const uint32_t* __restrict__ in, uint32_t* __restrict__ out) {
+  LANE_ITEM(n);
+  (void)lead;
+  fp_t v[6];
+#pragma unroll
+  for (int k = 0; k < 6; k++) v[k] = lane_load<fp_t>(in, 6 * item + k);
+  lane_store(out, 4 * item, fp_acc(v[0]).add(v[1]).add(v[2]).sub(v[3]).sub(v[4]).sub(v[5]).carry());
+  const fp2_t x = fp2_acc(fp2_t(v[0], v[1])).add(fp2_acc(fp2_t(v[2], v[3])).mul_xi()).sub(fp2_t(v[4], v[5])).carry();
+  lane_store(out, 4 * item + 1, x.c0);
+  lane_store(out, 4 * item + 2, x.c1);
+  lane_store(out, 4 * item + 3, fp_acc_neg(v[0]).sub(v[1]).add(v[2]).carry());
+}
+
 __global__ void LSG_KERNEL_ATTR k_probe_fp_mul(int n, int iters, uint32_t* __restrict__ io) {
   LANE_ITEM(n);
   (void)lead;
@@ -237,6 +250,9 @@
 hipError_t check_fp2_mul(hipStream_t st, int n, const uint32_t* in, uint32_t* out) {
   LSG_LAUNCH_ITEMS(k_check_fp2_mul, n, st, n, in, out);
 }
+hipError_t check_fp_acc(hipStream_t st, int n, const uint32_t* in, uint32_t* out) {
+  LSG_LAUNCH_ITEMS(k_check_fp_acc, n, st, n, in, out);
+}
 hipError_t probe_fp_mul(hipStream_t st, int items, int iters, uint32_t* io) {
   LSG_LAUNCH_ITEMS(k_probe_fp_mul, items, st, items, iters, io);
 }
diff --git a/lodestar_amd/csrc/lsg_k_sig.hip b/lodestar_amd/csrc/lsg_k_sig.hip
--- a/lodestar_amd/csrc/lsg_k_sig.hip
+++ b/lodestar_amd/csrc/lsg_k_sig.hip
@@ -29,7 +29,7 @@
   LANE_ITEM(n);
   if (err[item] != 0 || inf[item]) return;
   lds_park(park, lane_load<g2a_t>(sig_aff, item));
-  bool ok = g2_in_group_get([&]() { return proj_from_aff(lds_unpark<g2a_t>(park)); });
+  bool ok = g2_in_group_aff_get([&]() { return lds_unpark<g2a_t>(park); });
   if (lead && !ok) err[item] = LSG_BLST_POINT_NOT_IN_GROUP;
 }
 
diff --git a/lodestar_amd/csrc/lsg_launch.h b/lodestar_amd/csrc/lsg_launch.h
--- a/lodestar_amd/csrc/lsg_launch.h
+++ b/lodestar_amd/csrc/lsg_launch.h
@@ -97,5 +97,7 @@
 hipError_t fp12_pow_u64(hipStream_t st, const uint8_t* in576, uint64_t r, uint8_t* out576);
 hipError_t probe_fp_mul(hipStream_t st, int items, int iters, uint32_t* io);
 hipError_t check_fp2_mul(hipStream_t st, int n, const uint32_t* in, uint32_t* out);
+hipError_t check_fp_acc(hipStream_t st, int n, const uint32_t* in, uint32_t* out);
+hipError_t check_g1_scale(hipStream_t st, int n, const uint8_t* in96, const uint64_t* k, uint8_t* out96);
 hipError_t probe_mad(hipStream_t st, int blocks, int iters, uint32_t seed, uint64_t* io);
 }
diff --git a/lodestar_amd/csrc/lsg_pairing.hpp b/lodestar_amd/csrc/lsg_pairing.hpp
--- a/lodestar_amd/csrc/lsg_pairing.hpp
+++ b/lodestar_amd/csrc/lsg_pairing.hpp
@@ -12,17 +12,15 @@
   fp2_t XX = fp2_sqr(T.X);
   line_t L;
   L.l00 = fp2_sub(t2, t0);
-  L.l01 = fp2_add(fp2_add(XX, XX), XX);
-  L.l11 = fp2_neg(fp2_add(t1, t1));
+  L.l01 = fp2_acc(XX).add(XX).add(XX).carry();
+  L.l11 = fp2_acc_neg(t1).sub(t1).carry();
   fp2_t Z3 = fp2_add(t0, t0);
   Z3 = fp2_add(Z3, Z3);
   Z3 = fp2_add(Z3, Z3);
   fp2_t X3 = fp2_mul(t2, Z3);
   fp2_t Y3 = fp2_add(t0, t2);
   Z3 = fp2_mul(t1, Z3);
-  fp2_t u1 = fp2_add(t2, t2);
-  fp2_t u2 = fp2_add(u1, t2);
-  fp2_t s0 = fp2_sub(t0, u2);
+  fp2_t s0 = fp2_acc(t0).sub(t2).sub(t2).sub(t2).carry();
   Y3 = fp2_mul(s0, Y3);
   Y3 = fp2_add(X3, Y3);
   fp2_t v1 = fp2_mul(T.X, T.Y);
@@ -46,7 +44,7 @@
   fp2_t E = fp2_mul(D, delta);
   fp2_t F = fp2_mul(T.Z, C);
   fp2_t G = fp2_mul(T.X, D);
-  fp2_t H = fp2_sub(fp2_add(E, F), fp2_add(G, G));
+  fp2_t H = fp2_acc(E).add(F).sub(G).sub(G).carry();
   fp2_t X3 = fp2_mul(delta, H);
   fp2_t Y3 = fp2_sub(fp2_mul(theta, fp2_sub(G, H)), fp2_mul(E, T.Y));
   fp2_t Z3 = fp2_mul(E, T.Z);
@@ -60,6 +58,75 @@
   L.l01 = fp2_mul_fp(L.l01, xP);
   L.l11 = fp2_mul_fp(L.l11, yP);
   return L;
+}
+
+template <int J, class G>
+LSG_INL fp2_t line_pair_coef(const G& V) {
+  static_assert(J >= 0 && J < 4, "line_pair_coef: J = 0..3");
+  if constexpr (J == 0) return fp2_acc(V(0)).add(fp2_acc(V(1)).mul_xi()).carry();
+  if constexpr (J == 1) return fp2_acc(V(3)).sub(V(0)).sub(V(2)).carry();
+  if constexpr (J == 2) return fp2_acc(V(4)).sub(V(0)).sub(V(1)).carry();
+  if constexpr (J == 3) return fp2_acc(V(5)).sub(V(2)).sub(V(1)).carry();
+}
+
+template <int J, class G>
+LSG_INL fp2_t fp12_sqr_coef(const G& V) {
+  static_assert(J >= 0 && J < 6, "fp12_sqr_coef: J = 0..5");
+  if constexpr (J == 0) {
+    const fp2_t k = fp6_fin_k0(V(7), V(8), V(9)).sub(fp6_fin_k0(V(1), V(2), V(3))).carry();
+    const fp2_t i = fp2_acc(k).sub(fp6_fin_c2(V(0), V(1), V(2), V(5))).carry();
+    return fp2_acc(V(6)).sub(V(0)).add(fp2_acc(i).mul_xi()).carry();
+  }
+  if constexpr (J == 1) {
+    const fp2_t k = fp6_fin_k0(V(1), V(2), V(3)).carry();
+    const fp2_t a = fp2_acc(V(10)).sub(V(6)).sub(V(7)).sub(V(4)).add(V(1)).carry();
+    const fp2_t i = fp2_acc(V(8)).sub(V(2)).sub(k).carry();
+    return fp2_acc(a).add(fp2_acc(i).mul_xi()).carry();
+  }
+  if constexpr (J == 2) {
+    const fp2_t a = fp6_fin_c2(V(6), V(7), V(8), V(11)).carry();
+    const fp2_t c = fp6_fin_c1(V(0), V(1), V(2), V(4)).carry();
+    return fp2_acc(a).sub(fp6_fin_c2(V(0), V(1), V(2), V(5))).sub(c).carry();
+  }
+  if constexpr (J >= 3) {
+    fp2_t t;
+    if constexpr (J == 3) t = fp6_fin_c0(V(0), V(1), V(2), V(3)).carry();
+    if constexpr (J == 4) t = fp6_fin_c1(V(0), V(1), V(2), V(4)).carry();
+    if constexpr (J == 5) t = fp6_fin_c2(V(0), V(1), V(2), V(5)).carry();
+    return fp2_acc(t).add(t).carry();
+  }
+}
+
+template <int J, class G>
+LSG_INL fp2_t fp12_mul_pair_coef(const G& V) {
+  static_assert(J >= 0 && J < 6, "fp12_mul_pair_coef: J = 0..5");
+  if constexpr (J == 0) {
+    const fp2_t k = fp6_fin_k0(V(1), V(2), V(4)).add(V(8)).sub(V(6)).carry();
+    return fp2_acc(V(0)).add(fp2_acc(k).sub(V(7)).mul_xi()).carry();
+  }
+  if constexpr (J == 1) {
+    const fp2_t s = fp2_acc(V(2)).add(V(7)).add(V(9)).carry();
+    return fp2_acc(V(3)).sub(V(0)).sub(V(1)).add(fp2_acc(s).mul_xi()).carry();
+  }
+  if constexpr (J == 2) {
+    const fp2_t n0 = fp2_acc(V(6)).add(fp2_acc(V(10)).mul_xi()).carry();
+    return fp6_fin_c2(V(0), V(1), V(2), V(5)).add(n0).carry();
+  }
+  if constexpr (J == 3) {
+    const fp2_t k = fp6_fin_k0(V(12), V(13), V(15)).sub(fp6_fin_k0(V(1), V(2), V(4))).carry();
+    const fp2_t i = fp2_acc(k).sub(V(7)).sub(V(9)).carry();
+    return fp2_acc(V(11)).sub(V(0)).add(fp2_acc(i).mul_xi()).carry();
+  }
+  if constexpr (J == 4) {
+    const fp2_t a = fp2_acc(V(14)).sub(V(11)).sub(V(12)).sub(V(3)).add(V(0)).add(V(1)).carry();
+    const fp2_t i = fp2_acc(V(13)).sub(V(2)).sub(V(10)).carry();
+    return fp2_acc(a).sub(V(6)).add(fp2_acc(i).mul_xi()).carry();
+  }
+  if constexpr (J == 5) {
+    const fp2_t a = fp6_fin_c2(V(11), V(12), V(13), V(16)).carry();
+    const fp2_t b = fp2_acc(a).sub(fp6_fin_c2(V(0), V(1), V(2), V(5))).carry();
+    return fp2_acc(b).sub(V(8)).add(V(6)).add(V(7)).carry();
+  }
 }
 
 #ifdef LSG_ROW_SPLIT
diff --git a/lodestar_amd/csrc/lsg_tower.hpp b/lodestar_amd/csrc/lsg_tower.hpp
--- a/lodestar_amd/csrc/lsg_tower.hpp
+++ b/lodestar_amd/csrc/lsg_tower.hpp
@@ -61,11 +61,37 @@
 
 LSG_INL fp_t fp_inv(const fp_t& a) { return fp_pow_id(a, LSG_POW_INV); }
 
+#ifndef LSG_FP_ACC
+template <int P, int N>
+struct fp_acc_t {
+  static_assert(P >= 0 && N >= 0 && P <= 3 && N <= 3,
+                "fp_acc_t: at most 3 terms added and 3 subtracted between two carries");
+  fp_t v;
+  LSG_INL fp_acc_t<P + 1, N> add(const fp_t& b) const { return fp_acc_t<P + 1, N>{fp_add(v, b)}; }
+  LSG_INL fp_acc_t<P, N + 1> sub(const fp_t& b) const { return fp_acc_t<P, N + 1>{fp_sub(v, b)}; }
+  template <int P2, int N2>
+  LSG_INL fp_acc_t<P + P2, N + N2> add(const fp_acc_t<P2, N2>& b) const {
+    return fp_acc_t<P + P2, N + N2>{fp_add(v, b.v)};
+  }
+  template <int P2, int N2>
+  LSG_INL fp_acc_t<P + N2, N + P2> sub(const fp_acc_t<P2, N2>& b) const {
+    return fp_acc_t<P + N2, N + P2>{fp_sub(v, b.v)};
+  }
+  template <int P2, int N2>
+  LSG_INL fp_acc_t<P2, N2> widen() const {
+    static_assert(P2 >= P && N2 >= N, "fp_acc_t: widen() only raises the term counts");
+    return fp_acc_t<P2, N2>{v};
+  }
+  LSG_INL fp_t carry() const { return v; }
+};
+LSG_INL fp_acc_t<1, 0> fp_acc(const fp_t& a) { return fp_acc_t<1, 0>{a}; }
+LSG_INL fp_acc_t<0, 1> fp_acc_neg(const fp_t& a) { return fp_acc_t<0, 1>{fp_neg(a)}; }
+#endif
+
 LSG_INL fp_t fp_mul12(const fp_t& a) {
-  fp_t a2 = fp_dbl(a);
-  fp_t a4 = fp_dbl(a2);
-  fp_t a8 = fp_dbl(a4);
-  return fp_add(a8, a4);
+  const fp_t a3 = fp_acc(a).add(a).add(a).carry();
+  const fp_t a6 = fp_acc(a3).add(a3).carry();
+  return fp_acc(a6).add(a6).carry();
 }
 
 struct fp2_t {
@@ -95,6 +121,28 @@
 LSG_INL fp2_t fp2_neg(const fp2_t& a) { return fp2_t(fp_neg(a.c0), fp_neg(a.c1)); }
 LSG_INL fp2_t fp2_conj(const fp2_t& a) { return fp2_t(a.c0, fp_neg(a.c1)); }
 
+template <int P, int N>
+struct fp2_acc_t {
+  static constexpr int XP = P + N > 2 * P ? P + N : 2 * P, XN = P + N > 2 * N ? P + N : 2 * N;
+  fp_acc_t<P, N> c0, c1;
+  LSG_INL fp2_acc_t<P + 1, N> add(const fp2_t& b) const { return fp2_acc_t<P + 1, N>{c0.add(b.c0), c1.add(b.c1)}; }
+  LSG_INL fp2_acc_t<P, N + 1> sub(const fp2_t& b) const { return fp2_acc_t<P, N + 1>{c0.sub(b.c0), c1.sub(b.c1)}; }
+  template <int P2, int N2>
+  LSG_INL fp2_acc_t<P + P2, N + N2> add(const fp2_acc_t<P2, N2>& b) const {
+    return fp2_acc_t<P + P2, N + N2>{c0.add(b.c0), c1.add(b.c1)};
+  }
+  template <int P2, int N2>
+  LSG_INL fp2_acc_t<P + N2, N + P2> sub(const fp2_acc_t<P2, N2>& b) const {
+    return fp2_acc_t<P + N2, N + P2>{c0.sub(b.c0), c1.sub(b.c1)};
+  }
+  LSG_INL fp2_acc_t<XP, XN> mul_xi() const {
+    return fp2_acc_t<XP, XN>{c0.sub(c1).template widen<XP, XN>(), c0.add(c1).template widen<XP, XN>()};
+  }
+  LSG_INL fp2_t carry() const { return fp2_t(c0.carry(), c1.carry()); }
+};
+LSG_INL fp2_acc_t<1, 0> fp2_acc(const fp2_t& a) { return fp2_acc_t<1, 0>{fp_acc(a.c0), fp_acc(a.c1)}; }
+LSG_INL fp2_acc_t<0, 1> fp2_acc_neg(const fp2_t& a) { return fp2_acc_t<0, 1>{fp_acc_neg(a.c0), fp_acc_neg(a.c1)}; }
+
 LSG_INL fp2_t fp2_mul(const fp2_t& a, const fp2_t& b) {
 #ifdef LSG_FP2_LEAF
   const fp_duo d = pair_fp2_mul(a.c0, a.c1, b.c0, b.c1);
@@ -191,8 +239,9 @@
 }
 
 LSG_INL fp2_t fp2_mul_b3(const fp2_t& a) {
-  fp2_t t = fp2_mul_xi(a);
-  return fp2_t(fp_mul12(t.c0), fp_mul12(t.c1));
+  const fp_t d3 = fp_acc(a.c0).add(a.c0).add(a.c0).sub(a.c1).sub(a.c1).sub(a.c1).carry();
+  const fp_t d6 = fp_acc(d3).add(d3).carry();
+  return fp2_t(fp_acc(d6).add(d6).carry(), fp_mul12(fp_add(a.c0, a.c1)));
 }
 
 LSG_INL uint32_t fp2_sgn0(const fp2_t& a) {
@@ -263,14 +312,23 @@
   A[5] = fp2_add(a.c0, a.c2);
   B[5] = fp2_add(b.c0, b.c2);
 }
+LSG_INL fp2_acc_t<1, 2> fp6_fin_k0(const fp2_t& v1, const fp2_t& v2, const fp2_t& m0) {
+  return fp2_acc(m0).sub(v1).sub(v2);
+}
+LSG_INL fp2_acc_t<3, 1> fp6_fin_c0(const fp2_t& v0, const fp2_t& v1, const fp2_t& v2, const fp2_t& m0) {
+  return fp2_acc(v0).add(fp2_acc(fp6_fin_k0(v1, v2, m0).carry()).mul_xi());
+}
+LSG_INL fp2_acc_t<3, 3> fp6_fin_c1(const fp2_t& v0, const fp2_t& v1, const fp2_t& v2, const fp2_t& m1) {
+  return fp2_acc(m1).sub(v0).sub(v1).add(fp2_acc(v2).mul_xi());
+}
+LSG_INL fp2_acc_t<2, 2> fp6_fin_c2(const fp2_t& v0, const fp2_t& v1, const fp2_t& v2, const fp2_t& m2) {
+  return fp2_acc(m2).sub(v0).sub(v2).add(v1);
+}
 LSG_INL fp6_t fp6_mul_fin(const fp2_t* V) {
-  fp2_t c0 = fp2_add(V[0], fp2_mul_xi(fp2_sub(fp2_sub(V[3], V[1]), V[2])));
-  fp2_t c1 = fp2_add(fp2_sub(fp2_sub(V[4], V[0]), V[1]), fp2_mul_xi(V[2]));
-  fp2_t c2 = fp2_add(fp2_sub(fp2_sub(V[5], V[0]), V[2]), V[1]);
   fp6_t r;
-  r.c0 = c0;
-  r.c1 = c1;
-  r.c2 = c2;
+  r.c0 = fp6_fin_c0(V[0], V[1], V[2], V[3]).carry();
+  r.c1 = fp6_fin_c1(V[0], V[1], V[2], V[4]).carry();
+  r.c2 = fp6_fin_c2(V[0], V[1], V[2], V[5]).carry();
   return r;
 }
 #ifdef LSG_LEAN_TOWER
@@ -278,9 +336,9 @@
   fp2_t v0 = fp2_mul(a.c0, b.c0);
   fp2_t v1 = fp2_mul(a.c1, b.c1);
   fp2_t v2 = fp2_mul(a.c2, b.c2);
-  fp2_t c0 = fp2_add(v0, fp2_mul_xi(fp2_sub(fp2_sub(fp2_mul(fp2_add(a.c1, a.c2), fp2_add(b.c1, b.c2)), v1), v2)));
-  fp2_t c1 = fp2_add(fp2_sub(fp2_sub(fp2_mul(fp2_add(a.c0, a.c1), fp2_add(b.c0, b.c1)), v0), v1), fp2_mul_xi(v2));
-  fp2_t c2 = fp2_add(fp2_sub(fp2_sub(fp2_mul(fp2_add(a.c0, a.c2), fp2_add(b.c0, b.c2)), v0), v2), v1);
+  fp2_t c0 = fp6_fin_c0(v0, v1, v2, fp2_mul(fp2_add(a.c1, a.c2), fp2_add(b.c1, b.c2))).carry();
+  fp2_t c1 = fp6_fin_c1(v0, v1, v2, fp2_mul(fp2_add(a.c0, a.c1), fp2_add(b.c0, b.c1))).carry();
+  fp2_t c2 = fp6_fin_c2(v0, v1, v2, fp2_mul(fp2_add(a.c0, a.c2), fp2_add(b.c0, b.c2))).carry();
   return fp6_make(c0, c1, c2);
 }
 #else
@@ -297,10 +355,22 @@
 LSG_BIGFN fp6_t fp6_mul_01(fp6_t a, fp2_t b0, fp2_t b1) {
   fp2_t t0 = fp2_mul(a.c0, b0);
   fp2_t t1 = fp2_mul(a.c1, b1);
-  fp2_t c0 = fp2_add(fp2_mul_xi(fp2_mul(a.c2, b1)), t0);
-  fp2_t c1 = fp2_sub(fp2_sub(fp2_mul(fp2_add(a.c0, a.c1), fp2_add(b0, b1)), t0), t1);
+  fp2_t c0 = fp2_acc(t0).add(fp2_acc(fp2_mul(a.c2, b1)).mul_xi()).carry();
+  fp2_t c1 = fp2_acc(fp2_mul(fp2_add(a.c0, a.c1), fp2_add(b0, b1))).sub(t0).sub(t1).carry();
   fp2_t c2 = fp2_add(fp2_mul(a.c2, b0), t1);
   return fp6_make(c0, c1, c2);
+}
+
+LSG_INL fp6_t fp6_add_mul_v(const fp6_t& a, const fp6_t& b) {
+  return fp6_make(fp2_acc(a.c0).add(fp2_acc(b.c2).mul_xi()).carry(), fp2_add(a.c1, b.c0), fp2_add(a.c2, b.c1));
+}
+LSG_INL fp6_t fp6_sub2(const fp6_t& a, const fp6_t& b, const fp6_t& c) {
+  return fp6_make(fp2_acc(a.c0).sub(b.c0).sub(c.c0).carry(), fp2_acc(a.c1).sub(b.c1).sub(c.c1).carry(),
+                  fp2_acc(a.c2).sub(b.c2).sub(c.c2).carry());
+}
+LSG_INL fp6_t fp6_sub_mul_v1(const fp6_t& u, const fp6_t& t) {
+  return fp6_make(fp2_acc(u.c0).sub(t.c0).sub(fp2_acc(t.c2).mul_xi()).carry(),
+                  fp2_acc(u.c1).sub(t.c1).sub(t.c0).carry(), fp2_acc(u.c2).sub(t.c2).sub(t.c1).carry());
 }
 
 LSG_INL fp6_t fp6_mul_1(const fp6_t& a, const fp2_t& b1) {
@@ -334,12 +404,12 @@
   fp6_t t0 = fp6_mul(a.c0, b.c0);
   fp6_t t1 = fp6_mul(a.c1, b.c1);
   fp6_t t2 = fp6_mul(fp6_add(a.c0, a.c1), fp6_add(b.c0, b.c1));
-  return fp12_make(fp6_add(t0, fp6_mul_v(t1)), fp6_sub(fp6_sub(t2, t0), t1));
+  return fp12_make(fp6_add_mul_v(t0, t1), fp6_sub2(t2, t0, t1));
 }
 LSG_BIGFN fp12_t fp12_sqr(fp12_t a) {
   fp6_t t = fp6_mul(a.c0, a.c1);
-  fp6_t u = fp6_mul(fp6_add(a.c0, a.c1), fp6_add(a.c0, fp6_mul_v(a.c1)));
-  return fp12_make(fp6_sub(fp6_sub(u, t), fp6_mul_v(t)), fp6_add(t, t));
+  fp6_t u = fp6_mul(fp6_add(a.c0, a.c1), fp6_add_mul_v(a.c0, a.c1));
+  return fp12_make(fp6_sub_mul_v1(u, t), fp6_add(t, t));
 }
 #else
 LSG_BIGFN fp12_t fp12_mul(fp12_t a, fp12_t b) {
@@ -349,24 +419,24 @@
   fp6_mul_prep(A + 12, B + 12, fp6_add(a.c0, a.c1), fp6_add(b.c0, b.c1));
   fp2_mul_n<18>(V, A, B);
   fp6_t t0 = fp6_mul_fin(V), t1 = fp6_mul_fin(V + 6), t2 = fp6_mul_fin(V + 12);
-  return fp12_make(fp6_add(t0, fp6_mul_v(t1)), fp6_sub(fp6_sub(t2, t0), t1));
+  return fp12_make(fp6_add_mul_v(t0, t1), fp6_sub2(t2, t0, t1));
 }
 
 LSG_BIGFN fp12_t fp12_sqr(fp12_t a) {
   fp2_t A[12], B[12], V[12];
   fp6_mul_prep(A, B, a.c0, a.c1);
-  fp6_mul_prep(A + 6, B + 6, fp6_add(a.c0, a.c1), fp6_add(a.c0, fp6_mul_v(a.c1)));
+  fp6_mul_prep(A + 6, B + 6, fp6_add(a.c0, a.c1), fp6_add_mul_v(a.c0, a.c1));
   fp2_mul_n<12>(V, A, B);
   fp6_t t = fp6_mul_fin(V), u = fp6_mul_fin(V + 6);
-  return fp12_make(fp6_sub(fp6_sub(u, t), fp6_mul_v(t)), fp6_add(t, t));
+  return fp12_make(fp6_sub_mul_v1(u, t), fp6_add(t, t));
 }
 #endif
 
 LSG_INL void fp4_square(fp2_t& c0, fp2_t& c1, const fp2_t& a, const fp2_t& b) {
   fp2_t t0 = fp2_sqr(a);
   fp2_t t1 = fp2_sqr(b);
-  c0 = fp2_add(fp2_mul_xi(t1), t0);
-  c1 = fp2_sub(fp2_sub(fp2_sqr(fp2_add(a, b)), t0), t1);
+  c0 = fp2_acc(t0).add(fp2_acc(t1).mul_xi()).carry();
+  c1 = fp2_acc(fp2_sqr(fp2_add(a, b))).sub(t0).sub(t1).carry();
 }
 
 LSG_BIGFN fp12_t fp12_cyclotomic_sqr(fp12_t f) {
@@ -422,7 +492,7 @@
   fp6_t t0 = fp6_mul_01(f.c0, l00, l01);
   fp6_t u = fp6_mul_01(fp6_add(f.c0, f.c1), l00, fp2_add(l01, l11));
   fp6_t t1 = fp6_mul_1(f.c1, l11);
-  return fp12_make(fp6_add(t0, fp6_mul_v(t1)), fp6_sub(fp6_sub(u, t0), t1));
+  return fp12_make(fp6_add_mul_v(t0, t1), fp6_sub2(u, t0, t1));
 #else
   const fp6_t& a = f.c0;
   const fp6_t& c = f.c1;
@@ -446,7 +516,7 @@
   fp6_t t0 = fp6_make(fp2_add(fp2_mul_xi(V[2]), V[0]), fp2_sub(fp2_sub(V[3], V[0]), V[1]), fp2_add(V[4], V[1]));
   fp6_t u = fp6_make(fp2_add(fp2_mul_xi(V[7]), V[5]), fp2_sub(fp2_sub(V[8], V[5]), V[6]), fp2_add(V[9], V[6]));
   fp6_t t1 = fp6_make(fp2_mul_xi(V[10]), V[11], V[12]);
-  return fp12_make(fp6_add(t0, fp6_mul_v(t1)), fp6_sub(fp6_sub(u, t0), t1));
+  return fp12_make(fp6_add_mul_v(t0, t1), fp6_sub2(u, t0, t1));
 #endif
 }
 
```

Result: faster. 3.536 million, median of 6 (+4.1%).
